# highfem/tqdne

Measured on AMD Instinct MI355X. Metric: waveforms/sec (train step + 18-step EDM sample), 3ch x 4096, higher is better.
Workload: dtype f32 (contractions on MFMA with fp32 accumulate: bf16x3, and fp16 + block-scaled-fp6 corrections on the 128/256-channel forward convs; sampler state f64)

## Files before the change

### include/tqdne_hip.h

```cpp
#ifndef TQDNE_HIP_H
#define TQDNE_HIP_H

#include <stddef.h>
#include <stdint.h>

#ifdef __cplusplus
extern "C" {
#endif

#ifndef __HIP__
typedef struct ihipStream_t* hipStream_t;
#endif

#define TQ_ABI_VERSION 8

#define TQ_ERR_ARG (-1)
#define TQ_ERR_SHAPE (-2)

#define TQ_CONV_GN 1
#define TQ_CONV_SILU 2
#define TQ_CONV_EMB 4
#define TQ_CONV_RES 8
#define TQ_CONV_STATS 16
#define TQ_CONV_DROPOUT 32
#define TQ_CONV_POLY2 64
#define TQ_CONV_CH_TILES 128
#define TQ_CONV_WIDE_TABLE 256

#define TQ_WFMT_BF16X3 0
#define TQ_WFMT_F16_MX8 1
#define TQ_WFMT_F16_MX6 2

typedef struct TqGnFold {
    const float* stats0;
    const float* stats1;
    int32_t slot0, slot1;
    const float* gamma;
    const float* beta;
    float* mean_rstd;
} TqGnFold;

typedef struct TqConvDesc {
    int32_t B, T_in, T_out;
    int32_t C_in0, C_in1;
    int32_t C_out;
    int32_t ktaps, stride, pad;
    int32_t upsample;
    int32_t flags;
    int32_t emb_stride;
    uint32_t dropout_site;
    float dropout_p;
    uint64_t dropout_seed;
    int32_t C_skip0, C_skip1;
    int32_t wfmt;
    int32_t* range_flag;
    const void* reserved1;
    int32_t t_tile;
    int32_t reserved2;
    const TqGnFold* gn_fold;
} TqConvDesc;

#define TQ_BWD_GN 1
#define TQ_BWD_SILU 2
#define TQ_BWD_DROPOUT 4
#define TQ_BWD_ACCUM 8
#define TQ_BWD_STATS 16

typedef struct TqConvBwdDesc {
    int32_t B, T;
    int32_t C_dy;
    int32_t C_dx0, C_dx1;
    int32_t ktaps;
    int32_t flags;
    uint32_t dropout_site;
    float dropout_p;
    uint64_t dropout_seed;
    int32_t wfmt;
    int32_t reserved;
    const uint32_t* dy_amax;
} TqConvBwdDesc;

int tq_abi_version(void);
int tq_build_flags(void);

size_t tq_conv_weight_pack_bytes(int C_out, int C_in, int K, int mode);
int tq_pack_conv_weight(const float* w, int C_out, int C_in, int K, int mode, void* packed, hipStream_t stream);
int tq_conv_tile_co(int C_out);
int tq_conv1d_max_cin(int wfmt, int C_out);
int tq_conv1d_max_cout(void);
size_t tq_conv1d_wide_lds_bytes(int ktaps, int t_tile, int C_out);
int tq_conv1d_gn_table_entries(int wide);
int tq_conv1d_gn_fold_max_cin(int wfmt, int t_tile, int C_out);
int tq_colsum_max_channels(void);
typedef struct TqPackJob {
    const void* src;
    void* dst;
    int32_t C_out, C_in, K, mode;
    int32_t block_begin;
    int32_t reserved;
} TqPackJob;
int tq_pack_job_blocks(int C_out, int C_in, int K, int mode);
int tq_pack_jobs(const TqPackJob* jobs_device, int njobs, int total_blocks, hipStream_t stream);

int tq_conv1d_fwd(const TqConvDesc* desc, const float* x0, const float* x1, const float* gscale, const float* gshift,
                  const void* packed_w, const float* bias, const float* emb, const float* residual, float* y,
                  float* stats_partial, hipStream_t stream);

int tq_conv1d_fwd_skip(const TqConvDesc* desc, const float* x0, const float* x1, const float* gscale, const float* gshift,
                       const void* packed_w_main_then_skip, const float* bias, const float* emb, const float* skip_x0,
                       const float* skip_x1, const float* skip_bias, float* y, float* stats_partial, hipStream_t stream);

#define TQ_KV_V_BF16 0
#define TQ_KV_V_F16 1
int tq_conv1d_fwd_qkv(const TqConvDesc* desc, const float* x, const float* gscale, const float* gshift, const void* packed_w,
                      const float* bias, float* qkv, void* kv_planes, int H, int D, int v_format, hipStream_t stream);

int tq_conv1d_bwd_data(const TqConvBwdDesc* desc, const float* dy, const void* packed_w_t, const float* x0, const float* x1,
                       const float* gscale, const float* gshift, float* dx0, float* dx1, float* gstats_partial,
                       hipStream_t stream);

size_t tq_conv1d_bwd_weight_workspace(const TqConvDesc* desc);
int tq_conv1d_bwd_weight(const TqConvDesc* desc, const float* dy, const float* x0, const float* x1, const float* gscale,
                         const float* gshift, float* dw, void* workspace, size_t ws_bytes, hipStream_t stream);
int tq_conv1d_bwd_weight_colsum(const TqConvDesc* desc, const float* dy, const float* x0, const float* x1, const float* gscale,
                                const float* gshift, float* dw, void* workspace, size_t ws_bytes, float* colsum_bc, int bc_stride,
                                float* colsum_c, float* colsum_c2, hipStream_t stream);

size_t tq_stem_conv_lds_bytes(int C_in, int C_out, int ktaps);
int tq_stem_conv_fwd(const float* x_nct, const float* in_scale, const float* w, const float* bias, float* y,
                     float* stats_partial, int B, int C_in, int T, int C_out, int ktaps, hipStream_t stream);

size_t tq_head_conv_lds_bytes(int C_in, int C_out, int ktaps);
int tq_head_conv_fwd(const float* x, const float* gscale, const float* gshift, const float* w, const float* bias,
                     const float* c_out, const float* c_skip, const float* skip_src, float* y_nct, int B, int T, int C_in,
                     int C_out, int ktaps, hipStream_t stream);

int tq_gn_finalize(const float* stats0, int C0, const float* stats1, int C1, int B, int T, const float* gamma,
                   const float* beta, float* gscale, float* gshift, float* mean_rstd, int slot0, int slot1, hipStream_t stream);

int tq_gn_bwd_finalize(const float* gstats_partial, const float* mean_rstd, const float* gamma, int B, int C, int T,
                       float* coef_a, float* coef_b, float* coef_c, float* dgamma, float* dbeta, hipStream_t stream);
int tq_gn_bwd_apply(const float* g, const float* x, const float* r, const float* coef_a, const float* coef_b,
                    const float* coef_c, float* dx, int B, int T, int C_src, int C_total, int c_offset, int accumulate,
                    hipStream_t stream);
int tq_gn_bwd_apply_colsum(const float* g, const float* x, const float* r, const float* coef_a, const float* coef_b,
                           const float* coef_c, float* dx, int B, int T, int C_src, int C_total, int c_offset, int accumulate,
                           float* colsum_bc, int bc_stride, float* colsum_c, float* colsum_c2, uint32_t* amax_out,
                           hipStream_t stream);
typedef struct TqGemmJob {
    const float* A;
    const float* B;
    float* C;
    const float* U;
    int32_t M, N, K;
    int32_t sam, sak, sbk, sbn, ldc, ldu;
    int32_t pre_b;
    int32_t tile_begin;
} TqGemmJob;
int tq_gemm_tiles(int M, int N);
int tq_gemm_f32_jobs(const TqGemmJob* jobs_device, int njobs, int total_tiles, hipStream_t stream);
int tq_fourier_features(const float* t, const float* W, float* out, int B, int half, hipStream_t stream);

#define TQ_AMAX_WAYS 16
#define TQ_AMAX_STRIDE 32
#define TQ_AMAX_WORDS (TQ_AMAX_WAYS * TQ_AMAX_STRIDE)
int tq_colsum(const float* dy, int B, int T, int C, float* out_bc, int bc_stride, float* out_c, float* out_c2,
              const float* bscale, uint32_t* amax_out, hipStream_t stream);
int tq_zero_stuff(const float* dy, float* out, int B, int T_out, int T_in, int C, hipStream_t stream);
int tq_pair_sum(const float* d_up, float* dx, int B, int T, int C, int accumulate, hipStream_t stream);
int tq_upsample_poly_wgrad_fold(const float* dw2, float* dw, int C_out, int C_in, hipStream_t stream);
int tq_stem_conv_bwd_weight(const float* dy, const float* x_nct, const float* in_scale, float* dw, int B, int C_in, int T,
                            int C_out, int ktaps, hipStream_t stream);
size_t tq_stem_head_bwd_workspace(void);
int tq_stem_conv_bwd_weight_ws(const float* dy, const float* x_nct, const float* in_scale, float* dw, int B, int C_in, int T,
                               int C_out, int ktaps, void* workspace, size_t ws_bytes, hipStream_t stream);
int tq_head_conv_bwd_ws(const float* dpred_nct, const float* c_out, const float* x, const float* gscale, const float* gshift,
                        const float* w, float* g_out, float* gstats_partial, float* dw, float* db, int B, int T, int C_in,
                        int C_out, int ktaps, void* workspace, size_t ws_bytes, hipStream_t stream);
size_t tq_head_conv_bwd_lds_bytes(int C_in, int C_out, int ktaps);
int tq_head_conv_bwd(const float* dpred_nct, const float* c_out, const float* x, const float* gscale, const float* gshift,
                     const float* w, float* g_out, float* gstats_partial, float* dw, float* db, int B, int T, int C_in,
                     int C_out, int ktaps, hipStream_t stream);

int tq_embed_fwd(const float* t, const float* cond, const float* fourier_w, const float* w0, const float* b0,
                 const float* w2, const float* b2, const float* cw0, const float* cb0, const float* cw2, const float* cb2,
                 float* emb, float* silu_emb, float* hidden ,
                 int B, int mc, int ncond, hipStream_t stream);

int tq_linear_fwd(const float* x, const float* w, const float* bias, float* out, int B, int E, int N, hipStream_t stream);

size_t tq_attention_workspace_bytes(int B, int T, int H, int D);
int tq_attention_fwd(const float* qkv, float* out, float* lse ,
                     void* workspace , int B, int T,
                     int H, int D, hipStream_t stream);
int tq_attention_fwd_presplit(const float* qkv, const void* kv_planes, float* out, int B, int T, int H, int D, int v_format,
                              hipStream_t stream);
int tq_attention_bwd(const float* qkv, const float* out, const float* dout, const float* lse, float* delta, float* dqkv, int B,
                     int T, int H, int D, hipStream_t stream);
int tq_attention_bwd_ws(const float* qkv, const float* out, const float* dout, const float* lse, float* delta, float* dqkv,
                        void* workspace, int B, int T, int H, int D, hipStream_t stream);
int tq_attention_bwd_ws_kv(const float* qkv, const float* out, const float* dout, const float* lse, float* delta, float* dqkv,
                           void* workspace, const void* kv_planes, int B, int T, int H, int D, hipStream_t stream);

int tq_attention_head_tile(int D);
size_t tq_attention_hd_lds_bytes(int D, int pass);
size_t tq_attention_hd_workspace_bytes(int B, int T, int H, int D);
int tq_attention_fwd_hd(const float* qkv, float* out, float* lse, void* workspace, int B, int T, int H, int D, hipStream_t stream);
int tq_attention_bwd_hd(const float* qkv, const float* out, const float* dout, const float* lse, float* delta, float* dqkv,
                        void* workspace, int B, int T, int H, int D, hipStream_t stream);

int tq_edm_scalars(const float* sigma, int sigma_stride, float sigma_data, float* c_in, float* c_out, float* c_skip,
                   float* c_noise, float* lweight, int B, hipStream_t stream);
int tq_cm_scalars(const float* sigma, int sigma_stride, float sigma_data, float sigma_min, float* c_out, float* c_skip,
                  int B, hipStream_t stream);
int tq_edm_noise_inject(const float* y, const float* unit_noise, const float* eps, float P_mean, float P_std,
                        float* sigma, float* x_noisy, int B, int n_per_sample, hipStream_t stream);
int tq_edm_loss(const float* pred, const float* y, const float* lweight, float* loss_out, float* dpred, int B,
                int n_per_sample, hipStream_t stream);
int tq_heun_euler(const double* x, const float* denoised, const float* sigma, const float* sigma_next, double* d_cur,
                  double* x_next, float* x32, size_t n, hipStream_t stream);
int tq_heun_correct(const double* x, const double* x_next, const float* denoised_next, const double* d_cur,
                    const float* sigma, const float* sigma_next, double* x_out, float* x32, size_t n, hipStream_t stream);
int tq_sampler_init(const double* unit_noise, const float* sigma0, double* x, float* x32, size_t n, hipStream_t stream);

int tq_heun_churn(const double* x, const double* unit_noise, const float* coef, double s_noise, double* x_hat, float* x32,
                  size_t n, hipStream_t stream);

int tq_axpy_sigma(const float* x, const float* noise, const float* sigma, float* out, int B, int n_per_sample,
                  hipStream_t stream);

int tq_scale_add2(const float* x, const float* y, const float* a, const float* c, float* out, int B, int n_per_sample,
                  hipStream_t stream);
int tq_ddpm_step(const float* x, const float* model_out, const float* noise, float* out, size_t n, int epsilon_prediction,
                 double sqrt_one_minus_abar, double inv_sqrt_abar, double clip, double coef_x0, double coef_xt, double sigma,
                 hipStream_t stream);

int tq_pseudo_huber_loss(const float* pred, const float* target, const float* weight, float c, float* loss_out, float* dpred,
                         int B, int n_per_sample, hipStream_t stream);

int tq_mse_loss(const float* a, const float* b, float* loss_out, float* d, size_t n, hipStream_t stream);

int tq_vae_reparam_fwd(const float* enc, const float* eps, float* z, float* kl_out, int B, int L, int T, hipStream_t stream);
int tq_vae_reparam_bwd(const float* enc, const float* eps, const float* dz, float* denc, float kl_weight, int B, int L, int T,
                       hipStream_t stream);

int tq_concat_scale(const float* x, const float* scale, const float* cond_signal, float* out, int B, int C0, int C1, int T,
                    hipStream_t stream);

int tq_boundary_max_channels(void);
int tq_nct_to_btc(const float* x_nct, const float* scale, const float* cond_nct, float* out_btc, int B, int C0, int C1, int T, int Cp,
                  hipStream_t stream);
int tq_btc_to_nct(const float* v_btc, const float* a, const float* s, const float* skip_src, float* y_nct, int B, int T, int Cp,
                  int c_off, int C, hipStream_t stream);

int tq_avg_pool2_fwd(const float* x, float* y, float* stats, int B, int T_in, int C, hipStream_t stream);
int tq_nearest_up2_fwd(const float* x, float* y, float* stats, int B, int T_in, int C, hipStream_t stream);
int tq_avg_pool2_bwd(const float* dy, float* dx, int B, int T_in, int C, int accumulate, hipStream_t stream);

#define TQ_ADAM_CHUNK 4096
typedef struct TqAdamChunk {
    float* p;
    const float* g;
    float* m;
    float* v;
    float* ema;
    int32_t n;
    int32_t reserved;
} TqAdamChunk;
int tq_adam_ema_step(const TqAdamChunk* chunks, int n_chunks, double step_size, double beta1, double beta2, double eps,
                     double inv_bias2_sqrt, double ema_weight, double grad_scale, double decay_factor, hipStream_t stream);
int tq_adam_ema_step_guarded(const TqAdamChunk* chunks, int n_chunks, double step_size, double beta1, double beta2, double eps,
                             double inv_bias2_sqrt, double ema_weight, double grad_scale, double decay_factor,
// ... 36 lines not shown
```

### tqdne_amd/_build.py

```python

from __future__ import annotations

import os
import subprocess
import sys

HERE = os.path.dirname(os.path.abspath(__file__))
CSRC = os.path.join(HERE, "csrc")
LIBDIR = os.path.join(HERE, "lib")
LIBPATH = os.path.join(LIBDIR, "libtqdne_hip.so")
SOURCES = ["conv1d_fwd_k5a.hip", "conv1d_fwd_k5b.hip", "conv1d_fwd_k13.hip", "conv1d_resample.hip", "conv1d_dgrad.hip", "conv1d_mfma.hip",
           "conv1d_fwd_wide.hip", "conv1d_fwd_wide_k13.hip", "small_ops.hip", "attention.hip", "attention_hd.hip", "backward.hip", "ends_wide.hip", "boundary.hip",
           "resample_plain.hip", "classifier.hip"]
ARCH = "gfx950"


def _hipcc() -> str:
    for c in (os.environ.get("HIPCC"), "/opt/rocm/bin/hipcc", "hipcc"):
        if c and (os.path.isabs(c) and os.path.exists(c) or not os.path.isabs(c)):
            return c
    raise RuntimeError("hipcc not found")


def _deps():
    return [os.path.join(CSRC, f) for f in os.listdir(CSRC)] + [os.path.join(HERE, "..", "include", "tqdne_hip.h")]


def needs_build(path: str = None) -> bool:
    path = path or LIBPATH
    if not os.path.exists(path):
        return True
    t = os.path.getmtime(path)
    return any(os.path.getmtime(d) > t for d in _deps() if os.path.exists(d))


def build(force: bool = False, verbose: bool = True, extra_flags=(), out_name=None) -> str:
    global_out = LIBPATH if out_name is None else os.path.join(LIBDIR, out_name)
    if out_name is None and not force and not needs_build(global_out):
        return global_out
    os.makedirs(LIBDIR, exist_ok=True)
    tag = "" if out_name is None else "." + out_name.replace(".so", "")
    objs = []
    procs = []
    for src in SOURCES:
        path = os.path.join(CSRC, src)
        if not os.path.exists(path):
            continue
        obj = os.path.join(LIBDIR, src.replace(".hip", tag + ".o"))
        cmd = [_hipcc(), f"--offload-arch={ARCH}", "-O3", "-fPIC", "-std=c++17", "-Wno-unused-value", "-Wno-ignored-attributes", "-Wno-cuda-compat", *extra_flags,
               "-c", path, "-o", obj]
        if verbose:
            print("[tqdne_amd build]", " ".join(cmd), flush=True)
        procs.append((cmd, subprocess.Popen(cmd, stdout=subprocess.PIPE, stderr=subprocess.STDOUT, text=True)))
        objs.append(obj)
    for cmd, p in procs:
        out, _ = p.communicate()
        if p.returncode != 0:
            raise RuntimeError("hipcc failed: %s\n%s" % (" ".join(cmd), out))
        if verbose and out.strip():
            print(out)
    cmd = [_hipcc(), f"--offload-arch={ARCH}", "-shared", "-fPIC", "-o", global_out] + objs
    if verbose:
        print("[tqdne_amd build]", " ".join(cmd), flush=True)
    r = subprocess.run(cmd, stdout=subprocess.PIPE, stderr=subprocess.STDOUT, text=True)
    if r.returncode != 0:
        raise RuntimeError("link failed:\n" + r.stdout)
    return global_out


if __name__ == "__main__":
    print(build(force="--force" in sys.argv))
```

### tqdne_amd/_lib.py

```python

from __future__ import annotations

import ctypes as C
import os
from typing import Optional

from . import _build

_LIB = None

c_f32p = C.c_void_p
VP = C.c_void_p
I = C.c_int
F = C.c_float
SZ = C.c_size_t

TQ_CONV_GN, TQ_CONV_SILU, TQ_CONV_EMB, TQ_CONV_RES, TQ_CONV_STATS, TQ_CONV_DROPOUT = 1, 2, 4, 8, 16, 32
TQ_CONV_POLY2 = 64
TQ_CONV_CH_TILES = 128
TQ_CONV_WIDE_TABLE = 256
TQ_WFMT_BF16X3, TQ_WFMT_F16_MX8, TQ_WFMT_F16_MX6 = 0, 1, 2
TQ_KV_V_BF16, TQ_KV_V_F16 = 0, 1
PACK_MODE = {TQ_WFMT_BF16X3: 0, TQ_WFMT_F16_MX8: 2, TQ_WFMT_F16_MX6: 3}
PACK_MODE_T = {TQ_WFMT_BF16X3: 1, TQ_WFMT_F16_MX6: 5}


DEFAULT_SCHEME = "f16mx6"
ABI_VERSION = 8


def requested_scheme() -> str:
    v = os.environ.get("TQDNE_CONV_SCHEME", DEFAULT_SCHEME).lower()
    if v not in ("bf16x3", "f16mx8", "f16mx6"):
        raise ValueError(f"TQDNE_CONV_SCHEME={v!r}: expected bf16x3, f16mx8 or f16mx6")
    return v


def attn_v_format() -> int:
    if os.environ.get("TQDNE_ATTN_VF16", "1") == "0" or requested_scheme() == "bf16x3":
        return TQ_KV_V_BF16
    return TQ_KV_V_F16


MX6_C64 = os.environ.get("TQDNE_CONV_MX6_C64", "0") == "1"


WIDE_MX6 = os.environ.get("TQDNE_WIDE_MX6", "1") != "0"


def conv_max_cin(wfmt: int, C_out: int = 0) -> int:
    return load().tq_conv1d_max_cin(wfmt, C_out)


def forward_wfmt(C_out: int, sources, stride: int = 1, upsample: bool = False, k5_act: bool = False,
                 gn: Optional[bool] = None) -> int:
    v = requested_scheme()
    co_ok = C_out % 128 == 0 or (C_out % 64 == 0 and k5_act and not upsample and v == "f16mx6" and MX6_C64)
    ok = stride == 1 and co_ok and all(c % 64 == 0 for c in sources if c)
    if not ok or v == "bf16x3":
        return TQ_WFMT_BF16X3
    fmt = TQ_WFMT_F16_MX6 if v == "f16mx6" else TQ_WFMT_F16_MX8
    cin = sum(c for c in list(sources)[:2] if c)
    if gn is None or gn:
        if cin > conv_max_cin(fmt, C_out) or (cin > load().tq_conv1d_gn_table_entries(0) and not WIDE_MX6):
            return TQ_WFMT_BF16X3
    return fmt
TQ_BWD_GN, TQ_BWD_SILU, TQ_BWD_DROPOUT, TQ_BWD_ACCUM, TQ_BWD_STATS = 1, 2, 4, 8, 16
STAT_SLOT = 128
TQ_AMAX_WAYS, TQ_AMAX_STRIDE = 16, 32
TQ_AMAX_WORDS = TQ_AMAX_WAYS * TQ_AMAX_STRIDE


class TqGnFold(C.Structure):
    _fields_ = [("stats0", C.c_void_p), ("stats1", C.c_void_p), ("slot0", C.c_int32), ("slot1", C.c_int32),
                ("gamma", C.c_void_p), ("beta", C.c_void_p), ("mean_rstd", C.c_void_p)]


class TqConvDesc(C.Structure):
    _fields_ = [
        ("B", C.c_int32), ("T_in", C.c_int32), ("T_out", C.c_int32),
        ("C_in0", C.c_int32), ("C_in1", C.c_int32), ("C_out", C.c_int32),
        ("ktaps", C.c_int32), ("stride", C.c_int32), ("pad", C.c_int32),
        ("upsample", C.c_int32), ("flags", C.c_int32), ("emb_stride", C.c_int32),
        ("dropout_site", C.c_uint32), ("dropout_p", C.c_float), ("dropout_seed", C.c_uint64),
        ("C_skip0", C.c_int32), ("C_skip1", C.c_int32), ("wfmt", C.c_int32),
        ("range_flag", C.c_void_p), ("reserved1", C.c_void_p), ("t_tile", C.c_int32), ("reserved2", C.c_int32),
        ("gn_fold", C.POINTER(TqGnFold)),
    ]


class TqAdamChunk(C.Structure):
    _fields_ = [("p", C.c_void_p), ("g", C.c_void_p), ("m", C.c_void_p), ("v", C.c_void_p), ("ema", C.c_void_p),
                ("n", C.c_int32), ("reserved", C.c_int32)]


TQ_ADAM_CHUNK = 4096


class TqGemmJob(C.Structure):
    _fields_ = [("A", C.c_void_p), ("B", C.c_void_p), ("C", C.c_void_p), ("U", C.c_void_p),
                ("M", C.c_int32), ("N", C.c_int32), ("K", C.c_int32),
                ("sam", C.c_int32), ("sak", C.c_int32), ("sbk", C.c_int32), ("sbn", C.c_int32), ("ldc", C.c_int32), ("ldu", C.c_int32),
                ("pre_b", C.c_int32), ("tile_begin", C.c_int32)]


class TqPackJob(C.Structure):
    _fields_ = [("src", C.c_void_p), ("dst", C.c_void_p), ("C_out", C.c_int32), ("C_in", C.c_int32), ("K", C.c_int32),
                ("mode", C.c_int32), ("block_begin", C.c_int32), ("reserved", C.c_int32)]


class TqConvBwdDesc(C.Structure):
    _fields_ = [
        ("B", C.c_int32), ("T", C.c_int32), ("C_dy", C.c_int32), ("C_dx0", C.c_int32), ("C_dx1", C.c_int32),
        ("ktaps", C.c_int32), ("flags", C.c_int32), ("dropout_site", C.c_uint32), ("dropout_p", C.c_float),
        ("dropout_seed", C.c_uint64), ("wfmt", C.c_int32), ("reserved", C.c_int32), ("dy_amax", C.c_void_p),
    ]


_PROTOS = {
    "tq_abi_version": (I, []),
    "tq_build_flags": (I, []),
    "tq_conv_weight_pack_bytes": (SZ, [I, I, I, I]),
    "tq_pack_conv_weight": (I, [VP, I, I, I, I, VP, VP]),
    "tq_conv_tile_co": (I, [I]),
    "tq_conv1d_max_cin": (I, [I, I]),
    "tq_conv1d_max_cout": (I, []),
    "tq_conv1d_gn_table_entries": (I, [I]),
    "tq_conv1d_wide_lds_bytes": (SZ, [I, I, I]),
    "tq_conv1d_gn_fold_max_cin": (I, [I, I, I]),
    "tq_colsum_max_channels": (I, []),
    "tq_conv1d_fwd": (I, [C.POINTER(TqConvDesc)] + [VP] * 11),
    "tq_conv1d_fwd_skip": (I, [C.POINTER(TqConvDesc)] + [VP] * 13),
    "tq_stem_conv_fwd": (I, [VP] * 6 + [I] * 5 + [VP]),
    "tq_head_conv_fwd": (I, [VP] * 9 + [I] * 5 + [VP]),
    "tq_head_conv_lds_bytes": (SZ, [I, I, I]),
    "tq_stem_conv_lds_bytes": (SZ, [I, I, I]),
    "tq_head_conv_bwd_lds_bytes": (SZ, [I, I, I]),
    "tq_gn_finalize": (I, [VP, I, VP, I, I, I, VP, VP, VP, VP, VP, I, I, VP]),
    "tq_embed_fwd": (I, [VP] * 14 + [I, I, I, VP]),
    "tq_linear_fwd": (I, [VP] * 4 + [I, I, I, VP]),
    "tq_attention_fwd": (I, [VP, VP, VP, VP, I, I, I, I, VP]),
    "tq_attention_fwd_presplit": (I, [VP, VP, VP, I, I, I, I, I, VP]),
    "tq_conv1d_fwd_qkv": (I, [C.POINTER(TqConvDesc)] + [VP] * 7 + [I, I, I, VP]),
    "tq_attention_workspace_bytes": (SZ, [I, I, I, I]),
    "tq_attention_bwd": (I, [VP] * 6 + [I, I, I, I, VP]),
    "tq_attention_bwd_ws": (I, [VP] * 7 + [I, I, I, I, VP]),
    "tq_attention_bwd_ws_kv": (I, [VP] * 8 + [I, I, I, I, VP]),
    "tq_attention_head_tile": (I, [I]),
    "tq_attention_hd_lds_bytes": (SZ, [I, I]),
    "tq_attention_hd_workspace_bytes": (SZ, [I, I, I, I]),
    "tq_attention_fwd_hd": (I, [VP, VP, VP, VP, I, I, I, I, VP]),
    "tq_attention_bwd_hd": (I, [VP] * 7 + [I, I, I, I, VP]),
    "tq_edm_scalars": (I, [VP, I, F, VP, VP, VP, VP, VP, I, VP]),
    "tq_cm_scalars": (I, [VP, I, F, F, VP, VP, I, VP]),
    "tq_edm_noise_inject": (I, [VP, VP, VP, F, F, VP, VP, I, I, VP]),
    "tq_edm_loss": (I, [VP, VP, VP, VP, VP, I, I, VP]),
    "tq_heun_euler": (I, [VP] * 7 + [SZ, VP]),
    "tq_heun_correct": (I, [VP] * 8 + [SZ, VP]),
    "tq_sampler_init": (I, [VP] * 4 + [SZ, VP]),
    "tq_heun_churn": (I, [VP, VP, VP, C.c_double, VP, VP, SZ, VP]),
    "tq_axpy_sigma": (I, [VP, VP, VP, VP, I, I, VP]),
    "tq_pseudo_huber_loss": (I, [VP, VP, VP, F, VP, VP, I, I, VP]),
    "tq_mse_loss": (I, [VP, VP, VP, VP, SZ, VP]),
    "tq_scale_add2": (I, [VP, VP, VP, VP, VP, I, I, VP]),
    "tq_ddpm_step": (I, [VP, VP, VP, VP, SZ, I] + [C.c_double] * 6 + [VP]),
    "tq_vae_reparam_fwd": (I, [VP, VP, VP, VP, I, I, I, VP]),
    "tq_vae_reparam_bwd": (I, [VP, VP, VP, VP, F, I, I, I, VP]),
    "tq_concat_scale": (I, [VP, VP, VP, VP, I, I, I, I, VP]),
    "tq_envelope_fwd": (I, [VP, VP, I, I, I, I, C.c_double, C.c_double, VP]),
    "tq_envelope_inv": (I, [VP, VP, I, I, I, C.c_double, C.c_double, VP]),
    "tq_adam_ema_step": (I, [VP, I] + [C.c_double] * 8 + [VP]),
    "tq_adam_ema_step_guarded": (I, [VP, I] + [C.c_double] * 8 + [VP, VP]),
    "tq_radam_ema_step_guarded": (I, [VP, I] + [C.c_double] * 7 + [VP, VP]),
    "tq_adam_ema_step_clipped": (I, [VP, I] + [C.c_double] * 8 + [VP, VP, C.c_double, VP]),
    "tq_radam_ema_step_clipped": (I, [VP, I] + [C.c_double] * 7 + [VP, VP, C.c_double, VP]),
    "tq_grad_sumsq": (I, [VP, I, VP, VP]),
    "tq_grad_clip_coef": (I, [VP, I, C.c_double, C.c_double, VP, VP]),
    "tq_ema_swap": (I, [VP, I, VP]),
    "tq_conv1d_bwd_data": (I, [VP] * 11),
    "tq_conv1d_bwd_weight_workspace": (SZ, [VP]),
    "tq_conv1d_bwd_weight": (I, [VP] * 8 + [SZ, VP]),
    "tq_conv1d_bwd_weight_colsum": (I, [VP] * 8 + [SZ, VP, I, VP, VP, VP]),
    "tq_gn_bwd_finalize": (I, [VP, VP, VP, I, I, I, VP, VP, VP, VP, VP, VP]),
    "tq_gn_bwd_apply": (I, [VP] * 7 + [I] * 6 + [VP]),
    "tq_gn_bwd_apply_colsum": (I, [VP] * 7 + [I] * 6 + [VP, I, VP, VP, VP, VP]),
    "tq_pack_job_blocks": (I, [I, I, I, I]),
    "tq_pack_jobs": (I, [VP, I, I, VP]),
    "tq_gemm_tiles": (I, [I, I]),
    "tq_gemm_f32_jobs": (I, [VP, I, I, VP]),
    "tq_fourier_features": (I, [VP, VP, VP, I, I, VP]),
    "tq_colsum": (I, [VP, I, I, I, VP, I, VP, VP, VP, VP, VP]),
    "tq_zero_stuff": (I, [VP, VP, I, I, I, I, VP]),
    "tq_pair_sum": (I, [VP, VP, I, I, I, I, VP]),
    "tq_upsample_poly_wgrad_fold": (I, [VP, VP, I, I, VP]),
    "tq_stem_conv_bwd_weight": (I, [VP] * 4 + [I] * 5 + [VP]),
    "tq_head_conv_bwd": (I, [VP] * 10 + [I] * 5 + [VP]),
    "tq_stem_head_bwd_workspace": (SZ, []),
    "tq_stem_conv_bwd_weight_ws": (I, [VP] * 4 + [I] * 5 + [VP, SZ, VP]),
    "tq_head_conv_bwd_ws": (I, [VP] * 10 + [I] * 5 + [VP, SZ, VP]),
    "tq_boundary_max_channels": (I, []),
    "tq_nct_to_btc": (I, [VP] * 4 + [I] * 5 + [VP]),
    "tq_btc_to_nct": (I, [VP] * 5 + [I] * 5 + [VP]),
    "tq_avg_pool2_fwd": (I, [VP, VP, VP, I, I, I, VP]),
    "tq_nearest_up2_fwd": (I, [VP, VP, VP, I, I, I, VP]),
    "tq_avg_pool2_bwd": (I, [VP, VP, I, I, I, I, VP]),
    "tq_classifier_head_max_channels": (I, []),
    "tq_classifier_head_max_classes": (I, []),
    "tq_classifier_head_bwd_workspace": (SZ, [I, I]),
    "tq_classifier_head_fwd": (I, [VP] * 11 + [I] * 4 + [VP]),
    "tq_cross_entropy": (I, [VP, VP, VP, C.c_int64, VP, VP, I, I, VP]),
    "tq_classifier_head_bwd": (I, [VP] * 15 + [SZ] + [I] * 4 + [VP]),
}

def lib_path() -> str:
    return os.environ.get("TQDNE_HIP_LIB", _build.LIBPATH)


def load():
    global _LIB
    if _LIB is not None:
        return _LIB
    path = lib_path()
    if not os.path.exists(path):
        raise RuntimeError(
            f"{path} is missing: the tqdne_amd hot path is HIP-only (no CPU / PyTorch fallback). "
            "Build it with `python -m tqdne_amd._build` (needs hipcc, cross-compiles gfx950 without a GPU)."
        )
    lib = C.CDLL(path)
    for name, (res, args) in _PROTOS.items():
        fn = getattr(lib, name)
        fn.restype = res
        fn.argtypes = args
    if lib.tq_abi_version() != ABI_VERSION:
        raise RuntimeError("libtqdne_hip.so ABI version mismatch")
    _LIB = lib
    return lib


def exported_symbols():
    return sorted(_PROTOS)


class TqError(RuntimeError):
    pass


def _p(t):
    return None if t is None else t.data_ptr()


def check(rc: int, what: str = ""):
    if rc != 0:
        kind = {-1: "TQ_ERR_ARG", -2: "TQ_ERR_SHAPE"}.get(rc, f"hipError_t {rc}")
        raise TqError(f"libtqdne_hip: {what} failed with {kind}")
```

### tqdne_amd/csrc/backward.hip

```cpp
#include <cstdlib>
#include "common.hpp"
#include "ends_wide.hpp"
#include "../../include/tqdne_hip.h"

using namespace tq;

namespace {

typedef short s16x4 __attribute__((ext_vector_type(4)));

__device__ __forceinline__ uint2 lds_tr_read(const unsigned char* p) {
    s16x4 v = __builtin_amdgcn_ds_read_tr16_b64_v4i16((__attribute__((address_space(3))) s16x4*)(p));
    union { s16x4 s; uint2 u; } c;
    c.s = v;
    return c.u;
}

struct WgArgs {
    const float* dy;
    const float* x0;
    const float* x1;
    const float* gscale;
    const float* gshift;
    float* slab;
// ... 500 lines not shown

extern "C" size_t tq_conv1d_bwd_weight_workspace(const TqConvDesc* d) {
    if (!d) return 0;
    int a, b, c, nsplit, nsplit4, ups;
    wgrad_plan(d, true, a, b, c, nsplit, ups);
    wgrad_plan(d, false, a, b, c, nsplit4, ups);
    return (size_t)(nsplit > nsplit4 ? nsplit : nsplit4) * d->ktaps * d->C_out * (d->C_in0 + d->C_in1) * sizeof(float);
}

extern "C" int tq_conv1d_bwd_weight(const TqConvDesc* d, const float* dy, const float* x0, const float* x1,
                                    const float* gscale, const float* gshift, float* dw, void* workspace, size_t ws_bytes,
                                    hipStream_t stream) {
    return tq_conv1d_bwd_weight_colsum(d, dy, x0, x1, gscale, gshift, dw, workspace, ws_bytes, nullptr, 0, nullptr, nullptr, stream);
}

extern "C" int tq_conv1d_bwd_weight_colsum(const TqConvDesc* d, const float* dy, const float* x0, const float* x1,
                                           const float* gscale, const float* gshift, float* dw, void* workspace, size_t ws_bytes,
                                           float* colsum_bc, int bc_stride, float* colsum_c, float* colsum_c2,
                                           hipStream_t stream) {
    if (!d || !dy || !x0 || !dw || !workspace) return TQ_ERR_ARG;
    if (colsum_c2 && !colsum_c) return TQ_ERR_ARG;
    if (d->C_in0 <= 0 || d->C_in0 % 32 || d->C_in1 < 0 || d->C_in1 % 32 || d->C_out <= 0 || d->C_out % 32) return TQ_ERR_SHAPE;
    if (d->C_in1 > 0 && !x1) return TQ_ERR_ARG;
    if ((d->flags & TQ_CONV_GN) && (!gscale || !gshift)) return TQ_ERR_ARG;
    if (ws_bytes < tq_conv1d_bwd_weight_workspace(d)) return TQ_ERR_ARG;
    WgArgs a;
    a.dy = dy; a.x0 = x0; a.x1 = x1; a.gscale = gscale; a.gshift = gshift; a.slab = reinterpret_cast<float*>(workspace);
    a.B = d->B; a.T_in = d->T_in; a.T_out = d->T_out; a.C0 = d->C_in0; a.C1 = d->C_in1; a.C_out = d->C_out;
    a.flags = d->flags;
    a.cs_bc = colsum_bc; a.cs_stride = bc_stride; a.cs_c = colsum_c; a.cs_c2 = colsum_c2;
    const bool wide = !(colsum_bc || colsum_c);
    wgrad_plan(d, wide, a.n_cotiles, a.n_cichunks, a.n_ttiles, a.nsplit, a.units_per_split);
    static const bool plain_order = [] { const char* e = getenv("TQDNE_WGRAD_XCD"); return e && atoi(e) == 0; }();
    if (plain_order) a.flags |= TQ_WGRAD_PLAIN_ORDER;
    a.drop_site = d->dropout_site; a.drop_seed = d->dropout_seed;
    float pdrop = d->dropout_p;
    if (!(d->flags & TQ_CONV_DROPOUT) || pdrop <= 0.f) { a.flags &= ~TQ_CONV_DROPOUT; pdrop = 0.f; }
    a.drop_thresh = (uint32_t)((double)pdrop * 4294967296.0);
    a.drop_scale = 1.0f / (1.0f - pdrop);
    int rc;
    const int nci = wgrad_nci(d);
    const bool h64 = wide && wgrad_h64(d);
    const bool w8 = wide && !h64 && wgrad_w8(d);
    if (d->stride == 2) {
        if (d->ktaps != 3) return TQ_ERR_SHAPE;
        rc = launch_wgrad<3, 2, 0>(a, nci, w8, false, stream);
    } else if (d->upsample) {
        if (d->ktaps == 5) rc = launch_wgrad<5, 1, 1>(a, nci, w8, false, stream);
        else if (d->ktaps == 3) rc = launch_wgrad<3, 1, 1>(a, nci, w8, false, stream);
        else return TQ_ERR_SHAPE;
    } else {
        if (d->ktaps == 5) rc = launch_wgrad<5, 1, 0>(a, nci, w8, h64, stream);
        else if (d->ktaps == 3) rc = launch_wgrad<3, 1, 0>(a, nci, w8, h64, stream);
        else if (d->ktaps == 1) rc = launch_wgrad<1, 1, 0>(a, nci, false, false, stream);
        else return TQ_ERR_SHAPE;
    }
    if (rc) return rc;
    const size_t n = (size_t)d->C_out * (d->C_in0 + d->C_in1);
    const dim3 rgrid((unsigned)((n + 63) / 64)), rblock(16, 16);
    if (d->ktaps == 5) hipLaunchKernelGGL(wgrad_reduce_kernel<5>, rgrid, rblock, 0, stream, a.slab, dw, a.nsplit, n);
    else if (d->ktaps == 3) hipLaunchKernelGGL(wgrad_reduce_kernel<3>, rgrid, rblock, 0, stream, a.slab, dw, a.nsplit, n);
    else hipLaunchKernelGGL(wgrad_reduce_kernel<1>, rgrid, rblock, 0, stream, a.slab, dw, a.nsplit, n);
    TQ_CHECK_LAUNCH();
    return 0;
}

namespace {
__global__ __launch_bounds__(256) void gn_bwd_finalize_kernel(const float* __restrict__ gst, const float* __restrict__ mr,
                                                              const float* __restrict__ gamma, int C, int T, int nslots,
                                                              float* __restrict__ cA, float* __restrict__ cB,
                                                              float* __restrict__ cC, float* __restrict__ dgamma,
                                                              float* __restrict__ dbeta) {
    extern __shared__ double sh[];
    const int b = blockIdx.x;
    const int Cb = C / (int)gridDim.y;
    const int c0 = (int)blockIdx.y * Cb;
    int nsub = Cb <= 128 ? (int)blockDim.x / Cb : 1;
    if (nsub > nslots) nsub = nslots;
    double* cs = sh;
    double* gp = sh + 2 * Cb * nsub;
    for (int idx = threadIdx.x; idx < Cb * nsub; idx += blockDim.x) {
        const int c = idx % Cb, sub = idx / Cb;
        const float* pp = gst + ((size_t)b * nslots * C + c0 + c) * 2;
        double s1 = 0.0, s2 = 0.0;
        int s = sub;
        for (; s + 3 * nsub < nslots; s += 4 * nsub) {
            const float2 v0 = *reinterpret_cast<const float2*>(pp + (size_t)s * C * 2);
            const float2 v1 = *reinterpret_cast<const float2*>(pp + (size_t)(s + nsub) * C * 2);
            const float2 v2 = *reinterpret_cast<const float2*>(pp + (size_t)(s + 2 * nsub) * C * 2);
            const float2 v3 = *reinterpret_cast<const float2*>(pp + (size_t)(s + 3 * nsub) * C * 2);
            s1 += ((double)v0.x + (double)v1.x) + ((double)v2.x + (double)v3.x);
            s2 += ((double)v0.y + (double)v1.y) + ((double)v2.y + (double)v3.y);
        }
        for (; s < nslots; s += nsub) {
            const float2 v = *reinterpret_cast<const float2*>(pp + (size_t)s * C * 2);
            s1 += (double)v.x; s2 += (double)v.y;
        }
        cs[2 * idx] = s1; cs[2 * idx + 1] = s2;
    }
    __syncthreads();
    if (nsub > 1) {
        double t1 = 0.0, t2 = 0.0;
        const int c = threadIdx.x;
        if (c < Cb)
            for (int sub = 0; sub < nsub; ++sub) { t1 += cs[2 * (sub * Cb + c)]; t2 += cs[2 * (sub * Cb + c) + 1]; }
        __syncthreads();
        if (c < Cb) { cs[2 * c] = t1; cs[2 * c + 1] = t2; }
        __syncthreads();
    }
    const int G = C / GN_GROUPS;
    const int ngrp = Cb / G, g0 = c0 / G;
    if ((int)threadIdx.x < ngrp) {
        const int gl = threadIdx.x, g = g0 + gl;
        const double mean = (double)mr[((size_t)b * GN_GROUPS + g) * 2], rstd = (double)mr[((size_t)b * GN_GROUPS + g) * 2 + 1];
        double p1 = 0.0, p2 = 0.0;
        for (int j = 0; j < G; ++j) {
            const int cl = gl * G + j;
            const double gm = (double)gamma[c0 + cl];
            p1 += gm * cs[2 * cl];
            p2 += gm * (cs[2 * cl + 1] - mean * cs[2 * cl]);
        }
        p2 *= rstd;
        const double n = (double)G * (double)T;
        gp[2 * gl] = -rstd * rstd * p2 / n;
        gp[2 * gl + 1] = rstd * rstd * p2 * mean / n - rstd * p1 / n;
    }
    __syncthreads();
    for (int cl = threadIdx.x; cl < Cb; cl += blockDim.x) {
        const int c = c0 + cl;
        const int g = c / G, gl = g - g0;
        const float mean = mr[((size_t)b * GN_GROUPS + g) * 2], rstd = mr[((size_t)b * GN_GROUPS + g) * 2 + 1];
        cA[(size_t)b * C + c] = rstd * gamma[c];
        cB[(size_t)b * C + c] = (float)gp[2 * gl];
        cC[(size_t)b * C + c] = (float)gp[2 * gl + 1];
        atomicAdd(dgamma + c, (float)((double)rstd * (cs[2 * cl + 1] - (double)mean * cs[2 * cl])));
        atomicAdd(dbeta + c, (float)cs[2 * cl]);
    }
}

__global__ void gn_bwd_apply_kernel(const float* __restrict__ g, const float* __restrict__ x, const float* __restrict__ r,
                                    const float* __restrict__ cA, const float* __restrict__ cB, const float* __restrict__ cC,
                                    float* __restrict__ dx, int T, int Cs, int Ctot, int coff, int accum, size_t n4) {
    const int c4n = Cs >> 2;
    for (size_t i = (size_t)blockIdx.x * blockDim.x + threadIdx.x; i < n4; i += (size_t)gridDim.x * blockDim.x) {
        const int c4 = (int)(i % c4n);
        const size_t bt = i / c4n;
        const int b = (int)(bt / T);
        const size_t ko = (size_t)b * Ctot + coff + 4 * c4;
        const float4 a = *reinterpret_cast<const float4*>(cA + ko);
        const float4 bb = *reinterpret_cast<const float4*>(cB + ko);
        const float4 cc = *reinterpret_cast<const float4*>(cC + ko);
        const float4 gv = reinterpret_cast<const float4*>(g)[i];
        const float4 xv = reinterpret_cast<const float4*>(x)[i];
        float4 o = make_float4(a.x * gv.x + bb.x * xv.x + cc.x, a.y * gv.y + bb.y * xv.y + cc.y,
                               a.z * gv.z + bb.z * xv.z + cc.z, a.w * gv.w + bb.w * xv.w + cc.w);
        if (r) { const float4 rv = reinterpret_cast<const float4*>(r)[i]; o.x += rv.x; o.y += rv.y; o.z += rv.z; o.w += rv.w; }
        if (accum) { const float4 ov = reinterpret_cast<const float4*>(dx)[i]; o.x += ov.x; o.y += ov.y; o.z += ov.z; o.w += ov.w; }
        reinterpret_cast<float4*>(dx)[i] = o;
    }
}

constexpr int AMAX_WAYS = TQ_AMAX_WAYS;
constexpr int AMAX_STRIDE = TQ_AMAX_STRIDE;

template <int NT>
__device__ __forceinline__ void colsum_finish(float* red, const float4& a, float mx, bool active, int c4n, int nrow, int c4, int tr, int C,
                                              int b, float sc, float* __restrict__ out_bc, int bc_stride, float* __restrict__ out_c,
                                              float* __restrict__ out_c2, unsigned* __restrict__ amax_out) {
    if (active) *reinterpret_cast<float4*>(red + (tr * c4n + c4) * 4) = a;
    unsigned* wmax = reinterpret_cast<unsigned*>(red + (size_t)nrow * c4n * 4);
    if (amax_out) {
        unsigned m = __float_as_uint(mx);
#pragma unroll
        for (int o = 32; o > 0; o >>= 1) m = max(m, (unsigned)__shfl_xor((int)m, o));
        if ((threadIdx.x & 63) == 0) wmax[threadIdx.x >> 6] = m;
    }
    __syncthreads();
    if (amax_out && threadIdx.x == 0) {
        unsigned m = wmax[0];
#pragma unroll
        for (int w = 1; w < NT / 64; ++w) m = max(m, wmax[w]);
        if (m != 0u) atomicMax(amax_out + (blockIdx.x % AMAX_WAYS) * AMAX_STRIDE, m);
    }
    for (int c = threadIdx.x; c < C; c += NT) {
        float s = 0.f;
        for (int r2 = 0; r2 < nrow; ++r2) s += red[(r2 * c4n + (c >> 2)) * 4 + (c & 3)];
        s *= sc;
        if (out_bc) atomicAdd(out_bc + (size_t)b * bc_stride + c, s);
        if (out_c) atomicAdd(out_c + c, s);
        if (out_c2) atomicAdd(out_c2 + c, s);
    }
}
__device__ __forceinline__ float amax4(float m, const float4& v) {
    const float t = fmaxf(fmaxf(fabsf(v.x), fabsf(v.y)), fmaxf(fabsf(v.z), fabsf(v.w)));
    const bool bad = (v.x != v.x) | (v.y != v.y) | (v.z != v.z) | (v.w != v.w);
    return bad ? __builtin_inff() : fmaxf(m, t);
}

template <int NT>
__global__ __launch_bounds__(NT) void colsum_kernel(const float* __restrict__ dy, int T, int C, float* __restrict__ out_bc,
                                                     int bc_stride, float* __restrict__ out_c, float* __restrict__ out_c2,
                                                     const float* __restrict__ bscale, unsigned* __restrict__ amax_out, int rpw) {
    extern __shared__ float red[];
    const int nsl = (T + rpw - 1) / rpw;
    const int slot = blockIdx.x % nsl, b = blockIdx.x / nsl;
    const int c4n = C >> 2;
    const int nrow = NT / c4n > 0 ? NT / c4n : 1;
    const int c4 = threadIdx.x % c4n, tr = threadIdx.x / c4n;
    float4 a = make_float4(0.f, 0.f, 0.f, 0.f);
    float mx = 0.f;
    const bool active = tr < nrow && threadIdx.x < nrow * c4n;
    if (active) {
        const int nvalid = min(rpw, T - slot * rpw);
        const float* src = dy + ((size_t)b * T + (size_t)slot * rpw) * C + 4 * c4;
        int tl = tr;
        for (; tl + 7 * nrow < nvalid; tl += 8 * nrow) {
            float4 v[8];
#pragma unroll
            for (int q = 0; q < 8; ++q) v[q] = *reinterpret_cast<const float4*>(src + (size_t)(tl + q * nrow) * C);
#pragma unroll
            for (int q = 0; q < 8; ++q) { a.x += v[q].x; a.y += v[q].y; a.z += v[q].z; a.w += v[q].w; }
            if (amax_out) {
#pragma unroll
                for (int q = 0; q < 8; ++q) mx = amax4(mx, v[q]);
            }
        }
        for (; tl < nvalid; tl += nrow) {
            const float4 v = *reinterpret_cast<const float4*>(src + (size_t)tl * C);
            a.x += v.x; a.y += v.y; a.z += v.z; a.w += v.w;
            if (amax_out) mx = amax4(mx, v);
        }
    }
    colsum_finish<NT>(red, a, mx, active, c4n, nrow, c4, tr, C, b, bscale ? bscale[b] : 1.0f, out_bc, bc_stride, out_c, out_c2, amax_out);
}

template <int NT>
__global__ __launch_bounds__(NT) void gn_bwd_apply_cs_kernel(const float* __restrict__ g, const float* __restrict__ x,
                                                              const float* __restrict__ r, const float* __restrict__ cA,
                                                              const float* __restrict__ cB, const float* __restrict__ cC,
                                                              float* __restrict__ dx, int T, int Cs, int Ctot, int coff, int accum,
                                                              float* __restrict__ out_bc, int bc_stride, float* __restrict__ out_c,
                                                              float* __restrict__ out_c2, unsigned* __restrict__ amax_out, int rpw) {
    extern __shared__ float red[];
    const int nsl = (T + rpw - 1) / rpw;
    const int slot = blockIdx.x % nsl, b = blockIdx.x / nsl;
    const int c4n = Cs >> 2;
    const int nrow = NT / c4n > 0 ? NT / c4n : 1;
    const int c4 = threadIdx.x % c4n, tr = threadIdx.x / c4n;
    float4 a = make_float4(0.f, 0.f, 0.f, 0.f);
    float mx = 0.f;
    const bool active = tr < nrow && threadIdx.x < nrow * c4n;
    if (active) {
        const int nvalid = min(rpw, T - slot * rpw);
        const size_t ko = (size_t)b * Ctot + coff + 4 * c4;
        const float4 ka = *reinterpret_cast<const float4*>(cA + ko);
        const float4 kb = *reinterpret_cast<const float4*>(cB + ko);
        const float4 kc = *reinterpret_cast<const float4*>(cC + ko);
        const size_t base = ((size_t)b * T + (size_t)slot * rpw) * Cs + 4 * c4;
        auto one = [&](const float4& gv, const float4& xv, const float4& rv, const float4& ov) -> float4 __attribute__((always_inline)) {
            float4 o = make_float4(ka.x * gv.x + kb.x * xv.x + kc.x, ka.y * gv.y + kb.y * xv.y + kc.y,
                                   ka.z * gv.z + kb.z * xv.z + kc.z, ka.w * gv.w + kb.w * xv.w + kc.w);
            o.x += rv.x; o.y += rv.y; o.z += rv.z; o.w += rv.w;
            o.x += ov.x; o.y += ov.y; o.z += ov.z; o.w += ov.w;
            return o;
        };
        const float4 z4 = make_float4(0.f, 0.f, 0.f, 0.f);
        int tl = tr;
        for (; tl + 3 * nrow < nvalid; tl += 4 * nrow) {
            float4 gv[4], xv[4], rv[4], ov[4];
#pragma unroll
            for (int q = 0; q < 4; ++q) {
                const size_t o = base + (size_t)(tl + q * nrow) * Cs;
                gv[q] = *reinterpret_cast<const float4*>(g + o);
                xv[q] = *reinterpret_cast<const float4*>(x + o);
                rv[q] = r ? *reinterpret_cast<const float4*>(r + o) : z4;
                ov[q] = accum ? *reinterpret_cast<const float4*>(dx + o) : z4;
            }
#pragma unroll
            for (int q = 0; q < 4; ++q) {
                const float4 o4 = one(gv[q], xv[q], rv[q], ov[q]);
                *reinterpret_cast<float4*>(dx + base + (size_t)(tl + q * nrow) * Cs) = o4;
                a.x += o4.x; a.y += o4.y; a.z += o4.z; a.w += o4.w;
                mx = amax4(mx, o4);
            }
        }
        for (; tl < nvalid; tl += nrow) {
            const size_t o = base + (size_t)tl * Cs;
            const float4 o4 = one(*reinterpret_cast<const float4*>(g + o), *reinterpret_cast<const float4*>(x + o),
                                  r ? *reinterpret_cast<const float4*>(r + o) : z4, accum ? *reinterpret_cast<const float4*>(dx + o) : z4);
            *reinterpret_cast<float4*>(dx + o) = o4;
            a.x += o4.x; a.y += o4.y; a.z += o4.z; a.w += o4.w;
            mx = amax4(mx, o4);
        }
    }
    colsum_finish<NT>(red, a, mx, active, c4n, nrow, c4, tr, Cs, b, 1.0f, out_bc, bc_stride, out_c, out_c2, amax_out);
}

struct CsChunk { int c0, cw; };
__device__ __forceinline__ CsChunk cs_chunk(int C, int cw) {
    const int c0 = (int)blockIdx.y * cw;
    return CsChunk{c0, min(cw, C - c0)};
}

template <int NT>
__global__ __launch_bounds__(NT) void colsum_chunk_kernel(const float* __restrict__ dy, int T, int C, int cw, float* __restrict__ out_bc,
                                                           int bc_stride, float* __restrict__ out_c, float* __restrict__ out_c2,
                                                           const float* __restrict__ bscale, unsigned* __restrict__ amax_out, int rpw) {
    extern __shared__ float red[];
    const CsChunk ck = cs_chunk(C, cw);
    const int nsl = (T + rpw - 1) / rpw;
    const int slot = blockIdx.x % nsl, b = blockIdx.x / nsl;
    const int c4n = ck.cw >> 2;
    const int nrow = NT / c4n > 0 ? NT / c4n : 1;
    const int c4 = threadIdx.x % c4n, tr = threadIdx.x / c4n;
    float4 a = make_float4(0.f, 0.f, 0.f, 0.f);
    float mx = 0.f;
    const bool active = tr < nrow && threadIdx.x < nrow * c4n;
    if (active) {
        const int nvalid = min(rpw, T - slot * rpw);
        const float* src = dy + ((size_t)b * T + (size_t)slot * rpw) * C + ck.c0 + 4 * c4;
        int tl = tr;
        for (; tl + 7 * nrow < nvalid; tl += 8 * nrow) {
            float4 v[8];
#pragma unroll
            for (int q = 0; q < 8; ++q) v[q] = *reinterpret_cast<const float4*>(src + (size_t)(tl + q * nrow) * C);
#pragma unroll
            for (int q = 0; q < 8; ++q) { a.x += v[q].x; a.y += v[q].y; a.z += v[q].z; a.w += v[q].w; }
            if (amax_out) {
#pragma unroll
                for (int q = 0; q < 8; ++q) mx = amax4(mx, v[q]);
            }
        }
        for (; tl < nvalid; tl += nrow) {
            const float4 v = *reinterpret_cast<const float4*>(src + (size_t)tl * C);
            a.x += v.x; a.y += v.y; a.z += v.z; a.w += v.w;
            if (amax_out) mx = amax4(mx, v);
        }
    }
    colsum_finish<NT>(red, a, mx, active, c4n, nrow, c4, tr, ck.cw, b, bscale ? bscale[b] : 1.0f, out_bc ? out_bc + ck.c0 : nullptr, bc_stride,
                      out_c ? out_c + ck.c0 : nullptr, out_c2 ? out_c2 + ck.c0 : nullptr, amax_out);
}

template <int NT>
__global__ __launch_bounds__(NT) void gn_bwd_apply_cs_chunk_kernel(const float* __restrict__ g, const float* __restrict__ x,
                                                                    const float* __restrict__ r, const float* __restrict__ cA,
                                                                    const float* __restrict__ cB, const float* __restrict__ cC,
                                                                    float* __restrict__ dx, int T, int Cs, int cw, int Ctot, int coff, int accum,
                                                                    float* __restrict__ out_bc, int bc_stride, float* __restrict__ out_c,
                                                                    float* __restrict__ out_c2, unsigned* __restrict__ amax_out, int rpw) {
    extern __shared__ float red[];
    const CsChunk ck = cs_chunk(Cs, cw);
    const int nsl = (T + rpw - 1) / rpw;
    const int slot = blockIdx.x % nsl, b = blockIdx.x / nsl;
    const int c4n = ck.cw >> 2;
    const int nrow = NT / c4n > 0 ? NT / c4n : 1;
    const int c4 = threadIdx.x % c4n, tr = threadIdx.x / c4n;
    float4 a = make_float4(0.f, 0.f, 0.f, 0.f);
    float mx = 0.f;
    const bool active = tr < nrow && threadIdx.x < nrow * c4n;
    if (active) {
        const int nvalid = min(rpw, T - slot * rpw);
        const size_t ko = (size_t)b * Ctot + coff + ck.c0 + 4 * c4;
        const float4 ka = *reinterpret_cast<const float4*>(cA + ko);
        const float4 kb = *reinterpret_cast<const float4*>(cB + ko);
        const float4 kc = *reinterpret_cast<const float4*>(cC + ko);
        const size_t base = ((size_t)b * T + (size_t)slot * rpw) * Cs + ck.c0 + 4 * c4;
        const float4 z4 = make_float4(0.f, 0.f, 0.f, 0.f);
        for (int tl = tr; tl < nvalid; tl += nrow) {
            const size_t o = base + (size_t)tl * Cs;
            const float4 gv = *reinterpret_cast<const float4*>(g + o), xv = *reinterpret_cast<const float4*>(x + o);
            const float4 rv = r ? *reinterpret_cast<const float4*>(r + o) : z4, ov = accum ? *reinterpret_cast<const float4*>(dx + o) : z4;
            float4 o4 = make_float4(ka.x * gv.x + kb.x * xv.x + kc.x, ka.y * gv.y + kb.y * xv.y + kc.y,
                                    ka.z * gv.z + kb.z * xv.z + kc.z, ka.w * gv.w + kb.w * xv.w + kc.w);
            o4.x += rv.x; o4.y += rv.y; o4.z += rv.z; o4.w += rv.w;
            o4.x += ov.x; o4.y += ov.y; o4.z += ov.z; o4.w += ov.w;
            *reinterpret_cast<float4*>(dx + o) = o4;
            a.x += o4.x; a.y += o4.y; a.z += o4.z; a.w += o4.w;
            mx = amax4(mx, o4);
        }
    }
    colsum_finish<NT>(red, a, mx, active, c4n, nrow, c4, tr, ck.cw, b, 1.0f, out_bc ? out_bc + ck.c0 : nullptr, bc_stride,
                      out_c ? out_c + ck.c0 : nullptr, out_c2 ? out_c2 + ck.c0 : nullptr, amax_out);
}


__global__ void zero_stuff_kernel(const float* __restrict__ dy, float* __restrict__ out, int T_out, int T_in, int C, size_t n4) {
    const int c4n = C >> 2;
    for (size_t i = (size_t)blockIdx.x * blockDim.x + threadIdx.x; i < n4; i += (size_t)gridDim.x * blockDim.x) {
        const int c4 = (int)(i % c4n);
        const size_t bu = i / c4n;
        const int u = (int)(bu % T_in);
        const size_t b = bu / T_in;
        float4 v = make_float4(0.f, 0.f, 0.f, 0.f);
        if (!(u & 1) && (u >> 1) < T_out) v = reinterpret_cast<const float4*>(dy)[(b * T_out + (u >> 1)) * c4n + c4];
        reinterpret_cast<float4*>(out)[i] = v;
    }
}

__global__ void pair_sum_kernel(const float* __restrict__ dup, float* __restrict__ dx, int T, int C, int accum, size_t n4) {
    const int c4n = C >> 2;
    for (size_t i = (size_t)blockIdx.x * blockDim.x + threadIdx.x; i < n4; i += (size_t)gridDim.x * blockDim.x) {
        const int c4 = (int)(i % c4n);
        const size_t bt = i / c4n;
        const int t = (int)(bt % T);
        const size_t b = bt / T;
        const float4 a = reinterpret_cast<const float4*>(dup)[(b * 2 * T + 2 * t) * c4n + c4];
        const float4 c = reinterpret_cast<const float4*>(dup)[(b * 2 * T + 2 * t + 1) * c4n + c4];
        float4 o = make_float4(a.x + c.x, a.y + c.y, a.z + c.z, a.w + c.w);
        if (accum) { const float4 ov = reinterpret_cast<const float4*>(dx)[i]; o.x += ov.x; o.y += ov.y; o.z += ov.z; o.w += ov.w; }
        reinterpret_cast<float4*>(dx)[i] = o;
    }
}

inline unsigned ew_grid4(size_t n4) {
    size_t g = (n4 + 255) / 256;
    return (unsigned)(g > 4096 ? 4096 : (g ? g : 1));
}
}

extern "C" int tq_gn_bwd_finalize(const float* gstats, const float* mean_rstd, const float* gamma, int B, int C, int T,
                                  float* coef_a, float* coef_b, float* coef_c, float* dgamma, float* dbeta,
                                  hipStream_t stream) {
    if (!gstats || !mean_rstd || !gamma || !coef_a || !coef_b || !coef_c || !dgamma || !dbeta) return TQ_ERR_ARG;
    if (B <= 0 || T <= 0 || C <= 0 || C % GN_GROUPS) return TQ_ERR_SHAPE;
    const int nslots = (T + STAT_SLOT - 1) / STAT_SLOT;
    const int NP = 4;
    const int Cb = C / NP;
    int nsub = Cb <= 128 ? 256 / Cb : 1;
    if (nsub > nslots) nsub = nslots;
    const size_t sh = (size_t)(2 * Cb * nsub + 2 * GN_GROUPS) * sizeof(double);
    hipLaunchKernelGGL(gn_bwd_finalize_kernel, dim3(B, NP), dim3(256), sh, stream, gstats, mean_rstd, gamma, C, T, nslots, coef_a,
                       coef_b, coef_c, dgamma, dbeta);
    TQ_CHECK_LAUNCH();
    return 0;
}

extern "C" int tq_gn_bwd_apply(const float* g, const float* x, const float* r, const float* coef_a, const float* coef_b,
                               const float* coef_c, float* dx, int B, int T, int C_src, int C_total, int c_offset, int accumulate,
                               hipStream_t stream) {
    if (!g || !x || !coef_a || !coef_b || !coef_c || !dx) return TQ_ERR_ARG;
    if (B <= 0 || T <= 0 || C_src <= 0 || C_src % 4 || c_offset % 4 || c_offset + C_src > C_total) return TQ_ERR_SHAPE;
    const size_t n4 = (size_t)B * T * (C_src / 4);
    hipLaunchKernelGGL(gn_bwd_apply_kernel, dim3(ew_grid4(n4)), dim3(256), 0, stream, g, x, r, coef_a, coef_b, coef_c, dx, T,
                       C_src, C_total, c_offset, accumulate, n4);
    TQ_CHECK_LAUNCH();
    return 0;
}

constexpr int CS_NT = 256;
struct CsTiling { int rows; };
static CsTiling colsum_tiling(int B, int T) {
    CsTiling t;
    const size_t min_wgs = 256;
    int rpw = STAT_SLOT;
    while (rpw < 4096 && (size_t)B * ((T + 2 * rpw - 1) / (2 * rpw)) >= min_wgs) rpw <<= 1;
    t.rows = rpw;
    return t;
}

constexpr int CS_CHUNK = 1024;
constexpr int CS_MAX_C = CS_CHUNK * 64;
static int colsum_chunk_width(int C, int& nchunks) {
    const int c4 = C / 4;
    nchunks = (c4 + CS_CHUNK / 4 - 1) / (CS_CHUNK / 4);
    return ((c4 + nchunks - 1) / nchunks) * 4;
}
extern "C" int tq_colsum_max_channels(void) { return CS_MAX_C; }

extern "C" int tq_colsum(const float* dy, int B, int T, int C, float* out_bc, int bc_stride, float* out_c, float* out_c2,
                         const float* bscale, uint32_t* amax_out, hipStream_t stream) {
    if (!dy || (!out_bc && !out_c && !out_c2 && !amax_out)) return TQ_ERR_ARG;
    if (B <= 0 || T <= 0 || C < 4 || C % 4 || C > CS_MAX_C) return TQ_ERR_SHAPE;
    const CsTiling tl = colsum_tiling(B, T);
    const int nsl = (T + tl.rows - 1) / tl.rows;
    if (C > CS_CHUNK) {
        int nch;
        const int cw = colsum_chunk_width(C, nch);
        const size_t shw = (size_t)(CS_NT > cw / 4 ? CS_NT : cw / 4) * 4 * sizeof(float) + (CS_NT / 64) * sizeof(unsigned);
        hipLaunchKernelGGL(colsum_chunk_kernel<CS_NT>, dim3(B * nsl, nch), dim3(CS_NT), shw, stream, dy, T, C, cw, out_bc, bc_stride, out_c, out_c2, bscale, amax_out, tl.rows);
        TQ_CHECK_LAUNCH();
        return 0;
    }
    const int c4n = C / 4;
    const int nrow = CS_NT / c4n > 0 ? CS_NT / c4n : 1;
    const size_t sh = (size_t)nrow * c4n * 4 * sizeof(float) + (CS_NT / 64) * sizeof(unsigned);
    hipLaunchKernelGGL(colsum_kernel<CS_NT>, dim3(B * nsl), dim3(CS_NT), sh, stream, dy, T, C, out_bc, bc_stride, out_c, out_c2, bscale, amax_out, tl.rows);
    TQ_CHECK_LAUNCH();
    return 0;
}

extern "C" int tq_gn_bwd_apply_colsum(const float* g, const float* x, const float* r, const float* coef_a, const float* coef_b,
                                      const float* coef_c, float* dx, int B, int T, int C_src, int C_total, int c_offset, int accumulate,
                                      float* colsum_bc, int bc_stride, float* colsum_c, float* colsum_c2, uint32_t* amax_out,
                                      hipStream_t stream) {
    if (!g || !x || !coef_a || !coef_b || !coef_c || !dx) return TQ_ERR_ARG;
    if (colsum_c2 && !colsum_c) return TQ_ERR_ARG;
    if (B <= 0 || T <= 0 || C_src <= 0 || C_src % 4 || C_src > CS_MAX_C || c_offset % 4 || c_offset + C_src > C_total) return TQ_ERR_SHAPE;
    if (!colsum_bc && !colsum_c && !amax_out)
        return tq_gn_bwd_apply(g, x, r, coef_a, coef_b, coef_c, dx, B, T, C_src, C_total, c_offset, accumulate, stream);
    const CsTiling tl = colsum_tiling(B, T);
    const int nsl = (T + tl.rows - 1) / tl.rows;
    if (C_src > CS_CHUNK) {
        int nch;
        const int cw = colsum_chunk_width(C_src, nch);
        const size_t shw = (size_t)(CS_NT > cw / 4 ? CS_NT : cw / 4) * 4 * sizeof(float) + (CS_NT / 64) * sizeof(unsigned);
        hipLaunchKernelGGL(gn_bwd_apply_cs_chunk_kernel<CS_NT>, dim3(B * nsl, nch), dim3(CS_NT), shw, stream, g, x, r, coef_a, coef_b, coef_c, dx, T,
                           C_src, cw, C_total, c_offset, accumulate, colsum_bc, bc_stride, colsum_c, colsum_c2, amax_out, tl.rows);
        TQ_CHECK_LAUNCH();
        return 0;
    }
    const int c4n = C_src / 4;
    const int nrow = CS_NT / c4n > 0 ? CS_NT / c4n : 1;
    const size_t sh = (size_t)nrow * c4n * 4 * sizeof(float) + (CS_NT / 64) * sizeof(unsigned);
    hipLaunchKernelGGL(gn_bwd_apply_cs_kernel<CS_NT>, dim3(B * nsl), dim3(CS_NT), sh, stream, g, x, r, coef_a, coef_b, coef_c, dx, T, C_src,
                       C_total, c_offset, accumulate, colsum_bc, bc_stride, colsum_c, colsum_c2, amax_out, tl.rows);
    TQ_CHECK_LAUNCH();
    return 0;
}

extern "C" int tq_zero_stuff(const float* dy, float* out, int B, int T_out, int T_in, int C, hipStream_t stream) {
    if (!dy || !out || B <= 0 || T_out <= 0 || T_in <= 0 || C <= 0 || C % 4) return TQ_ERR_ARG;
    const size_t n4 = (size_t)B * T_in * (C / 4);
    hipLaunchKernelGGL(zero_stuff_kernel, dim3(ew_grid4(n4)), dim3(256), 0, stream, dy, out, T_out, T_in, C, n4);
    TQ_CHECK_LAUNCH();
    return 0;
}
// ... 593 lines not shown
```

### tqdne_amd/csrc/common.hpp

```cpp
#pragma once
#include <hip/hip_runtime.h>
#include <stdint.h>

#include <cstdlib>

namespace tq {

typedef __bf16 bf16x8 __attribute__((ext_vector_type(8)));
typedef __bf16 bf16x4 __attribute__((ext_vector_type(4)));
typedef float f32x4 __attribute__((ext_vector_type(4)));
typedef _Float16 f16x8 __attribute__((ext_vector_type(8)));
typedef _Float16 f16x4 __attribute__((ext_vector_type(4)));
typedef short i16x2 __attribute__((ext_vector_type(2)));
typedef int i32x8 __attribute__((ext_vector_type(8)));

constexpr int WAVE = 64;

constexpr int GN_GROUPS = 32;
constexpr float GN_EPS = 1e-5f;
constexpr int STAT_SLOT = 128;

__device__ __forceinline__ float silu_f(float u) {
    return u * __builtin_amdgcn_rcpf(1.0f + __expf(-u));
}
__device__ __forceinline__ float dsilu_f(float u) {
    float s = __builtin_amdgcn_rcpf(1.0f + __expf(-u));
    return s * (1.0f + u * (1.0f - s));
}

__device__ __forceinline__ void split_bf16(float x, __bf16& hi, __bf16& lo) {
    hi = (__bf16)x;
    lo = (__bf16)(x - (float)hi);
}

union Frag {
    bf16x8 v;
    uint4 u;
    uint2 h[2];
};

__device__ __forceinline__ f32x4 mfma_bf16(const bf16x8& a, const bf16x8& b, f32x4 c) {
    return __builtin_amdgcn_mfma_f32_16x16x32_bf16(a, b, c, 0, 0, 0);
}

__device__ __forceinline__ f32x4 mfma_x3(const bf16x8& ah, const bf16x8& al, const bf16x8& bh, const bf16x8& bl, f32x4 c) {
    c = mfma_bf16(al, bh, c);
    c = mfma_bf16(ah, bl, c);
    c = mfma_bf16(ah, bh, c);
    return c;
}

__device__ __forceinline__ int xcd_group_id(int bid, int inner, int n_outer) {
    if (n_outer & 7) return bid;
    const int x = bid & 7, s = bid >> 3;
    return (x + 8 * (s / inner)) * inner + (s % inner);
}

__device__ __forceinline__ float wave_sum(float v) {
#pragma unroll
    for (int o = 32; o > 0; o >>= 1) v += __shfl_xor(v, o);
    return v;
}
__device__ __forceinline__ double wave_sum_d(double v) {
#pragma unroll
    for (int o = 32; o > 0; o >>= 1) v += __shfl_xor(v, o);
    return v;
}

__device__ __forceinline__ uint32_t mix32(uint32_t x) {
    x ^= x >> 16; x *= 0x7FEB352Du;
    x ^= x >> 15; x *= 0x846CA68Bu;
    x ^= x >> 16;
    return x;
}
struct DropKey { uint32_t a, b; };
__device__ __forceinline__ DropKey drop_key(uint64_t seed, uint32_t site, uint32_t b) {
    uint32_t k = mix32((uint32_t)seed ^ 0x9E3779B9u);
    k = mix32(k ^ (uint32_t)(seed >> 32));
    k = mix32(k + 0x85EBCA6Bu * (site + 1u));
    DropKey r;
    r.a = mix32(k + 0xC2B2AE35u * (b + 1u));
    r.b = mix32((k ^ 0x27D4EB2Fu) + 0x165667B1u * (b + 1u));
    return r;
}
__device__ __forceinline__ uint32_t drop_hash(DropKey key, uint32_t e) {
    uint32_t x = e ^ key.a;
    x ^= x >> 16; x *= 0x7FEB352Du;
    x += key.b;
    x ^= x >> 15; x *= 0x846CA68Bu;
    x ^= x >> 16;
    return x;
}

}

#define TQ_CHECK_LAUNCH()                                   \
    do {                                                    \
        hipError_t e__ = hipGetLastError();                 \
        if (e__ != hipSuccess) return (int)e__;             \
    } while (0)
```

### tqdne_amd/csrc/conv1d_kernel.hpp

```cpp
#pragma once
#include <cmath>
#include <cstdlib>
#include <type_traits>

#include "common.hpp"
#include "conv_args.hpp"
#include "gn_fold.hpp"
#include <atomic>
#include "../../include/tqdne_hip.h"

using namespace tq;

#ifdef TQ_STAMP
static __device__ unsigned long long tq_stamps[12];
#ifdef TQ_STAMP_OWNER
extern "C" int tq_debug_read_stamps(unsigned long long* out, int reset) {
    hipError_t e = hipMemcpyFromSymbol(out, HIP_SYMBOL(tq_stamps), sizeof(unsigned long long) * 12);
    if (e != hipSuccess) return (int)e;
    if (reset) {
        unsigned long long z[12] = {0, 0, 0, 0, 0, 0, 0, 0, 0, 0, 0, 0};
        e = hipMemcpyToSymbol(HIP_SYMBOL(tq_stamps), z, sizeof(z));
    }
    return (int)e;
}
#endif
static __device__ unsigned long long tq_timeline[4096 * 8];
#ifdef TQ_STAMP_OWNER
extern "C" int tq_debug_read_timeline(unsigned long long* out, int n) {
    return (int)hipMemcpyFromSymbol(out, HIP_SYMBOL(tq_timeline), sizeof(unsigned long long) * 8 * n);
}
#endif
#define TQ_T(x) const unsigned long long x = __builtin_amdgcn_s_memtime(); __builtin_amdgcn_sched_barrier(0);
#else
#define TQ_T(x)
#endif

namespace {

#ifndef TQ_STAGE_PRE
#define TQ_STAGE_PRE 5
#endif

template <int KT, int STRIDE, int UPS, int WM, int WN, int SCH = 0, int TBW = 8, int NCB = 2>
struct Cfg {
    static constexpr int CH = SCH ? 64 : 32;
    static constexpr int ROWB = 2 * CH;
    static constexpr int TPR = (SCH == 2) ? 4 : CH / 4;
    static constexpr int NWB = SCH ? 4 : 2;
    static constexpr int NW = NWB * NCB;
    static constexpr int NBF = SCH ? 4 : 2;
    static constexpr int NTHR = 64 * WM * WN;
    static constexpr int WT = 16 * TBW;
    static constexpr int NT = WT * WN;
    static constexpr int MT = 16 * NCB * WM;
    static constexpr int ROWS = (STRIDE == 1) ? (NT + KT - 1) : (2 * NT + 1);
    static constexpr int NIT = (ROWS * TPR + NTHR - 1) / NTHR;
    static constexpr int PRE_MAX = (SCH == 1 && WM == 4) ? 1 : TQ_STAGE_PRE;
    static constexpr int PRE = NIT < PRE_MAX ? NIT : PRE_MAX;
    static constexpr int SYNC_BATCH = 4;
    static constexpr int ITERS = (NIT <= PRE) ? NIT : PRE + ((NIT - PRE + SYNC_BATCH - 1) / SYNC_BATCH) * SYNC_BATCH;
    static constexpr int NFULL = (SCH == 2) ? (NT * 4) / NTHR : 0;
    static constexpr int HALO_TASKS = (SCH == 2) ? (ROWS - NT) * 4 : 0;
    static constexpr int ROWS_PAD = (SCH == 2) ? ROWS : (ITERS * NTHR + TPR - 1) / TPR;
    static constexpr int PLANE = (ROWS_PAD > ROWS ? ROWS_PAD : ROWS) * ROWB;
    static constexpr int BUF = 2 * PLANE;
    static constexpr int LDS_BYTES = 2 * BUF;
    static constexpr int PAD = (STRIDE == 1) ? (KT / 2) : 1;
};

template <int KT, int STRIDE, int UPS, int WM, int WN, int EPI, int ACT, bool FUSE, int SCH, bool PW = false, int TBW = 8, int NCB = 2, int GTW = 1024>
__global__ __launch_bounds__(64 * WM * WN, 2) void conv1d_mfma_kernel(const ConvArgs p) {
    static_assert(GTW == 1024 || (GTW == 2048 && SCH == 2 && ACT >= 1 && EPI == 0 && !PW && STRIDE == 1 && UPS == 0 && WN == 1 && NCB == 2 && (TBW == 8 || TBW == 2)),
                  "wide coefficient table: the fp16 + MX-fp6 forward tiles of 128 and 32 positions");
    static_assert(SCH == 0 || STRIDE == 1, "the fp16-range schemes serve stride-1 launches");
    static_assert(EPI != 1 || SCH == 0 || (SCH == 2 && ACT == 0 && !FUSE && !PW), "data gradients: bf16x3, or fp16 + MX-fp6 on a dy scaled into the fp16 range");
    static_assert(NCB == 2, "waves are 32 channels wide");
    constexpr bool C64 = TBW == 4 && NCB == 2 && SCH == 2 && WM == 2 && WN == 2;
    static_assert(!C64 || (STRIDE == 1 && UPS == 0 && !PW && EPI != 2), "64-channel fp16 + MX-fp6 tile: stride-1 forward and data-gradient launches");
    static_assert(TBW == 8 || C64 || (TBW == 2 && (SCH == 0 || (SCH == 2 && WM == 4)) && STRIDE == 1 && UPS == 0 && EPI == 0 && WN == 1 && !PW),
                  "small tile (32 positions per workgroup): stride-1 forward, one wave column");
    static_assert(!PW || (KT == 1 && STRIDE == 1 && UPS == 0 && SCH >= 1 && !FUSE && WN == 1 && EPI != 1), "PW: 1x1, fp16-range schemes");
    static_assert(SCH != 2 || WN == 1 || C64, "scheme 2 tiles are 128 positions wide");
    using C = Cfg<KT, STRIDE, UPS, WM, WN, SCH, TBW, NCB>;
    extern __shared__ __attribute__((aligned(16))) unsigned char lds[];
#ifdef TQ_STAMP
    const unsigned long long t_entry = __builtin_amdgcn_s_memtime();
    const unsigned long long r_entry = __builtin_amdgcn_s_memrealtime();
#endif

    const int tid = threadIdx.x;
    const int lane = tid & 63;
    const int wave = __builtin_amdgcn_readfirstlane(tid >> 6);
    const int wm = wave % WM;
    const int wn = wave / WM;

    const int n_ttiles = (p.T_out + C::NT - 1) / C::NT;
    const int n_ctiles = (p.C_out + C::MT - 1) / C::MT;
    int bid = blockIdx.x;
    int ct, tile;
    const int ntile = p.B * n_ttiles;
    if constexpr (PW) {
        ct = 0;
        tile = bid;
    } else if (n_ctiles > 1 && (ntile & 7) == 0) {
        const int grp = bid / (8 * n_ctiles), within = bid % (8 * n_ctiles);
        ct = within >> 3;
        tile = grp * 8 + (within & 7);
    } else {
        ct = bid % n_ctiles;
        tile = bid / n_ctiles;
    }
    const int tt = tile % n_ttiles;
    const int b = tile / n_ttiles;
    const int t0 = tt * C::NT;
    float dy_scale = 1.f, dy_unscale = 1.f;
    if constexpr (EPI == 1 && SCH == 2) {
        if (p.in_amax) {
            uint32_t amx = 0u;
#pragma unroll
            for (int w = 0; w < TQ_AMAX_WAYS; ++w) amx = max(amx, p.in_amax[w * TQ_AMAX_STRIDE]);
            const int e = (int)((amx >> 23) & 0xFFu);
            int k = 140 - e;
            k = k > 126 ? 126 : (k < -126 ? -126 : k);
            dy_scale = __uint_as_float((unsigned)(127 + k) << 23);
            dy_unscale = __uint_as_float((unsigned)(127 - k) << 23);
        }
    }
    const DropKey dkey = (ACT == 3 || EPI == 1) ? drop_key(p.drop_seed, p.drop_site, (uint32_t)b) : DropKey{0u, 0u};
    int co_wave = ct * C::MT + wm * (16 * NCB);
    const bool wave_active = co_wave < p.C_out;

    const int Cin = p.C0 + p.C1;
    const int nchunks = Cin / C::CH;
    const int nskip = FUSE ? ((p.sC0 + p.sC1) / C::CH) : 0;
    const int nstages = nchunks + nskip;
    const int T_src = UPS ? 2 * p.T_in : p.T_in;

    const int m = tid % C::TPR;
    const int wslot = m >> 1, whalf = m & 1;
    constexpr bool TIGHT = SCH == 1 && WM == 8 && C::PRE == 5 && C::NIT == 5;
    constexpr int PRE = (TIGHT && ACT == 3) ? 1 : (TIGHT && FUSE) ? 4 : C::PRE;
    constexpr int SYNC_BATCH = (TIGHT && ACT == 3) ? 4 : (TIGHT && FUSE) ? 1 : C::SYNC_BATCH;
    float4 raw[PRE];
    float4 g_a, g_s;

    auto src_pos = [&](int i) -> int __attribute__((always_inline)) {
        if (STRIDE == 1) return t0 - C::PAD + i;
        const int par = (i > C::NT) ? 1 : 0;
        const int idx = i - par * (C::NT + 1);
        return 2 * t0 - C::PAD + 2 * idx + par;
    };

    auto chunk_base = [&](int stage, int& cs) -> const float* __attribute__((always_inline)) {
        const bool sk = FUSE && stage >= nchunks;
        const int cb = (sk ? stage - nchunks : stage) * C::CH;
        const float* a0 = sk ? p.sx0 : p.x0;
        const float* a1 = sk ? p.sx1 : p.x1;
        const int c0 = sk ? p.sC0 : p.C0, c1 = sk ? p.sC1 : p.C1;
        const bool first = cb < c0;
        const float* src = first ? a0 : a1;
        cs = first ? c0 : c1;
        const int coff = first ? cb : cb - c0;
        return src + (size_t)b * p.T_in * cs + coff + 4 * m;
    };

    auto load_one = [&](const float* base, int cs, int it) -> float4 __attribute__((always_inline)) {
        const int i = (tid + it * C::NTHR) / C::TPR;
        int pos = src_pos(i);
        pos = pos < 0 ? 0 : (pos >= T_src ? T_src - 1 : pos);
        const int srow = UPS ? (pos >> 1) : pos;
        return *reinterpret_cast<const float4*>(base + (size_t)srow * cs);
    };

    auto write_one = [&](int chunk, int buf, int it, const float4& rv) __attribute__((always_inline)) {
        unsigned char* hi_plane = lds + buf * C::BUF;
        unsigned char* lo_plane = hi_plane + C::PLANE;
        const int i = (tid + it * C::NTHR) / C::TPR;
        const int pos = src_pos(i);
        const float msk = (pos >= 0 && pos < T_src) ? 1.f : 0.f;
        float u[4] = {rv.x, rv.y, rv.z, rv.w};
        const bool act = !(FUSE && chunk >= nchunks);
        if (ACT >= 1 && act) {
            u[0] = fmaf(g_a.x, u[0], g_s.x); u[1] = fmaf(g_a.y, u[1], g_s.y);
            u[2] = fmaf(g_a.z, u[2], g_s.z); u[3] = fmaf(g_a.w, u[3], g_s.w);
        }
        if (ACT >= 2 && act) {
#pragma unroll
            for (int j = 0; j < 4; ++j)
                u[j] = u[j] * __builtin_amdgcn_rcpf(1.0f + __builtin_amdgcn_exp2f(u[j] * -1.4426950408889634f));
        }
        if (ACT == 3 && act) {
            const int cb = chunk * C::CH;
            const int pc = pos < 0 ? 0 : pos;
            const uint32_t e0 = (uint32_t)pc * (uint32_t)Cin + (uint32_t)(cb + 4 * m);
#pragma unroll
            for (int j = 0; j < 4; ++j)
                u[j] = (drop_hash(dkey, e0 + j) >= p.drop_thresh) ? u[j] * p.drop_scale : 0.f;
        }
        if constexpr (SCH == 0) {
            uint32_t hb[4];
            float lo[4];
#pragma unroll
            for (int j = 0; j < 4; ++j) {
                u[j] *= msk;
                hb[j] = __float_as_uint(u[j]) & 0xFFFF0000u;
                lo[j] = u[j] - __uint_as_float(hb[j]);
            }
            uint2 hv;
            hv.x = (hb[0] >> 16) | hb[1];
            hv.y = (hb[2] >> 16) | hb[3];
            bf16x4 l;
            l[0] = (__bf16)lo[0]; l[1] = (__bf16)lo[1]; l[2] = (__bf16)lo[2]; l[3] = (__bf16)lo[3];
            const int off = i * 64 + ((wslot ^ (((i >> 2) & 1) << 1)) << 4) + (whalf << 3);
            *reinterpret_cast<uint2*>(hi_plane + off) = hv;
            *reinterpret_cast<bf16x4*>(lo_plane + off) = l;
        } else {
            f16x4 hv;
            float xl[4], xc[4];
#pragma unroll
            for (int j = 0; j < 4; ++j) {
                u[j] *= msk;
                hv[j] = (_Float16)u[j];
                xl[j] = __builtin_amdgcn_fmed3f(u[j] - (float)hv[j], -0.109375f, 0.109375f);
                xc[j] = __builtin_amdgcn_fmed3f(u[j], -448.f, 448.f);
// ... 583 lines not shown
            const float sc = sec == 1 ? p.kvscale : 1.0f;
            const int dch = d0 + (odd ? 16 + 4 * (g - 1) : 4 * g);
            unsigned char* base0 = p.kv + (((size_t)b * p.kvH + h) * 4 + (sec == 1 ? 0 : 2)) * plane + (size_t)dch * 2;
            float vmax = 0.f;
#pragma unroll
            for (int tb = 0; tb < TBW; ++tb) {
                const int t = t0 + wn * C::WT + tb * 16 + (lane & 15);
                uint2 hi[2], lo[2];
#pragma unroll
                for (int cbk = 0; cbk < 2; ++cbk) {
                    const float v[4] = {acc[cbk][tb][0] + add[cbk].x, acc[cbk][tb][1] + add[cbk].y,
                                        acc[cbk][tb][2] + add[cbk].z, acc[cbk][tb][3] + add[cbk].w};
                    if (sec == 2 && p.kv_vf16) {
                        f16x4 hh, ll;
#pragma unroll
                        for (int j = 0; j < 4; ++j) {
                            hh[j] = (_Float16)v[j];
                            ll[j] = (_Float16)(v[j] - (float)hh[j]);
                            vmax = fmaxf(vmax, fabsf(v[j]));
                        }
                        hi[cbk] = __builtin_bit_cast(uint2, hh);
                        lo[cbk] = __builtin_bit_cast(uint2, ll);
                    } else {
                        bf16x4 hh, ll;
#pragma unroll
                        for (int j = 0; j < 4; ++j) {
                            __bf16 a, c;
                            split_bf16(v[j] * sc, a, c);
                            hh[j] = a; ll[j] = c;
                        }
                        hi[cbk] = __builtin_bit_cast(uint2, hh);
                        lo[cbk] = __builtin_bit_cast(uint2, ll);
                    }
                }
                const uint2 sh = odd ? hi[0] : hi[1], sl = odd ? lo[0] : lo[1];
                uint2 rh, rl;
                rh.x = __shfl_xor((int)sh.x, 16); rh.y = __shfl_xor((int)sh.y, 16);
                rl.x = __shfl_xor((int)sl.x, 16); rl.y = __shfl_xor((int)sl.y, 16);
                const uint4 oh = odd ? make_uint4(rh.x, rh.y, hi[1].x, hi[1].y) : make_uint4(hi[0].x, hi[0].y, rh.x, rh.y);
                const uint4 ol = odd ? make_uint4(rl.x, rl.y, lo[1].x, lo[1].y) : make_uint4(lo[0].x, lo[0].y, rl.x, rl.y);
                if (t < p.T_out) {
                    unsigned char* dst = base0 + (size_t)t * p.kvD * 2;
                    *reinterpret_cast<uint4*>(dst) = oh;
                    *reinterpret_cast<uint4*>(dst + plane) = ol;
                }
            }
            if (p.range_flag && !(vmax < 32752.f)) *p.range_flag = 1;
        }
    } else if constexpr (EPI == 0) {
    const bool poly = p.flags & TQ_CONV_POLY2;
    const int Cr = poly ? (p.C_out >> 1) : p.C_out;
    const int ph = (poly && co_wave >= Cr) ? 1 : 0;
    const int co_real = co_wave - ph * Cr;
    const int slot = poly ? 2 * ((t0 >> 7) + wn) + ph : (TBW == 2 ? (t0 >> 5) : (t0 >> 7) + (TBW == 8 ? wn : 0));
    const float* emb_b = (p.flags & TQ_CONV_EMB) ? p.emb + (size_t)b * p.emb_stride : nullptr;
    float4 add[NCB];
    float s1[NCB][4], s2[NCB][4];
#pragma unroll
    for (int cbk = 0; cbk < NCB; ++cbk) {
        const int co = co_real + cbk * 16 + 4 * (lane >> 4);
        add[cbk] = make_float4(0.f, 0.f, 0.f, 0.f);
        if (p.bias) add[cbk] = *reinterpret_cast<const float4*>(p.bias + co);
        if (emb_b) {
            const float4 e = *reinterpret_cast<const float4*>(emb_b + co);
            add[cbk].x += e.x; add[cbk].y += e.y; add[cbk].z += e.z; add[cbk].w += e.w;
        }
        if (FUSE && p.sbias) {
            const float4 e = *reinterpret_cast<const float4*>(p.sbias + co);
            add[cbk].x += e.x; add[cbk].y += e.y; add[cbk].z += e.z; add[cbk].w += e.w;
        }
#pragma unroll
        for (int j = 0; j < 4; ++j) { s1[cbk][j] = 0.f; s2[cbk][j] = 0.f; }
    }
    const bool res_epi = (!RES_EARLY || poly) && (p.flags & TQ_CONV_RES);
    float4 rq[TBW][NCB];
    if (res_epi) {
#pragma unroll
        for (int tb = 0; tb < TBW; ++tb) {
            const int t = t0 + wn * C::WT + tb * 16 + (lane & 15);
            const int tc = t < p.T_out ? t : p.T_out - 1;
#pragma unroll
            for (int cbk = 0; cbk < NCB; ++cbk) {
                const int co = co_real + cbk * 16 + 4 * (lane >> 4);
                const size_t o = poly ? ((size_t)b * 2 * p.T_out + 2 * tc + ph) * Cr + co : ((size_t)b * p.T_out + tc) * p.C_out + co;
                rq[tb][cbk] = *reinterpret_cast<const float4*>(p.res + o);
            }
        }
    }
#pragma unroll
    for (int tb = 0; tb < TBW; ++tb) {
        int t = t0 + wn * C::WT + tb * 16 + (lane & 15);
        asm volatile("" : "+v"(t));
        if (t < p.T_out) {
#pragma unroll
            for (int cbk = 0; cbk < NCB; ++cbk) {
                const int co = co_real + cbk * 16 + 4 * (lane >> 4);
                const size_t o = poly ? ((size_t)b * 2 * p.T_out + 2 * t + ph) * Cr + co : ((size_t)b * p.T_out + t) * p.C_out + co;
                float4 v = make_float4(acc[cbk][tb][0] + add[cbk].x, acc[cbk][tb][1] + add[cbk].y,
                                       acc[cbk][tb][2] + add[cbk].z, acc[cbk][tb][3] + add[cbk].w);
                if (res_epi) {
                    const float4 r = rq[tb][cbk];
                    v.x += r.x; v.y += r.y; v.z += r.z; v.w += r.w;
                }
#ifdef TQ_ABL_NOEPI
                if (v.x == 1.2345e30f)
#endif
                *reinterpret_cast<float4*>(p.y + o) = v;
                s1[cbk][0] += v.x; s1[cbk][1] += v.y; s1[cbk][2] += v.z; s1[cbk][3] += v.w;
                s2[cbk][0] += v.x * v.x; s2[cbk][1] += v.y * v.y; s2[cbk][2] += v.z * v.z; s2[cbk][3] += v.w * v.w;
            }
        }
    }
    if (p.flags & TQ_CONV_STATS) {
#pragma unroll
        for (int cbk = 0; cbk < NCB; ++cbk) {
#pragma unroll
            for (int j = 0; j < 4; ++j) {
#pragma unroll
                for (int o = 1; o < 16; o <<= 1) {
                    s1[cbk][j] += __shfl_xor(s1[cbk][j], o);
                    s2[cbk][j] += __shfl_xor(s2[cbk][j], o);
                }
            }
        }
        if constexpr (TBW == 4) {
            __syncthreads();
            float* red = reinterpret_cast<float*>(lds) + (wm * 4 + (lane >> 4)) * (8 * NCB);
            if (wn == 1 && (lane & 15) == 0) {
#pragma unroll
                for (int cbk = 0; cbk < NCB; ++cbk)
#pragma unroll
                    for (int j = 0; j < 4; ++j) { red[(cbk * 4 + j) * 2] = s1[cbk][j]; red[(cbk * 4 + j) * 2 + 1] = s2[cbk][j]; }
            }
            __syncthreads();
            if (wn == 0 && (lane & 15) == 0) {
#pragma unroll
                for (int cbk = 0; cbk < NCB; ++cbk)
#pragma unroll
                    for (int j = 0; j < 4; ++j) { s1[cbk][j] += red[(cbk * 4 + j) * 2]; s2[cbk][j] += red[(cbk * 4 + j) * 2 + 1]; }
            }
        }
#pragma unroll
        for (int cbk = 0; cbk < NCB; ++cbk) {
            const int co = co_real + cbk * 16 + 4 * (lane >> 4);
            if ((lane & 15) == 0 && slot < p.nslots && (TBW == 8 || wn == 0)) {
                float* st = p.stats + (((size_t)b * p.nslots + slot) * Cr + co) * 2;
                *reinterpret_cast<float4*>(st) = make_float4(s1[cbk][0], s2[cbk][0], s1[cbk][1], s2[cbk][1]);
                *reinterpret_cast<float4*>(st + 4) = make_float4(s1[cbk][2], s2[cbk][2], s1[cbk][3], s2[cbk][3]);
                const float q = fmaxf(fmaxf(s2[cbk][0], s2[cbk][1]), fmaxf(s2[cbk][2], s2[cbk][3]));
                if (p.range_flag && !(q < 1.0727e9f)) *p.range_flag = 1;
            }
        }
    }
    } else {
        const int slot = (t0 >> 7) + (TBW == 8 ? wn : 0);
        const int Ctot = p.C_out;
        float* dst[2]; const float* fx[2]; int cs[2], cc[2];
        float4 ga[2], gs[2];
        float s1[2][4], s2[2][4];
#pragma unroll
        for (int cbk = 0; cbk < 2; ++cbk) {
            const int co = co_wave + cbk * 16 + 4 * (lane >> 4);
            if (co < p.OC0) { dst[cbk] = p.y; fx[cbk] = p.fx0; cs[cbk] = p.OC0; cc[cbk] = co; }
            else            { dst[cbk] = p.y1; fx[cbk] = p.fx1; cs[cbk] = Ctot - p.OC0; cc[cbk] = co - p.OC0; }
            ga[cbk] = make_float4(1.f, 1.f, 1.f, 1.f); gs[cbk] = make_float4(0.f, 0.f, 0.f, 0.f);
            if (p.bflags & TQ_BWD_GN) {
                ga[cbk] = *reinterpret_cast<const float4*>(p.fgs + (size_t)b * Ctot + co);
                gs[cbk] = *reinterpret_cast<const float4*>(p.fgh + (size_t)b * Ctot + co);
            }
#pragma unroll
            for (int j = 0; j < 4; ++j) { s1[cbk][j] = 0.f; s2[cbk][j] = 0.f; }
        }
        const bool need_x = p.bflags & (TQ_BWD_GN | TQ_BWD_SILU | TQ_BWD_STATS);
        const bool accum = p.bflags & TQ_BWD_ACCUM;
        f32x4 lq[TBW][2];
        if (need_x || accum) {
#pragma unroll
            for (int tb = 0; tb < TBW; ++tb) {
                const int t = t0 + wn * C::WT + tb * 16 + (lane & 15);
                const int tc = t < p.T_out ? t : p.T_out - 1;
#pragma unroll
                for (int cbk = 0; cbk < 2; ++cbk) {
                    const size_t o = ((size_t)b * p.T_out + tc) * cs[cbk] + cc[cbk];
                    lq[tb][cbk] = *reinterpret_cast<const f32x4*>((need_x ? fx[cbk] : dst[cbk]) + o);
                }
            }
        }
#pragma unroll
        for (int tb = 0; tb < TBW; ++tb) {
            int t = t0 + wn * C::WT + tb * 16 + (lane & 15);
            asm volatile("" : "+v"(t));
            if (t < p.T_out) {
#pragma unroll
                for (int cbk = 0; cbk < 2; ++cbk) {
                    const int co = co_wave + cbk * 16 + 4 * (lane >> 4);
                    const size_t o = ((size_t)b * p.T_out + t) * cs[cbk] + cc[cbk];
                    float v[4] = {acc[cbk][tb][0], acc[cbk][tb][1], acc[cbk][tb][2], acc[cbk][tb][3]};
                    if constexpr (SCH == 2) { v[0] *= dy_unscale; v[1] *= dy_unscale; v[2] *= dy_unscale; v[3] *= dy_unscale; }
                    float xv[4] = {0.f, 0.f, 0.f, 0.f};
                    if (need_x) {
                        const f32x4 x4 = lq[tb][cbk];
                        xv[0] = x4[0]; xv[1] = x4[1]; xv[2] = x4[2]; xv[3] = x4[3];
                    }
                    if (p.bflags & TQ_BWD_SILU) {
                        const float a4[4] = {ga[cbk].x, ga[cbk].y, ga[cbk].z, ga[cbk].w};
                        const float h4[4] = {gs[cbk].x, gs[cbk].y, gs[cbk].z, gs[cbk].w};
#pragma unroll
                        for (int j = 0; j < 4; ++j) v[j] *= dsilu_f(a4[j] * xv[j] + h4[j]);
                    }
                    if (p.bflags & TQ_BWD_DROPOUT) {
                        const uint32_t e0 = (uint32_t)t * (uint32_t)Ctot + (uint32_t)co;
#pragma unroll
                        for (int j = 0; j < 4; ++j)
                            v[j] = (drop_hash(dkey, e0 + j) >= p.drop_thresh) ? v[j] * p.drop_scale : 0.f;
                    }
                    if (accum) {
                        f32x4 r = lq[tb][cbk];
                        if (need_x) r = *reinterpret_cast<const f32x4*>(dst[cbk] + o);
                        v[0] += r[0]; v[1] += r[1]; v[2] += r[2]; v[3] += r[3];
                    }
                    *reinterpret_cast<float4*>(dst[cbk] + o) = make_float4(v[0], v[1], v[2], v[3]);
#pragma unroll
                    for (int j = 0; j < 4; ++j) { s1[cbk][j] += v[j]; s2[cbk][j] += v[j] * xv[j]; }
                }
            }
        }
        if (p.bflags & TQ_BWD_STATS) {
#pragma unroll
            for (int cbk = 0; cbk < 2; ++cbk) {
                const int co = co_wave + cbk * 16 + 4 * (lane >> 4);
#pragma unroll
                for (int j = 0; j < 4; ++j) {
#pragma unroll
                    for (int o = 1; o < 16; o <<= 1) {
                        s1[cbk][j] += __shfl_xor(s1[cbk][j], o);
                        s2[cbk][j] += __shfl_xor(s2[cbk][j], o);
                    }
                }
                if constexpr (TBW == 8) {
                    if ((lane & 15) == 0 && slot < p.nslots) {
                        float* st = p.stats + (((size_t)b * p.nslots + slot) * Ctot + co) * 2;
                        *reinterpret_cast<float4*>(st) = make_float4(s1[cbk][0], s2[cbk][0], s1[cbk][1], s2[cbk][1]);
                        *reinterpret_cast<float4*>(st + 4) = make_float4(s1[cbk][2], s2[cbk][2], s1[cbk][3], s2[cbk][3]);
                    }
                }
            }
            if constexpr (TBW == 4) {
                __syncthreads();
                float* red = reinterpret_cast<float*>(lds) + (wm * 4 + (lane >> 4)) * 16;
                if (wn == 1 && (lane & 15) == 0) {
#pragma unroll
                    for (int cbk = 0; cbk < 2; ++cbk)
#pragma unroll
                        for (int j = 0; j < 4; ++j) { red[(cbk * 4 + j) * 2] = s1[cbk][j]; red[(cbk * 4 + j) * 2 + 1] = s2[cbk][j]; }
                }
                __syncthreads();
                if (wn == 0 && (lane & 15) == 0 && slot < p.nslots) {
#pragma unroll
                    for (int cbk = 0; cbk < 2; ++cbk) {
                        const int co = co_wave + cbk * 16 + 4 * (lane >> 4);
                        float a1[4], a2[4];
#pragma unroll
                        for (int j = 0; j < 4; ++j) { a1[j] = s1[cbk][j] + red[(cbk * 4 + j) * 2]; a2[j] = s2[cbk][j] + red[(cbk * 4 + j) * 2 + 1]; }
                        float* st = p.stats + (((size_t)b * p.nslots + slot) * Ctot + co) * 2;
                        *reinterpret_cast<float4*>(st) = make_float4(a1[0], a2[0], a1[1], a2[1]);
                        *reinterpret_cast<float4*>(st + 4) = make_float4(a1[2], a2[2], a1[3], a2[3]);
                    }
                }
            }
        }
    }
    if constexpr (PW) {
        co_wave += C::MT;
        if (++pass < npass) goto next_pass;
    }
#ifdef TQ_STAMP
    if (tid == 0 && blockIdx.x < 4096) {
        unsigned long long* tl = tq_timeline + blockIdx.x * 8;
        tl[3] = __builtin_amdgcn_s_memrealtime(); tl[7] = __builtin_amdgcn_s_memtime();
    }
#endif
}

template <int KT, int STRIDE, int UPS, int WM, int WN, int EPI, int ACT, int SCH, bool PW, int TBW, int NCB, int GTW>
struct ConvLds {
    using C = Cfg<KT, STRIDE, UPS, WM, WN, SCH, TBW, NCB>;
    static constexpr int GTAB_MAX = ((SCH == 2 && ACT >= 1) || (SCH == 0 && TBW == 2 && ACT >= 1 && !PW && EPI == 0)) ? 2 * 4 * GTW : 0;
    static constexpr int STAGE = PW ? 4 * C::BUF : C::LDS_BYTES;
    static constexpr int BYTES = STAGE + GTAB_MAX;
    static constexpr int FOLD_MAX_CIN = GTW != 1024 ? 0 : ((STAGE / 8 - 64) / 2 < 1024 ? (STAGE / 8 - 64) / 2 : 1024);
};
constexpr int TQ_LDS_WORKGROUP_MAX = 163840;

template <int KT, int STRIDE, int UPS, int WM, int WN, int EPI, int ACT, bool FUSE, int SCH = 0, bool PW = false, int TBW = 8, int NCB = 2, int GTW = 1024>
int launch(const ConvArgs& a, hipStream_t stream) {
    using C = Cfg<KT, STRIDE, UPS, WM, WN, SCH, TBW, NCB>;
    using L = ConvLds<KT, STRIDE, UPS, WM, WN, EPI, ACT, SCH, PW, TBW, NCB, GTW>;
    auto kern = conv1d_mfma_kernel<KT, STRIDE, UPS, WM, WN, EPI, ACT, FUSE, SCH, PW, TBW, NCB, GTW>;
    constexpr int GTAB_MAX = L::GTAB_MAX;
    constexpr int LDS_BYTES = L::BYTES;
    static_assert(LDS_BYTES <= TQ_LDS_WORKGROUP_MAX, "tile + coefficient table exceed the LDS a workgroup may declare");
    if (a.cf_st0 && GTW != 1024) return TQ_ERR_SHAPE;
    if (GTAB_MAX && a.cf_st0 && a.C0 + a.C1 > 1024) return TQ_ERR_SHAPE;
    if (SCH == 2 && ACT >= 1 && a.C0 + a.C1 > GTW) return TQ_ERR_SHAPE;
    if (a.cf_st0) {
        constexpr bool built = (TBW == 2 && ACT >= 1 && !PW && EPI == 0) || (SCH == 2 && ACT >= 1 && !PW && EPI == 0 && TBW == 8);
        if (!built || (size_t)(2 * (a.C0 + a.C1) + 64) * sizeof(double) > (size_t)(LDS_BYTES - GTAB_MAX)) return TQ_ERR_SHAPE;
    }
    static std::atomic<uint64_t> attr_done{0};
    int dev_ord = 0;
    (void)hipGetDevice(&dev_ord);
    const uint64_t dev_bit = 1ull << (dev_ord & 63);
    if (!(attr_done.load(std::memory_order_acquire) & dev_bit)) {
        hipError_t e = hipFuncSetAttribute(reinterpret_cast<const void*>(kern),
                                           hipFuncAttributeMaxDynamicSharedMemorySize, LDS_BYTES);
        if (e != hipSuccess) return (int)e;
        attr_done.fetch_or(dev_bit, std::memory_order_release);
    }
    const int n_ttiles = (a.T_out + C::NT - 1) / C::NT;
    const int n_ctiles = (a.C_out + C::MT - 1) / C::MT;
    const unsigned grid = (unsigned)(a.B * n_ttiles * (PW ? 1 : n_ctiles));
    hipLaunchKernelGGL(kern, dim3(grid), dim3(C::NTHR), LDS_BYTES, stream, a);
    TQ_CHECK_LAUNCH();
    return 0;
}

template <int KT, int STRIDE, int UPS, int EPI, int ACT, bool FUSE = false>
int dispatch_tile(const ConvArgs& a, hipStream_t s) {
    if (a.t_tile == 32) {
        if constexpr (KT == 5 && STRIDE == 1 && UPS == 0 && EPI == 0 && ACT >= 2) {
            if (a.flags & TQ_CONV_POLY2) return TQ_ERR_SHAPE;
            if (a.wfmt == TQ_WFMT_F16_MX6) {
                if (a.C0 % 64 || a.C1 % 64 || a.sC0 % 64 || a.sC1 % 64 || a.C_out % 128) return TQ_ERR_SHAPE;
                if (conv_wide_table(a)) return conv_launch_fwd_wide(a, KT, ACT, FUSE, s);
                return launch<KT, STRIDE, UPS, 4, 1, EPI, ACT, FUSE, 2, false, 2>(a, s);
            }
            if (a.wfmt != TQ_WFMT_BF16X3) return TQ_ERR_SHAPE;
            if (a.C_out % 128 == 0) return launch<KT, STRIDE, UPS, 4, 1, EPI, ACT, FUSE, 0, false, 2>(a, s);
            if (a.C_out % 64 == 0) return launch<KT, STRIDE, UPS, 2, 1, EPI, ACT, FUSE, 0, false, 2>(a, s);
            return launch<KT, STRIDE, UPS, 1, 1, EPI, ACT, FUSE, 0, false, 2>(a, s);
        }
        return TQ_ERR_SHAPE;
    }
    if (a.wfmt == TQ_WFMT_F16_MX6) {
        if constexpr (STRIDE == 1 && UPS == 0 && EPI == 1 && ACT == 0 && !FUSE) {
            if (a.C0 % 64 || a.C1) return TQ_ERR_SHAPE;
            if (a.C_out % 256 == 0) return launch<KT, STRIDE, UPS, 8, 1, EPI, ACT, FUSE, 2>(a, s);
            if (a.C_out % 128 == 0) return launch<KT, STRIDE, UPS, 4, 1, EPI, ACT, FUSE, 2>(a, s);
            if (a.C_out % 64 == 0) return launch<KT, STRIDE, UPS, 2, 2, EPI, ACT, FUSE, 2, false, 4>(a, s);
            return TQ_ERR_SHAPE;
        }
        if constexpr (STRIDE == 1 && EPI != 1) {
            if (a.C0 % 64 || a.C1 % 64 || a.sC0 % 64 || a.sC1 % 64) return TQ_ERR_SHAPE;
            if constexpr (UPS == 0 && EPI == 0 && ACT >= 1) {
                if (conv_wide_table(a)) return conv_launch_fwd_wide(a, KT, ACT, FUSE, s);
            }
            if constexpr (KT == 1 && UPS == 0 && ACT <= 1) {
                const int cin = a.C0 + a.C1;
                const bool pw = !(a.flags & TQ_CONV_CH_TILES);
                if (pw && a.C_out % 256 == 0 && a.C_out >= 512 && (cin == 128 || cin == 256))
                    return launch<KT, STRIDE, UPS, 8, 1, EPI, ACT, FUSE, 2, true>(a, s);
            }
            if (a.C_out % 256 == 0) return launch<KT, STRIDE, UPS, 8, 1, EPI, ACT, FUSE, 2>(a, s);
            if (a.C_out % 128 == 0) return launch<KT, STRIDE, UPS, 4, 1, EPI, ACT, FUSE, 2>(a, s);
            if constexpr (KT == 5 && UPS == 0 && EPI == 0 && ACT >= 2) {
                if (a.C_out % 64 == 0 && !(a.flags & TQ_CONV_POLY2)) return launch<KT, STRIDE, UPS, 2, 2, EPI, ACT, FUSE, 2, false, 4>(a, s);
            }
        }
        return TQ_ERR_SHAPE;
    }
    if (a.wfmt == TQ_WFMT_F16_MX8) {
        if constexpr (STRIDE == 1 && EPI != 1) {

            if (a.C0 % 64 || a.C1 % 64 || a.sC0 % 64 || a.sC1 % 64) return TQ_ERR_SHAPE;
            if constexpr (KT == 1 && UPS == 0 && ACT <= 1) {
                const int cin = a.C0 + a.C1;
                if (a.C_out % 256 == 0 && a.C_out >= 512 && (cin == 128 || cin == 256))
                    return launch<KT, STRIDE, UPS, 8, 1, EPI, ACT, FUSE, 1, true>(a, s);
            }
            if (a.C_out % 256 == 0) return launch<KT, STRIDE, UPS, 8, 1, EPI, ACT, FUSE, 1>(a, s);
            if (a.C_out % 128 == 0) return launch<KT, STRIDE, UPS, 4, 1, EPI, ACT, FUSE, 1>(a, s);
        }
        return TQ_ERR_SHAPE;
    }
    if (a.wfmt != TQ_WFMT_BF16X3) return TQ_ERR_ARG;
    if constexpr (STRIDE == 1 && UPS == 0) {
        if (a.C_out % 256 == 0) return launch<KT, STRIDE, UPS, 8, 1, EPI, ACT, FUSE>(a, s);
    }
    if (a.C_out % 128 == 0) return launch<KT, STRIDE, UPS, 4, 1, EPI, ACT, FUSE>(a, s);
    if constexpr (STRIDE == 1) {
        if (a.C_out % 64 == 0) return launch<KT, STRIDE, UPS, 2, 2, EPI, ACT, FUSE>(a, s);
        return launch<KT, STRIDE, UPS, 1, 2, EPI, ACT, FUSE>(a, s);
    } else {
        if (a.C_out % 64 == 0) return launch<KT, STRIDE, UPS, 2, 1, EPI, ACT, FUSE>(a, s);
        return launch<KT, STRIDE, UPS, 1, 1, EPI, ACT, FUSE>(a, s);
    }
}

template <int KT>
int dispatch_act(const ConvArgs& a, hipStream_t s) {
    const bool gn = a.flags & TQ_CONV_GN, silu = a.flags & TQ_CONV_SILU, drop = a.flags & TQ_CONV_DROPOUT;
    if ((!gn && silu) || (drop && !silu)) return TQ_ERR_ARG;
    if (a.sx0) {
        if constexpr (KT == 5) {
            if (gn && silu && drop) return dispatch_tile<KT, 1, 0, 0, 3, true>(a, s);
            if (gn && silu) return dispatch_tile<KT, 1, 0, 0, 2, true>(a, s);
        }
        return TQ_ERR_SHAPE;
    }
    if (gn && silu && drop) return dispatch_tile<KT, 1, 0, 0, 3>(a, s);
    if (gn && silu) return dispatch_tile<KT, 1, 0, 0, 2>(a, s);
    if (gn) return dispatch_tile<KT, 1, 0, 0, 1>(a, s);
    return dispatch_tile<KT, 1, 0, 0, 0>(a, s);
}

}
```

### tqdne_amd/csrc/conv1d_mfma.hip

```cpp
#include <cmath>

#include "common.hpp"
#include "conv_args.hpp"
#include "../../include/tqdne_hip.h"

using namespace tq;

extern "C" int tq_conv_tile_co(int C_out) {
    if (C_out % 128 == 0) return 128;
    if (C_out % 64 == 0) return 64;
    return 32;
}

static int conv1d_fwd_impl(const TqConvDesc* d, const float* x0, const float* x1, const float* gscale, const float* gshift,
                           const void* wpk, const float* bias, const float* emb, const float* res, const float* skip_x0,
                           const float* skip_x1, const float* skip_bias, float* y, float* stats, hipStream_t stream,
                           unsigned char* kv_planes = nullptr, int kvH = 0, int kvD = 0, int kvTp = 0, float kvscale = 1.f, int kv_vf16 = 0);

extern "C" int tq_conv1d_fwd_qkv(const TqConvDesc* d, const float* x, const float* gscale, const float* gshift, const void* wpk,
                                 const float* bias, float* qkv, void* kv_planes, int H, int D, int v_format, hipStream_t stream) {
    if (!d || !kv_planes || H <= 0 || (D != 32 && D != 64)) return TQ_ERR_ARG;
    if (v_format != TQ_KV_V_BF16 && v_format != TQ_KV_V_F16) return TQ_ERR_ARG;
    if (d->ktaps != 1 || d->stride != 1 || d->upsample || d->C_in1 || d->C_out != 3 * H * D || (d->C_skip0 | d->C_skip1)) return TQ_ERR_SHAPE;
    if (d->flags & (TQ_CONV_EMB | TQ_CONV_RES | TQ_CONV_STATS | TQ_CONV_DROPOUT | TQ_CONV_SILU)) return TQ_ERR_ARG;
    const int Tp = (d->T_out + 63) / 64 * 64;
    const float scale = (float)(1.0 / sqrt(sqrt((double)D)));
    return conv1d_fwd_impl(d, x, nullptr, gscale, gshift, wpk, bias, nullptr, nullptr, nullptr, nullptr, nullptr, qkv, nullptr, stream,
                           reinterpret_cast<unsigned char*>(kv_planes), H, D, Tp, scale, v_format == TQ_KV_V_F16 ? 1 : 0);
}

extern "C" int tq_conv1d_fwd(const TqConvDesc* d, const float* x0, const float* x1, const float* gscale,
                             const float* gshift, const void* wpk, const float* bias, const float* emb,
                             const float* res, float* y, float* stats, hipStream_t stream) {
    if (d && (d->C_skip0 || d->C_skip1)) return TQ_ERR_ARG;
    return conv1d_fwd_impl(d, x0, x1, gscale, gshift, wpk, bias, emb, res, nullptr, nullptr, nullptr, y, stats, stream);
}

extern "C" int tq_conv1d_fwd_skip(const TqConvDesc* d, const float* x0, const float* x1, const float* gscale,
                                  const float* gshift, const void* wpk_main_then_skip, const float* bias, const float* emb,
                                  const float* skip_x0, const float* skip_x1, const float* skip_bias, float* y, float* stats,
                                  hipStream_t stream) {
    if (!d || !skip_x0 || d->C_skip0 <= 0 || d->C_skip0 % 32 || d->C_skip1 < 0 || d->C_skip1 % 32) return TQ_ERR_ARG;
    if (d->C_skip1 > 0 && !skip_x1) return TQ_ERR_ARG;
    if (d->stride != 1 || d->upsample || (d->flags & TQ_CONV_RES)) return TQ_ERR_SHAPE;
    return conv1d_fwd_impl(d, x0, x1, gscale, gshift, wpk_main_then_skip, bias, emb, nullptr, skip_x0, skip_x1, skip_bias, y,
                           stats, stream);
}

static int conv1d_fwd_impl(const TqConvDesc* d, const float* x0, const float* x1, const float* gscale, const float* gshift,
                           const void* wpk, const float* bias, const float* emb, const float* res, const float* skip_x0,
                           const float* skip_x1, const float* skip_bias, float* y, float* stats, hipStream_t stream,
                           unsigned char* kv_planes, int kvH, int kvD, int kvTp, float kvscale, int kv_vf16) {
    if (!d || !x0 || !wpk || !y) return TQ_ERR_ARG;
    if (d->C_in0 <= 0 || d->C_in0 % 32 || d->C_in1 < 0 || d->C_in1 % 32 || d->C_out <= 0 || d->C_out % 32) return TQ_ERR_SHAPE;
    if (d->C_in1 > 0 && !x1) return TQ_ERR_ARG;
    if ((d->flags & TQ_CONV_GN) && (!gscale || !gshift)) return TQ_ERR_ARG;
    if ((d->flags & TQ_CONV_EMB) && !emb) return TQ_ERR_ARG;
    if ((d->flags & TQ_CONV_RES) && !res) return TQ_ERR_ARG;
    if ((d->flags & TQ_CONV_STATS) && !stats) return TQ_ERR_ARG;
    if (d->B <= 0 || d->T_in <= 0 || d->T_out <= 0) return TQ_ERR_SHAPE;
    if (d->stride == 1) {
        const int Tsrc = d->upsample ? 2 * d->T_in : d->T_in;
        if (d->T_out != Tsrc || d->pad != d->ktaps / 2) return TQ_ERR_SHAPE;
    } else if (d->stride == 2) {
        if (d->ktaps != 3 || d->pad != 1 || d->upsample || d->T_out != (d->T_in + 2 - 3) / 2 + 1) return TQ_ERR_SHAPE;
    } else {
        return TQ_ERR_SHAPE;
    }
    ConvArgs a;
    a.x0 = x0; a.x1 = x1; a.gscale = gscale; a.gshift = gshift;
    a.wpk = reinterpret_cast<const uint4*>(wpk);
    a.bias = bias; a.emb = emb; a.res = res; a.y = y; a.stats = stats;
    a.B = d->B; a.T_in = d->T_in; a.T_out = d->T_out; a.C0 = d->C_in0; a.C1 = d->C_in1; a.C_out = d->C_out;
    a.emb_stride = d->emb_stride; a.flags = d->flags;
    const int tile = tq_conv_tile_co(d->C_out);
    a.ncob_pad = ((d->C_out + tile - 1) / tile) * tile / 16;
    a.nslots = (d->T_out + STAT_SLOT - 1) / STAT_SLOT;
    a.t_tile = 0;
    if (d->t_tile) {
        const int need = TQ_CONV_GN | TQ_CONV_SILU;
        if (d->t_tile != 32) return TQ_ERR_ARG;
        if (d->ktaps != 5 || d->stride != 1 || d->upsample || kv_planes || (d->flags & need) != need || (d->flags & TQ_CONV_POLY2))
            return TQ_ERR_SHAPE;
        a.t_tile = 32;
        a.nslots = (d->T_out + 31) / 32;
    }
    if (d->flags & TQ_CONV_POLY2) {
        if (d->ktaps != 3 || d->stride != 1 || d->upsample || (d->C_out & 63) || kv_planes || d->C_skip0 || d->C_skip1) return TQ_ERR_SHAPE;
        if ((d->flags & TQ_CONV_STATS) && d->T_out % STAT_SLOT && d->T_out % STAT_SLOT <= STAT_SLOT / 2) return TQ_ERR_SHAPE;
        a.nslots *= 2;
    }
    a.drop_site = d->dropout_site;
    a.drop_seed = d->dropout_seed;
    float pdrop = d->dropout_p;
    if (!(d->flags & TQ_CONV_DROPOUT) || pdrop <= 0.f) { a.flags &= ~TQ_CONV_DROPOUT; pdrop = 0.f; }
    if (pdrop >= 1.f) return TQ_ERR_ARG;
    a.drop_thresh = (uint32_t)((double)pdrop * 4294967296.0);
    a.drop_scale = 1.0f / (1.0f - pdrop);
    a.fx0 = a.fx1 = a.fgs = a.fgh = nullptr; a.y1 = nullptr; a.OC0 = d->C_out; a.bflags = 0;
    a.sx0 = skip_x0; a.sx1 = skip_x1; a.sbias = skip_bias; a.sC0 = d->C_skip0; a.sC1 = d->C_skip1;
    a.wfmt = d->wfmt;
    a.kv = kv_planes; a.kvH = kvH; a.kvD = kvD; a.kvTp = kvTp; a.kvscale = kvscale; a.kv_vf16 = (kv_planes && kv_vf16) ? 1 : 0;
    a.range_flag = d->range_flag;
    a.in_amax = nullptr;
    a.cf_st0 = a.cf_st1 = a.cf_gamma = a.cf_beta = nullptr; a.cf_mean_rstd = nullptr; a.cf_ns0 = a.cf_ns1 = 0;
    if (d->gn_fold) {
        const TqGnFold* f = d->gn_fold;
        if (!(d->flags & TQ_CONV_GN) || kv_planes || (a.t_tile != 32 && d->wfmt != TQ_WFMT_F16_MX6)) return TQ_ERR_SHAPE;
        if (!f->stats0 || !f->gamma || !f->beta || (d->C_in1 > 0 && !f->stats1)) return TQ_ERR_ARG;
        const int s0 = f->slot0 ? f->slot0 : STAT_SLOT, s1 = f->slot1 ? f->slot1 : STAT_SLOT;
        if ((s0 != STAT_SLOT && s0 != 32) || (s1 != STAT_SLOT && s1 != 32)) return TQ_ERR_ARG;
        if ((d->C_in0 + d->C_in1) % GN_GROUPS) return TQ_ERR_SHAPE;
        a.cf_st0 = f->stats0; a.cf_st1 = d->C_in1 > 0 ? f->stats1 : nullptr;
        a.cf_ns0 = (d->T_in + s0 - 1) / s0; a.cf_ns1 = (d->T_in + s1 - 1) / s1;
        a.cf_gamma = f->gamma; a.cf_beta = f->beta; a.cf_mean_rstd = f->mean_rstd;
    }
    if (d->reserved1) return TQ_ERR_ARG;

    if (d->stride == 2 || d->upsample) {
        if (a.flags & (TQ_CONV_GN | TQ_CONV_SILU | TQ_CONV_DROPOUT)) return TQ_ERR_SHAPE;
        return conv_launch_resample(a, d->ktaps, d->stride, stream);
    }
    if (a.kv) {
        return conv_launch_qkv(a, stream);
    }
    switch (d->ktaps) {
        case 1: return conv_launch_fwd_k1(a, stream);
        case 3: return conv_launch_fwd_k3(a, stream);
        case 5: return conv_launch_fwd_k5(a, stream);
        default: return TQ_ERR_SHAPE;
    }
}

extern "C" int tq_conv1d_bwd_data(const TqConvBwdDesc* d, const float* dy, const void* wpk_t, const float* x0,
                                  const float* x1, const float* gscale, const float* gshift, float* dx0, float* dx1,
                                  float* gstats, hipStream_t stream) {
    if (!d || !dy || !wpk_t || !dx0) return TQ_ERR_ARG;
    if (d->C_dy <= 0 || d->C_dy % 32 || d->C_dx0 <= 0 || d->C_dx0 % 32 || d->C_dx1 < 0 || d->C_dx1 % 32) return TQ_ERR_SHAPE;
    if (d->C_dx1 > 0 && !dx1) return TQ_ERR_ARG;
    const int need_x = d->flags & (TQ_BWD_GN | TQ_BWD_SILU | TQ_BWD_STATS);
    if (need_x && (!x0 || (d->C_dx1 > 0 && !x1))) return TQ_ERR_ARG;
    if ((d->flags & TQ_BWD_GN) && (!gscale || !gshift)) return TQ_ERR_ARG;
    if ((d->flags & TQ_BWD_STATS) && !gstats) return TQ_ERR_ARG;
    if (d->B <= 0 || d->T <= 0 || (d->ktaps != 1 && d->ktaps != 3 && d->ktaps != 5)) return TQ_ERR_SHAPE;
    ConvArgs a;
    a.x0 = dy; a.x1 = nullptr; a.gscale = nullptr; a.gshift = nullptr;
    a.wpk = reinterpret_cast<const uint4*>(wpk_t);
    a.bias = nullptr; a.emb = nullptr; a.res = nullptr; a.y = dx0; a.stats = gstats;
    a.B = d->B; a.T_in = d->T; a.T_out = d->T; a.C0 = d->C_dy; a.C1 = 0; a.C_out = d->C_dx0 + d->C_dx1;
    a.emb_stride = 0; a.flags = 0;
    const int tile = tq_conv_tile_co(a.C_out);
    a.ncob_pad = ((a.C_out + tile - 1) / tile) * tile / 16;
    a.nslots = (d->T + STAT_SLOT - 1) / STAT_SLOT;
    a.drop_site = d->dropout_site; a.drop_seed = d->dropout_seed;
    float pdrop = d->dropout_p;
    a.bflags = d->flags;
    if (!(d->flags & TQ_BWD_DROPOUT) || pdrop <= 0.f) { a.bflags &= ~TQ_BWD_DROPOUT; pdrop = 0.f; }
    if (pdrop >= 1.f) return TQ_ERR_ARG;
    a.drop_thresh = (uint32_t)((double)pdrop * 4294967296.0);
    a.drop_scale = 1.0f / (1.0f - pdrop);
    a.fx0 = x0; a.fx1 = x1; a.fgs = gscale; a.fgh = gshift; a.y1 = dx1; a.OC0 = d->C_dx0;
    a.sx0 = a.sx1 = a.sbias = nullptr; a.sC0 = a.sC1 = 0;
    a.wfmt = TQ_WFMT_BF16X3;
    a.in_amax = nullptr;
    a.t_tile = 0;
    if (d->wfmt == TQ_WFMT_F16_MX6) {
        if (!d->dy_amax) return TQ_ERR_ARG;
        if (d->C_dy % 64 || a.C_out % 64) return TQ_ERR_SHAPE;
        a.wfmt = TQ_WFMT_F16_MX6;
        a.in_amax = d->dy_amax;
    } else if (d->wfmt != TQ_WFMT_BF16X3) {
        return TQ_ERR_ARG;
    }
    a.kv = nullptr; a.kvH = a.kvD = a.kvTp = 0; a.kvscale = 1.f; a.kv_vf16 = 0;
    a.range_flag = nullptr;
    a.cf_st0 = a.cf_st1 = a.cf_gamma = a.cf_beta = nullptr; a.cf_mean_rstd = nullptr; a.cf_ns0 = a.cf_ns1 = 0;
    return conv_launch_dgrad(a, d->ktaps, stream);
}

namespace {
__device__ __forceinline__ void pack_mx_body(const float* __restrict__ w, int C_out, int C_in, int K, int ncob_pad,
                                             uint4* __restrict__ out, size_t gid) {
    const int nchunks = (C_in + 63) / 64;
    const size_t total = (size_t)nchunks * K * ncob_pad * 64;
    if (gid >= total) return;
    const int lane = gid & 63;
    size_t r = gid >> 6;
    const int cob = r % ncob_pad; r /= ncob_pad;
    const int tap = r % K;
    const int chunk = r / K;
    const int row = cob * 16 + (lane & 15), kq = lane >> 4;
    auto wv = [&](int ch) -> float {
        return (row < C_out && ch < C_in) ? w[((size_t)row * C_in + ch) * K + tap] : 0.f;
    };
    f16x8 m0, m1;
#pragma unroll
    for (int j = 0; j < 8; ++j) {
        m0[j] = (_Float16)wv(chunk * 64 + 8 * kq + j);
        m1[j] = (_Float16)wv(chunk * 64 + 32 + 8 * kq + j);
    }
    int c0[4], c1[4];
#pragma unroll
    for (int q = 0; q < 4; ++q) {
        float a[4], l[4];
#pragma unroll
        for (int j = 0; j < 4; ++j) {
            const float v = wv(chunk * 64 + 16 * kq + 4 * q + j);
            a[j] = __builtin_amdgcn_fmed3f(v, -448.f, 448.f);
            l[j] = __builtin_amdgcn_fmed3f((v - (float)(_Float16)v) * 4096.f, -448.f, 448.f);
        }
        c0[q] = __builtin_amdgcn_cvt_pk_fp8_f32(a[0], a[1], 0, false);
        c0[q] = __builtin_amdgcn_cvt_pk_fp8_f32(a[2], a[3], c0[q], true);
        c1[q] = __builtin_amdgcn_cvt_pk_fp8_f32(l[0], l[1], 0, false);
        c1[q] = __builtin_amdgcn_cvt_pk_fp8_f32(l[2], l[3], c1[q], true);
    }
    const size_t o = ((((size_t)chunk * K + tap) * ncob_pad + cob) * 4) * 64 + lane;
    out[o] = __builtin_bit_cast(uint4, m0);
    out[o + 64] = __builtin_bit_cast(uint4, m1);
    out[o + 128] = make_uint4((unsigned)c0[0], (unsigned)c0[1], (unsigned)c0[2], (unsigned)c0[3]);
    out[o + 192] = make_uint4((unsigned)c1[0], (unsigned)c1[1], (unsigned)c1[2], (unsigned)c1[3]);
}

__global__ void pack_conv_weight_mx_kernel(const float* __restrict__ w, int C_out, int C_in, int K, int ncob_pad,
                                           uint4* __restrict__ out) {
    pack_mx_body(w, C_out, C_in, K, ncob_pad, out, (size_t)blockIdx.x * blockDim.x + threadIdx.x);
}

template <bool TRANSPOSED = false>
__device__ __forceinline__ void pack_mx6_body(const float* __restrict__ w, int C_out, int C_in, int K, int ncob_pad,
                                              uint4* __restrict__ out, size_t gid) {
    const int rows = TRANSPOSED ? C_in : C_out, kdim = TRANSPOSED ? C_out : C_in;
    const int nchunks = (kdim + 63) / 64;
    const size_t total = (size_t)nchunks * K * ncob_pad * 64;
    if (gid >= total) return;
    const int lane = gid & 63;
    size_t r = gid >> 6;
    const int cob = r % ncob_pad; r /= ncob_pad;
    const int tap = r % K;
    const int chunk = r / K;
    const int row = cob * 16 + (lane & 15), kq = lane >> 4;
    auto wv = [&](int ch) -> float {
        if (!(row < rows && ch < kdim)) return 0.f;
        return TRANSPOSED ? w[((size_t)ch * C_in + row) * K + (K - 1 - tap)] : w[((size_t)row * C_in + ch) * K + tap];
    };
    f16x8 m0, m1;
#pragma unroll
    for (int j = 0; j < 8; ++j) {
        m0[j] = (_Float16)wv(chunk * 64 + 8 * kq + j);
        m1[j] = (_Float16)wv(chunk * 64 + 32 + 8 * kq + j);
    }
    f32x16 wa, wl;
    float mx = 0.f;
#pragma unroll
    for (int i = 0; i < 16; ++i) {
        const float v = wv(chunk * 64 + 16 * kq + i);
        const float l = (v - (float)(_Float16)v) * 4096.f;
        wa[i] = v; wl[i] = l;
        mx = fmaxf(mx, fmaxf(fabsf(v), fabsf(l)));
    }
    const unsigned ba = e8m0_block_scale(mx);
    const u32x6 pk = cvt_2xpk16_fp6(wa, wl, __uint_as_float(ba << 23));
    const size_t o = ((((size_t)chunk * K + tap) * ncob_pad + cob) * 4) * 64 + lane;
    out[o] = __builtin_bit_cast(uint4, m0);
    out[o + 64] = __builtin_bit_cast(uint4, m1);
    out[o + 128] = make_uint4(pk[0], pk[1], pk[2], pk[3]);
    out[o + 192] = make_uint4(pk[4], pk[5], ba, 0u);
}

__global__ void pack_conv_weight_mx6_kernel(const float* __restrict__ w, int C_out, int C_in, int K, int ncob_pad,
                                            uint4* __restrict__ out, int transposed) {
    if (transposed) pack_mx6_body<true>(w, C_out, C_in, K, ncob_pad, out, (size_t)blockIdx.x * blockDim.x + threadIdx.x);
    else pack_mx6_body<false>(w, C_out, C_in, K, ncob_pad, out, (size_t)blockIdx.x * blockDim.x + threadIdx.x);
}

__device__ __forceinline__ void pack_bf16_body(const float* __restrict__ w, int C_out, int C_in, int K, int mode, int rows, int kdim,
                                               int ncob_pad, uint4* __restrict__ out, size_t gid) {
    const int nchunks = (kdim + 31) / 32;
    const size_t total = (size_t)nchunks * K * ncob_pad * 64;
    if (gid >= total) return;
    const int lane = gid & 63;
    size_t r = gid >> 6;
    const int cob = r % ncob_pad; r /= ncob_pad;
    const int tap = r % K;
    const int chunk = r / K;
    const int row = cob * 16 + (lane & 15);
    Frag hi, lo;
#pragma unroll
    for (int j = 0; j < 8; ++j) {
        const int kk = chunk * 32 + 8 * (lane >> 4) + j;
        float v = 0.f;
        if (row < rows && kk < kdim) {
            if (mode == 0) v = w[((size_t)row * C_in + kk) * K + tap];
            else           v = w[((size_t)kk * C_in + row) * K + (K - 1 - tap)];
        }
        __bf16 h, l;
        split_bf16(v, h, l);
        hi.v[j] = h; lo.v[j] = l;
    }
    const size_t o = ((((size_t)chunk * K + tap) * ncob_pad + cob) * 2) * 64 + lane;
    out[o] = hi.u;
    out[o + 64] = lo.u;
}

__global__ void pack_conv_weight_kernel(const float* __restrict__ w, int C_out, int C_in, int K, int mode,
                                        int rows, int kdim, int ncob_pad, uint4* __restrict__ out) {
    pack_bf16_body(w, C_out, C_in, K, mode, rows, kdim, ncob_pad, out, (size_t)blockIdx.x * blockDim.x + threadIdx.x);
}

__global__ __launch_bounds__(256) void pack_jobs_kernel(const TqPackJob* __restrict__ jobs, int njobs) {
    int lo = 0, hi = njobs - 1;
    while (lo < hi) {
        const int mid = (lo + hi + 1) >> 1;
        if (jobs[mid].block_begin <= (int)blockIdx.x) lo = mid; else hi = mid - 1;
    }
    const TqPackJob jb = jobs[lo];
    const size_t gid = (size_t)(blockIdx.x - jb.block_begin) * 256 + threadIdx.x;
    const float* w = reinterpret_cast<const float*>(jb.src);
    if (jb.mode == 4) {
        if (gid < (size_t)jb.C_out) reinterpret_cast<float*>(jb.dst)[gid] = w[gid];
        return;
    }
    const bool tr = jb.mode == 1 || jb.mode == 5;
    const int rows = tr ? jb.C_in : jb.C_out;
    const int kdim = tr ? jb.C_out : jb.C_in;
    const int tile = (rows % 128 == 0) ? 128 : ((rows % 64 == 0) ? 64 : 32);
    const int ncob_pad = ((rows + tile - 1) / tile) * tile / 16;
    uint4* out = reinterpret_cast<uint4*>(jb.dst);
    if (jb.mode == 2) pack_mx_body(w, jb.C_out, jb.C_in, jb.K, ncob_pad, out, gid);
    else if (jb.mode == 3) pack_mx6_body<false>(w, jb.C_out, jb.C_in, jb.K, ncob_pad, out, gid);
    else if (jb.mode == 5) pack_mx6_body<true>(w, jb.C_out, jb.C_in, jb.K, ncob_pad, out, gid);
// ... 63 lines not shown
```

### tqdne_amd/csrc/conv_args.hpp

```cpp
#pragma once
#include "common.hpp"
#include "../../include/tqdne_hip.h"

namespace tq {

struct ConvArgs {
    const float* x0;
    const float* x1;
    const float* gscale;
    const float* gshift;
    const uint4* wpk;
    const float* bias;
    const float* emb;
    const float* res;
    float* y;
    float* stats;
    int B, T_in, T_out, C0, C1, C_out;
    int emb_stride, flags, ncob_pad, nslots;
    uint32_t drop_site;
    uint32_t drop_thresh;
    float drop_scale;
    uint64_t drop_seed;
    const float* fx0;
    const float* fx1;
    const float* fgs;
    const float* fgh;
    float* y1;
    int OC0;
    int bflags;
    const float* sx0;
    const float* sx1;
    const float* sbias;
    int sC0, sC1;
    int wfmt;
    unsigned char* kv;
    int kvH, kvD, kvTp;
    float kvscale;
    int kv_vf16;
    int* range_flag;
    int t_tile;
    const uint32_t* in_amax;
    const float* cf_st0;
    const float* cf_st1;
    int cf_ns0, cf_ns1;
    const float* cf_gamma;
    const float* cf_beta;
    float* cf_mean_rstd;
};


typedef float f32x16 __attribute__((ext_vector_type(16)));
typedef float f32x2 __attribute__((ext_vector_type(2)));
typedef unsigned u32x6 __attribute__((ext_vector_type(6)));

__device__ __forceinline__ u32x6 cvt_2xpk16_fp6(const f32x16& a, const f32x16& b, float scale) {
    u32x6 out;
    asm volatile("v_cvt_scalef32_2xpk16_fp6_f32 %0, %1, %2, %3" : "=&v"(out) : "v"(a), "v"(b), "v"(scale));
    return out;
}
__device__ __forceinline__ unsigned e8m0_block_scale(float mx) {
    const unsigned b = (__float_as_uint(mx * (1.0f / 7.5f)) + 0x7FFFFFu) >> 23;
    return b < 13u ? 13u : (b > 254u ? 254u : b);
}


int conv_launch_fwd_k1(const ConvArgs& a, hipStream_t stream);
int conv_launch_fwd_k3(const ConvArgs& a, hipStream_t stream);
int conv_launch_fwd_k5(const ConvArgs& a, hipStream_t stream);
int conv_launch_fwd_k5b(const ConvArgs& a, hipStream_t stream);
int conv_launch_qkv(const ConvArgs& a, hipStream_t stream);
int conv_launch_resample(const ConvArgs& a, int ktaps, int stride, hipStream_t stream);
int conv_launch_dgrad(const ConvArgs& a, int ktaps, hipStream_t stream);
constexpr int CONV_GTAB_NARROW = 1024, CONV_GTAB_WIDE = 2048;
inline bool conv_wide_table(const ConvArgs& a) { return a.C0 + a.C1 > CONV_GTAB_NARROW || (a.flags & TQ_CONV_WIDE_TABLE); }
int conv_launch_fwd_wide(const ConvArgs& a, int ktaps, int act, bool fuse, hipStream_t stream);
int conv_launch_fwd_wide_k5(const ConvArgs& a, int act, bool fuse, hipStream_t stream);
int conv_launch_fwd_wide_k13(const ConvArgs& a, int ktaps, int act, hipStream_t stream);

}
```

### tqdne_amd/engine_bwd.py

```python

from __future__ import annotations

import ctypes as C
import math
from typing import Dict, List

import torch

from . import _lib
from ._lib import (PACK_MODE_T, TQ_AMAX_WORDS, TQ_BWD_ACCUM, TQ_BWD_DROPOUT, TQ_BWD_GN, TQ_BWD_SILU, TQ_BWD_STATS, TQ_WFMT_BF16X3, TQ_WFMT_F16_MX6, STAT_SLOT,
                   TqConvBwdDesc, TqConvDesc, _p, check)


TAIL_WORDS = 2


BWD_STREAMS = int(__import__("os").environ.get("TQDNE_BWD_STREAMS", "2"))

DGRAD_MX6_C64 = __import__("os").environ.get("TQDNE_DGRAD_MX6_C64", "0") == "1"
N_AMAX = 160


def _copy_floats(dst, src, n, stream):
    from .engine import _lib_copy_floats
    _lib_copy_floats(dst, src, n, stream)
    return 0


def _nslots(T):
    return (T + STAT_SLOT - 1) // STAT_SLOT


class BackwardPlan:
    def __init__(self, eng):
        self.e = eng
        self.lib = eng.lib
        self.B, self.dev = eng.B, eng.dev
        self.m = eng.m
        self._keep = []
        self.ops: List = []
        self.bwd_dropout_descs: List[TqConvBwdDesc] = []
        self._scratch: Dict = {}
        self.op_flops: Dict[int, int] = {}
        self._trace = None
        self._wgrad_ops = []
        self.ws_bytes = 0
        self._grad_writer = {}
        self.head_op = self.stem_op = None
        self.dx_op = None
        self.last_dx = None
        self.wide_head = eng.wide_head
        self.wide_stem = eng.wide_stem
        self.stem_cp = eng.x_btc.C if eng.wide_stem else 32
        self.stem_generic = False
        self.stem_x_btc = self.dw_stem32 = None
        self._side_evs = {}
        self._fire_cache = None
        self._gemm_levels = None
        self._layout_gradients()
        for a in eng.acts:
            a.gw = False
        self._build()
        self._finish_workspace()
        eng.enable_block_kv()

    def _finish_workspace(self):
        self.ws = torch.empty(max(self.ws_bytes, 16), dtype=torch.uint8, device=self.dev)
        for i in self._wgrad_ops:
            self.ops[i][1][7] = self.ws.data_ptr()
            self.ops[i][1][8] = self.ws.numel()

    def _empty(self, *shape):
        t = torch.empty(*shape, dtype=torch.float32, device=self.dev)
        self._keep.append(t)
        return t

    def scratch(self, tag, *shape):
        key = (tag,) + tuple(shape)
        t = self._scratch.get(key)
        if t is None:
            t = self._empty(self.B, *shape)
            self._scratch[key] = t
        return t

    def grad(self, act):
        if act.grad is None:
            act.grad = self._empty(self.B, act.T, act.C)
        return act.grad

    def _readiness_keys(self):
        e, m = self.e, self.m
        n = len(e.tape)
        key = {}

        def mark(ps, k):
            for p in ps:
                if p is not None:
                    key.setdefault(id(p), k)

        head = [m.out] if hasattr(m, "out") else [m.output_layer]
        for mod in head:
            mark(mod.parameters(), 0)
        for k, (kind, t) in enumerate(e.tape):
            pos = n - k
            if kind == "res":
                mark([p for name, p in t["rb"].named_parameters() if not name.startswith("emb_layers")], pos)
            elif kind == "attn":
                mark(t["ab"].parameters(), pos)
            elif kind in ("down_plain", "up_plain"):
                pass
            else:
                mark([t["rec"].site.weight, t["rec"].site.bias], pos)
        stem = m.input_blocks[0][0] if hasattr(m, "input_blocks") else m.input_layer
        mark(stem.parameters(), n + 1)
        return key, n + 2

    def _layout_gradients(self):
        e, m = self.e, self.m
        named = list(m.named_parameters())
        self.param_order = [p for _, p in named]
        emb_w, emb_b = [], []
        for rb in e.res_blocks:
            if hasattr(rb, "emb_layers"):
                emb_w.append(rb.emb_layers[1].weight)
                emb_b.append(rb.emb_layers[1].bias)
        emb_ids = {id(p) for p in emb_w + emb_b}
        key, last = self._readiness_keys()
        rest = [p for _, p in named if id(p) not in emb_ids]
        order = sorted(range(len(rest)), key=lambda i: (key.get(id(rest[i]), last), i))
        swept = [rest[i] for i in order if key.get(id(rest[i]), last) < last]
        tail = [rest[i] for i in order if key.get(id(rest[i]), last) >= last]
        total, offs = 0, {}
        for p in swept:
            total = (total + 63) // 64 * 64
            offs[id(p)] = total
            total += p.numel()
        total = (total + 63) // 64 * 64
        self.off_emb = total
        for p in emb_w + emb_b:
            offs[id(p)] = total
            total += p.numel()
        for p in tail:
            total = (total + 63) // 64 * 64
            offs[id(p)] = total
            total += p.numel()
        self.n_grad = total
        total += TAIL_WORDS
        total = (total + 63) // 64 * 64
        self.off_demb = total
        total += self.B * e.emb_total
        total = (total + 63) // 64 * 64
        off_amax = total
        total += N_AMAX * TQ_AMAX_WORDS
        self.flat = torch.zeros(total, dtype=torch.float32, device=self.dev)
        self.amax = self.flat[off_amax:off_amax + N_AMAX * TQ_AMAX_WORDS].view(torch.int32)
        self._amax_slot = {}
        self.dgrad_descs = []
        self._mx6_dgrads = []
        self.gview = {id(p): self.flat[offs[id(p)]:offs[id(p)] + p.numel()].view_as(p) for p in swept + emb_w + emb_b + tail}
        self.demb_all = self.flat[self.off_demb:self.off_demb + self.B * e.emb_total].view(self.B, e.emb_total)
        o = self.off_emb
        self.g_emb_w = self.flat[o:o + e.emb_total * e.E].view(e.emb_total, e.E)
        self.g_emb_b = self.flat[o + e.emb_total * e.E:o + e.emb_total * e.E + e.emb_total]
        self.offs = offs
        self._ready = {}
        self._swept_ids = {id(p) for p in swept}

    END = 1 << 30

    def plan_buckets(self, bucket_elems: int):
        spans = []
        for p in self.param_order:
            o = self.offs[id(p)]
            r = self._ready.get(id(p), self.END) if id(p) in self._swept_ids else self.END
            if r >= len(self.ops):
                r = self.END
            if not p.requires_grad:
                r = -1
            spans.append((o, o + p.numel(), r))
        spans.sort()
        buckets, lo, ready = [], 0, -1
        for o, hi, r in spans:
            ready = max(ready, r)
            if hi - lo >= bucket_elems:
                hi_al = min((hi + 63) // 64 * 64, self.n_grad)
                buckets.append((lo, hi_al, ready))
                lo = hi_al
        if lo < self.n_grad:
            buckets.append((lo, self.n_grad, max(ready, spans[-1][2]) if buckets else ready))
        out, run_max = [], -1
        for lo_, hi_, r in buckets:
            run_max = max(run_max, r)
            out.append((lo_, hi_, run_max))
        return out

    def amax_ptr(self, dy_ptr: int, create: bool = True):
        i = self._amax_slot.get(dy_ptr)
        if i is None:
            if not create or len(self._amax_slot) >= N_AMAX:
                return None
            i = self._amax_slot[dy_ptr] = len(self._amax_slot)
        return self.amax.data_ptr() + 4 * TQ_AMAX_WORDS * i

    def g(self, param):
        self._ready[id(param)] = len(self.ops)
        return self.gview[id(param)]

    def gv(self, param):
        return self.gview[id(param)]

    def _wgrad(self, rec, dy, bias_colsum=True, colsum=None, dw=None):
        lib, site = self.lib, rec.site
        need = lib.tq_conv1d_bwd_weight_workspace(C.byref(rec.desc))
        self.ws_bytes = max(self.ws_bytes, need)
        self._wgrad_ops.append(len(self.ops))
        s0 = rec.srcs[0]
        s1 = rec.srcs[1] if len(rec.srcs) > 1 else None
        if colsum is None and bias_colsum and site.bias is not None:
            colsum = (None, 0, site.bias, None)
        if colsum is not None:
            self._colsum_pass(dy, rec.out.T if rec.out is not None else rec.desc.T_out, site.C_out, *colsum, site.name)
            self._wgrad_ops[-1] = len(self.ops)
        self.op_flops[len(self.ops)] = 2 * site.C_in * site.C_out * site.K * rec.desc.T_out * self.B
        self.ops.append([lib.tq_conv1d_bwd_weight_colsum, [C.byref(rec.desc), _p(dy), _p(s0.buf), _p(s1.buf) if s1 else None,
                                                           _p(rec.gn[0]) if rec.gn else None, _p(rec.gn[1]) if rec.gn else None,
                                                           _p(dw) if dw is not None else _p(self.g(site.weight)), None, 0, None, 0, None,
                                                           None], "wgrad:" + site.name])

    def _colsum_pass(self, dy, T_dy, C_dy, bc, stride, c1, c2, name):
        lib = self.lib
        amax = self.amax_ptr(dy.data_ptr())
        wr = self._grad_writer.get(dy.data_ptr())
        if wr is not None and wr[0][0] is lib.tq_gn_bwd_apply:
            op = wr[0]
            op[0] = lib.tq_gn_bwd_apply_colsum
            op[1] = op[1] + [bc, stride, _p(self.g(c1)) if c1 is not None else None, _p(self.g(c2)) if c2 is not None else None, amax]
            op[2] = "gn_bwd_apply+colsum:" + name
        else:
            self.ops.append([lib.tq_colsum, [_p(dy), self.B, T_dy, C_dy, bc, stride,
                                             _p(self.g(c1)) if c1 is not None else None, _p(self.g(c2)) if c2 is not None else None, None, amax],
                             "colsum:" + name])

    def _dgrad(self, rec, dy, T, dsts, accumulate, chain=True, stats=True, amax_of=None):
        lib, site = self.lib, rec.site
        amax = self.amax_ptr((amax_of if amax_of is not None else dy).data_ptr(), create=False)
        cin_ok = site.C_in % 128 == 0 or (site.C_in % 64 == 0 and DGRAD_MX6_C64)
        mx6 = (_lib.requested_scheme() == "f16mx6"
               and amax is not None and site.C_out % 64 == 0 and cin_ok
               and self.e.scheme == "auto" and getattr(self.m, "_conv_scheme", "auto") == "auto")
        want = 5 if mx6 else 1
        if site.packed_t is None:
            nb = max(lib.tq_conv_weight_pack_bytes(site.C_out, site.C_in, site.K, 1),
                     lib.tq_conv_weight_pack_bytes(site.C_out, site.C_in, site.K, 5) if site.C_out % 64 == 0 else 0)
            site.packed_t = torch.empty(nb, dtype=torch.uint8, device=self.dev)
            site.pack_mode_t = want
            self.e.dgrad_sites.append(site)
        elif site.pack_mode_t != want:
            raise RuntimeError(f"{site.name}: data gradient planned twice with different weight formats")
        d = TqConvBwdDesc()
        d.wfmt = TQ_WFMT_F16_MX6 if mx6 else TQ_WFMT_BF16X3
        d.dy_amax = amax if mx6 else None
        self.dgrad_descs.append(d)
        if mx6:
            self._mx6_dgrads.append((d, site))
        d.B, d.T, d.C_dy = self.B, T, site.C_out
        d.C_dx0 = dsts[0].shape[2]
        d.C_dx1 = dsts[1].shape[2] if len(dsts) > 1 else 0
        assert d.C_dx0 + d.C_dx1 == site.C_in
        d.ktaps = site.K
        f = TQ_BWD_ACCUM if accumulate else 0
        gst = None
        s0 = rec.srcs[0]
        s1 = rec.srcs[1] if len(rec.srcs) > 1 else None
        if chain:
            if rec.gn is not None:
                f |= TQ_BWD_GN
                if stats:
                    f |= TQ_BWD_STATS
                    gst = self._empty(self.B, _nslots(T), site.C_in, 2)
            if rec.silu:
                f |= TQ_BWD_SILU
            if rec.dropout:
                self.bwd_dropout_descs.append(d)
        d.flags = f
        d.dropout_site = rec.desc.dropout_site
        self._keep.append(d)
        self.op_flops[len(self.ops)] = 2 * site.C_in * site.C_out * site.K * (rec.desc.T_out if rec.stride == 2 else T) * self.B
        self.ops.append([lib.tq_conv1d_bwd_data, [C.byref(d), _p(dy), _p(site.packed_t), _p(s0.buf) if chain else None,
                                                  _p(s1.buf) if (chain and s1) else None,
                                                  _p(rec.gn[0]) if (chain and rec.gn) else None,
                                                  _p(rec.gn[1]) if (chain and rec.gn) else None, _p(dsts[0]),
                                                  _p(dsts[1]) if len(dsts) > 1 else None, _p(gst)], "dgrad:" + site.name])
        for t_ in dsts:
            self._wrote(t_)
        return gst

    def _gn_bwd(self, gst, gn, norm, T, Ctot):
        ca, cb, cc = self._empty(self.B, Ctot), self._empty(self.B, Ctot), self._empty(self.B, Ctot)
        self.ops.append([self.lib.tq_gn_bwd_finalize, [_p(gst), _p(gn[2]), _p(norm.weight), self.B, Ctot, T, _p(ca), _p(cb), _p(cc),
                                                       _p(self.g(norm.weight)), _p(self.g(norm.bias))], "gn_bwd_finalize"])
        return ca, cb, cc

    def _gn_apply(self, G, act, coef, Ctot, coff, r=None):
        dx = self.grad(act)
        self.ops.append([self.lib.tq_gn_bwd_apply, [_p(G), _p(act.buf), _p(r), _p(coef[0]), _p(coef[1]), _p(coef[2]), _p(dx), self.B,
                                                    act.T, act.C, Ctot, coff, int(act.gw)], "gn_bwd_apply"])
        self._wrote(dx)
        act.gw = True

    def _wrote(self, grad_tensor):
        self._grad_writer[grad_tensor.data_ptr()] = (self.ops[-1],)

    def _build(self):
        e, m, lib, B = self.e, self.m, self.lib, self.B
        final = e.final
        head = m.out[2]
        from .engine import _check_head_bwd_limits
        if not self.wide_head:
            _check_head_bwd_limits(final.C, m.out_channels, head.kernel_size[0])
        Gh = self.scratch("G", final.T, final.C)
        nws = lib.tq_stem_head_bwd_workspace()
        self._ws_head = torch.empty(nws, dtype=torch.uint8, device=self.dev)
        self._ws_stem = torch.empty(nws, dtype=torch.uint8, device=self.dev)
        if self.wide_head:
            gst = self._wide_head_bwd(e.head_rec, head, final, Gh, m.out_channels)
        else:
            gst = self._empty(B, _nslots(final.T), final.C, 2)
            self.head_op = [lib.tq_head_conv_bwd_ws, [None, None, _p(final.buf), _p(e.head_gn[0]), _p(e.head_gn[1]), _p(head.weight), _p(Gh),
                                                      _p(gst), _p(self.g(head.weight)), _p(self.g(head.bias)), B, final.T, final.C,
                                                      m.out_channels, head.kernel_size[0], _p(self._ws_head), nws], "head bwd"]
        coef = self._gn_bwd(gst, e.head_gn, m.out[0], final.T, final.C)
        self._gn_apply(Gh, final, coef, final.C, 0)
        for kind, t in reversed(e.tape):
            getattr(self, "_bwd_" + kind)(t)
        stem = m.input_blocks[0][0]
        so = e.stem_out
        self.stem_op = [lib.tq_stem_conv_bwd_weight_ws, [_p(so.grad), None, None, _p(self.g(stem.weight)), B, m.in_channels, so.T,
                                                         stem.out_channels, stem.kernel_size[0], _p(self._ws_stem), nws], "stem wgrad"]
        self._ready[id(stem.weight)] = self.END
        self._stem_gradients(stem, self.wide_stem or stem.out_channels * m.in_channels * stem.kernel_size[0] > 2048, "wgrad:stem (generic)")

    def _stem_gradients(self, stem, generic: bool, what: str):
        e, lib, B, so = self.e, self.lib, self.B, self.e.stem_out
        assert so.gw
        self.stem_generic = generic
        if generic:
            K, Cp = stem.kernel_size[0], self.stem_cp
            if self.wide_stem:
                self.stem_x_btc = e.x_btc.buf
            else:
                self.stem_x_btc = self._empty(B, so.T, Cp)
                self.stem_x_btc.zero_()
            d = TqConvDesc()
            d.B, d.T_in, d.T_out, d.C_in0, d.C_in1, d.C_out = B, so.T, so.T, Cp, 0, stem.out_channels
            d.ktaps, d.stride, d.pad, d.upsample, d.flags = K, 1, K // 2, 0, 0
            self._keep.append(d)
            self.dw_stem32 = self._empty(stem.out_channels, Cp, K)
            self.ws_bytes = max(self.ws_bytes, lib.tq_conv1d_bwd_weight_workspace(C.byref(d)))
            self._wgrad_ops.append(len(self.ops))
            self.ops.append([lib.tq_conv1d_bwd_weight, [C.byref(d), _p(so.grad), _p(self.stem_x_btc), None, None, None,
                                                        _p(self.dw_stem32), None, 0], what])
        self.ops.append([lib.tq_colsum, [_p(so.grad), B, so.T, so.C, None, 0, _p(self.g(stem.bias)), None, None, None], "colsum:stem"])

    def _wide_head_bwd(self, rec, head, final, Gh, co):
        site, Cp = rec.site, rec.site.C_out
        self.dF = self._empty(self.B, final.T, Cp)
        self.head_op = [self.lib.tq_nct_to_btc, [None, None, None, _p(self.dF), self.B, co, 0, final.T, Cp], "head dF (nct_to_btc)"]
        if self.offs[id(head.bias)] % 64 or Cp > 64 or id(head.bias) not in self._swept_ids:
            raise RuntimeError(f"{site.name}: the padded bias gradient ({Cp} column sums) needs the 64-float alignment gap behind the bias "
                               "gradient in the flat buffer (_layout_gradients)")
        self._colsum_pass(self.dF, final.T, Cp, None, 0, head.bias, None, site.name)
        self.dw_head_pad = self._empty(Cp, site.C_in, site.K)
        self._wgrad(rec, self.dF, bias_colsum=False, dw=self.dw_head_pad)
        self.ops.append([_copy_floats, [_p(self.g(head.weight)), _p(self.dw_head_pad), head.weight.numel()], "wgrad:rows:" + site.name])
        return self._dgrad(rec, self.dF, final.T, [Gh], accumulate=False)

    def _recompute(self, t):
        for i in t.get("recompute") or ():
            fn, args, what, _fl = self.e.ops[i]
            self.ops.append([fn, list(args), "recompute:" + what])

    def _bwd_res(self, t):
        self._recompute(t)
        rb, srcs, h1, out = t["rb"], t["srcs"], t["h1"], t["out"]
        rec1, rec2, rec_sk = t["rec1"], t["rec2"], t["rec_sk"]
        B, T, Co = self.B, out.T, out.C
        assert out.gw, "gradient of a block output must be complete before its backward"
        dout = out.grad
        self._wgrad(rec2, dout, colsum=(None, 0, rec2.site.bias, rec_sk.site.bias if rec_sk is not None else None))
        G2 = self.scratch("G", T, Co)
        gst2 = self._dgrad(rec2, dout, T, [G2], accumulate=False)
        coef2 = self._gn_bwd(gst2, t["g2"], rb.out_layers[0], T, Co)
        h1.gw = False
        self._gn_apply(G2, h1, coef2, Co, 0)
        dh1 = h1.grad
        emb_dst = None
        if hasattr(rb, "emb_layers"):
            emb_dst = self.demb_all.data_ptr() + 4 * self.e.emb_offsets[id(rb)]
        self._wgrad(rec1, dh1, colsum=(emb_dst, self.e.emb_total, rec1.site.bias, None))
        Ctot = sum(s.C for s in srcs)
        G1 = [self.scratch("G1_%d" % i, T, s.C) for i, s in enumerate(srcs)]
        gst1 = self._dgrad(rec1, dh1, T, G1, accumulate=False)
        coef1 = self._gn_bwd(gst1, t["g1"], rb.in_layers[0], T, Ctot)
        if rec_sk is None:
            self._gn_apply(G1[0], srcs[0], coef1, Ctot, 0, r=dout)
        else:
            self._wgrad(rec_sk, dout, bias_colsum=False)
            acc = srcs[0].gw
            assert all(s.gw == acc for s in srcs)
            self._dgrad(rec_sk, dout, T, [self.grad(s) for s in srcs], accumulate=acc, chain=False)
            for s in srcs:
                s.gw = True
            coff = 0
            for Gs, s in zip(G1, srcs):
                self._gn_apply(Gs, s, coef1, Ctot, coff)
                coff += s.C

    def _bwd_attn(self, t):
        self._recompute(t)
        ab, x, qkv, att, out = t["ab"], t["x"], t["qkv"], t["att"], t["out"]
        B, T, Cc = self.B, x.T, x.C
        assert out.gw
        dout = out.grad
        self._wgrad(t["rec_proj"], dout)
        datt = self.grad(att)
        self._dgrad(t["rec_proj"], dout, T, [datt], accumulate=False, chain=False)
        dqkv = self.grad(qkv)
        delta = self._empty(B, ab.num_heads, T)
        self.op_flops[len(self.ops)] = 2 * 4 * ab.channels * T * T * B
        Tp = (T + 63) // 64 * 64
        ws = self.scratch("attn_bwd_ws", 4 * ab.num_heads * Tp * t["D"]) if t["D"] in (32, 64) else None
        if ws is not None:
            e, lib = self.e, self.lib

            def attn_bwd(qkv_p, att_p, datt_p, lse_p, delta_p, dqkv_p, ws_p, B_, T_, H_, D_, stream, _t=t):
                kv = _t.get("kv_ws") if (e._last.get("block_kv") or _t.get("kv_always")) else None
                if kv is not None:
                    return lib.tq_attention_bwd_ws_kv(qkv_p, att_p, datt_p, lse_p, delta_p, dqkv_p, ws_p, kv.data_ptr(), B_, T_, H_, D_, stream)
                return lib.tq_attention_bwd_ws(qkv_p, att_p, datt_p, lse_p, delta_p, dqkv_p, ws_p, B_, T_, H_, D_, stream)
            fn = attn_bwd
        else:
            fn = self.lib.tq_attention_bwd_ws if t["D"] in (32, 64, 128) else self.lib.tq_attention_bwd_hd
        self.ops.append([fn, [_p(qkv.buf), _p(att.buf), _p(datt), _p(t["lse"]), _p(delta), _p(dqkv), _p(ws),
                              B, T, ab.num_heads, t["D"]], "attention bwd"])
        self._wrote(dqkv)
        self._wgrad(t["rec_qkv"], dqkv)
        G = self.scratch("G", T, Cc)
        gst = self._dgrad(t["rec_qkv"], dqkv, T, [G], accumulate=False)
        coef = self._gn_bwd(gst, t["g"], ab.norm, T, Cc)
        self._gn_apply(G, x, coef, Cc, 0, r=dout)

    def _bwd_down(self, t):
        x, out, rec = t["x"], t["out"], t["rec"]
        assert out.gw
        dout = out.grad
        self._wgrad(rec, dout)
        dyz = self.scratch("dyz", x.T, out.C)
        self.ops.append([self.lib.tq_zero_stuff, [_p(dout), _p(dyz), self.B, out.T, x.T, out.C], "zero_stuff"])
        self._dgrad(rec, dyz, x.T, [self.grad(x)], accumulate=x.gw, chain=False, amax_of=dout)
        x.gw = True

    def _bwd_up_poly(self, t):
        from .engine import ConvRec
        lib = self.lib
        x, out, rec = t["x"], t["out"], t["rec"]
        ps, d2 = rec.poly
        site = rec.site
        assert out.gw and len(rec.srcs) == 1
        dout = out.grad
        self._colsum_pass(dout, out.T, site.C_out, None, 0, site.bias, None, site.name)
        dw = TqConvDesc()
        dw.B, dw.T_in, dw.T_out, dw.C_in0, dw.C_in1, dw.C_out = self.B, x.T, x.T, x.C, 0, 2 * site.C_out
        dw.ktaps, dw.stride, dw.pad, dw.upsample, dw.flags = 3, 1, 1, 0, 0
        self._keep.append(dw)
        dW2 = self._empty(2 * site.C_out, site.C_in, 3)
        self.ws_bytes = max(self.ws_bytes, lib.tq_conv1d_bwd_weight_workspace(C.byref(dw)))
        self._wgrad_ops.append(len(self.ops))
        self.op_flops[len(self.ops)] = 2 * site.C_in * 2 * site.C_out * 3 * x.T * self.B
        self.ops.append([lib.tq_conv1d_bwd_weight_colsum, [C.byref(dw), _p(dout), _p(x.buf), None, None, None, _p(dW2), None, 0,
                                                           None, 0, None, None], "wgrad:" + site.name + "+polyphase"])
        self.ops.append([lib.tq_upsample_poly_wgrad_fold, [_p(dW2), _p(self.g(site.weight)), site.C_out, site.C_in],
                         "wgrad:fold:" + site.name])
        rec2 = ConvRec(ps, d2, rec.srcs, None, None, 1, False, False, False)
        self._dgrad(rec2, dout, x.T, [self.grad(x)], accumulate=x.gw, chain=False)
        x.gw = True

    def _bwd_up(self, t):
        if t["rec"].poly is not None:
            return self._bwd_up_poly(t)
        x, out, rec = t["x"], t["out"], t["rec"]
        assert out.gw
        dout = out.grad
        self._wgrad(rec, dout)
        dup = self.scratch("dup", out.T, x.C)
        self._dgrad(rec, dout, out.T, [dup], accumulate=False, chain=False)
        self.ops.append([self.lib.tq_pair_sum, [_p(dup), _p(self.grad(x)), self.B, x.T, x.C, int(x.gw)], "pair_sum"])
        self._wrote(x.grad)
        x.gw = True

    def _bwd_down_plain(self, t):
        x, out = t["x"], t["out"]
        assert out.gw
        self.ops.append([self.lib.tq_avg_pool2_bwd, [_p(out.grad), _p(self.grad(x)), self.B, x.T, x.C, int(x.gw)], "avg_pool2_bwd"])
        self._wrote(x.grad)
        x.gw = True

    def _bwd_up_plain(self, t):
        x, out = t["x"], t["out"]
        assert out.gw
        self.ops.append([self.lib.tq_pair_sum, [_p(out.grad), _p(self.grad(x)), self.B, x.T, x.C, int(x.gw)], "pair_sum"])
        self._wrote(x.grad)
        x.gw = True

    def _input_gradient(self, stem, stream, what: str, in_scale=None, c0=None):
        lib, so = self.lib, self.e.stem_out
        cin, K = stem.in_channels, stem.kernel_size[0]
        Cp = self.stem_cp
        if cin > Cp:
            raise NotImplementedError(f"input gradient for more than {Cp} input channels")
        if self.dx_op is None:
            self.dx_btc = self._empty(self.B, so.T, Cp)
            self.stem_packed_t = torch.empty(lib.tq_conv_weight_pack_bytes(stem.out_channels, cin, K, 1), dtype=torch.uint8, device=self.dev)
            bd = TqConvBwdDesc()
            bd.B, bd.T, bd.C_dy, bd.C_dx0, bd.C_dx1, bd.ktaps, bd.flags = self.B, so.T, stem.out_channels, Cp, 0, K, 0
            self._keep.append(bd)
            self.dx_op = [lib.tq_conv1d_bwd_data, [C.byref(bd), _p(so.grad), _p(self.stem_packed_t), None, None, None, None,
                                                   _p(self.dx_btc), None, None], "dgrad:" + what]
        check(lib.tq_pack_conv_weight(stem.weight.data_ptr(), stem.out_channels, cin, K, 1, self.stem_packed_t.data_ptr(), stream),
              "pack^T " + what)
        fn, args, name = self.dx_op
        check(fn(*args, stream), name)
        if self.wide_stem:
            c0 = cin if c0 is None else c0
            dx = torch.empty(self.B, c0, so.T, dtype=torch.float32, device=self.dev)
            check(lib.tq_btc_to_nct(_p(self.dx_btc), _p(in_scale), None, None, _p(dx), self.B, so.T, Cp, 0, c0, stream),
                  "input gradient (btc_to_nct)")
            return dx
        dx = self.dx_btc[:, :, :cin].permute(0, 2, 1).contiguous()
        if in_scale is not None:
            dx.mul_(in_scale[:, None, None])
        return dx

    def _begin_run(self, stream):
        last = self.e._last
        self._follow_scheme()
        self.e.repack_transposed(stream)
        self.flat.zero_()
        self.e._arm_dropout(float(last["dropout_p"]), int(last["dropout_seed"]), self.bwd_dropout_descs, TQ_BWD_DROPOUT)
        return last

    def _sweep(self, stream, side=None, fire=None, on_bucket=None, trace=None):
        if side is None and not fire and trace is None:
            for fn, args, what in self.ops:
                rc = fn(*args, stream)
                if rc:
                    check(rc, what)
            return
        from .engine import _recorded_event
        main_t = torch.cuda.current_stream(self.dev)
        fire = fire or {}
        for i, (fn, args, what) in enumerate(self.ops):
            on = stream
            if side is not None:
                if what.startswith("recompute:"):
                    main_t.wait_stream(side)
                elif what.startswith("wgrad:"):
                    ev = self._side_evs.get(i)
                    if ev is None:
                        ev = self._side_evs[i] = torch.cuda.Event()
# ... 209 lines not shown
```

### tqdne_amd/ops.py

```python

from __future__ import annotations

import ctypes as C
from typing import Optional, Tuple

import torch

from . import _lib
from ._lib import (TQ_CONV_DROPOUT, TQ_CONV_EMB, TQ_CONV_GN, TQ_CONV_RES, TQ_CONV_SILU, TQ_CONV_STATS, STAT_SLOT,
                   TqConvDesc, _p, check)


def _stream(dev):
    return torch.cuda.current_stream(dev).cuda_stream


def nslots(T):
    return (T + STAT_SLOT - 1) // STAT_SLOT


def pack_conv_weight(w: torch.Tensor, mode: int = 0, geometry=None) -> torch.Tensor:
    lib = _lib.load()
    co, ci, k = w.shape
    gco, gci = geometry or (co, ci)
# ... 63 lines not shown
        check(lib.tq_conv1d_fwd_skip(C.byref(d), _p(x0), _p(x1), _p(gscale), _p(gshift), _p(wp), _p(bias), _p(emb), _p(sx0),
                                     _p(sx1), _p(bsk), _p(y), _p(st), _stream(x0.device)), "conv1d_skip")
        return y, st
    check(lib.tq_conv1d_fwd(C.byref(d), _p(x0), _p(x1), _p(gscale), _p(gshift), _p(wp), _p(bias), _p(emb), _p(residual),
                            _p(y), _p(st), _stream(x0.device)), "conv1d")
    return y, st


def gn_finalize(stats0, C0, T, gamma, beta, stats1=None, C1=0, slot0=0, slot1=0):
    lib = _lib.load()
    B = stats0.shape[0]
    Cn = C0 + C1
    gs, gh = torch.empty(B, Cn, device=gamma.device), torch.empty(B, Cn, device=gamma.device)
    mr = torch.empty(B, 32, 2, device=gamma.device)
    check(lib.tq_gn_finalize(_p(stats0), C0, _p(stats1), C1, B, T, _p(gamma), _p(beta), _p(gs), _p(gh), _p(mr), slot0, slot1,
                             _stream(gamma.device)), "gn_finalize")
    return gs, gh, mr


def stem_conv(x_nct, weight, bias, in_scale=None, stats=True, out=None):
    lib = _lib.load()
    B, Cin, T = x_nct.shape
    Cout, _, K = weight.shape
    if out is not None:
        y, st = out
    else:
        y = torch.empty(B, T, Cout, device=x_nct.device)
        st = torch.empty(B, nslots(T), Cout, 2, device=x_nct.device) if stats else None
    check(lib.tq_stem_conv_fwd(_p(x_nct.contiguous()), _p(in_scale), _p(weight.contiguous()), _p(bias), _p(y), _p(st), B, Cin,
                               T, Cout, K, _stream(x_nct.device)), "stem")
    return y, st


def head_conv(x, weight, bias, gscale=None, gshift=None, c_out=None, c_skip=None, skip_src=None, out=None):
    lib = _lib.load()
    B, T, Cin = x.shape
    Cout, _, K = weight.shape
    y = torch.empty(B, Cout, T, device=x.device) if out is None else out
    check(lib.tq_head_conv_fwd(_p(x), _p(gscale), _p(gshift), _p(weight.contiguous()), _p(bias), _p(c_out), _p(c_skip),
                               _p(skip_src), _p(y), B, T, Cin, Cout, K, _stream(x.device)), "head")
    return y


def nct_to_btc(x_nct, scale=None, cond_nct=None, Cp=None, out=None):
    lib = _lib.load()
    B, C0, T = x_nct.shape
    C1 = 0 if cond_nct is None else cond_nct.shape[1]
    if Cp is None:
        Cp = (C0 + C1 + 31) // 32 * 32 if out is None else out.shape[2]
    y = torch.empty(B, T, Cp, device=x_nct.device) if out is None else out
    check(lib.tq_nct_to_btc(_p(x_nct.contiguous()), _p(scale), _p(None if cond_nct is None else cond_nct.contiguous()), _p(y), B, C0, C1,
                            T, Cp, _stream(x_nct.device)), "nct_to_btc")
    return y


def btc_to_nct(v_btc, C, c_off=0, a=None, s=None, skip_src=None, out=None):
    lib = _lib.load()
    B, T, Cp = v_btc.shape
    y = torch.empty(B, C, T, device=v_btc.device) if out is None else out
    check(lib.tq_btc_to_nct(_p(v_btc), _p(a), _p(s), _p(skip_src), _p(y), B, T, Cp, c_off, C, _stream(v_btc.device)), "btc_to_nct")
    return y


def _head_dim_route(lib, D, hd):
    return bool(lib.tq_attention_head_tile(D)) and (hd or D not in (32, 64, 128))


def attention(qkv, heads, return_lse=False, workspace=True, hd=False, out=None, lse=None):
    lib = _lib.load()
    B, T, C3 = qkv.shape
    D = C3 // (3 * heads)
    out = torch.empty(B, T, heads * D, device=qkv.device) if out is None else out
    if return_lse and lse is None:
        lse = torch.empty(B, heads, T, device=qkv.device)
    if _head_dim_route(lib, D, hd):
        ws = torch.empty(lib.tq_attention_hd_workspace_bytes(B, T, heads, D), dtype=torch.uint8, device=qkv.device) if workspace else None
        check(lib.tq_attention_fwd_hd(_p(qkv), _p(out), _p(lse), _p(ws), B, T, heads, D, _stream(qkv.device)), "attention (hd)")
        return (out, lse) if return_lse else out
    ws = torch.empty(lib.tq_attention_workspace_bytes(B, T, heads, D), dtype=torch.uint8, device=qkv.device) if workspace else None
    check(lib.tq_attention_fwd(_p(qkv), _p(out), _p(lse), _p(ws), B, T, heads, D, _stream(qkv.device)), "attention")
    return (out, lse) if return_lse else out


def attention_bwd(qkv, out, dout, lse, heads, workspace=True, hd=False, dqkv=None):
    lib = _lib.load()
    B, T, C3 = qkv.shape
    D = C3 // (3 * heads)
    dqkv = torch.empty_like(qkv) if dqkv is None else dqkv
    delta = torch.empty(B, heads, T, device=qkv.device)
    if _head_dim_route(lib, D, hd):
        check(lib.tq_attention_bwd_hd(_p(qkv), _p(out), _p(dout), _p(lse), _p(delta), _p(dqkv), None, B, T, heads, D,
                                      _stream(qkv.device)), "attention bwd (hd)")
        return dqkv
    ws = (torch.empty(2 * lib.tq_attention_workspace_bytes(B, T, heads, D), dtype=torch.uint8, device=qkv.device)
          if (workspace and D in (32, 64)) else None)
    check(lib.tq_attention_bwd_ws(_p(qkv), _p(out), _p(dout), _p(lse), _p(delta), _p(dqkv), _p(ws), B, T, heads, D,
                                  _stream(qkv.device)), "attention bwd")
    return dqkv


def linear(x, w, b=None):
    lib = _lib.load()
    B, E = x.shape
    N = w.shape[0]
    out = torch.empty(B, N, device=x.device)
    check(lib.tq_linear_fwd(_p(x), _p(w.contiguous()), _p(b), _p(out), B, E, N, _stream(x.device)), "linear")
    return out


from ._lib import TQ_BWD_ACCUM, TQ_BWD_DROPOUT, TQ_BWD_GN, TQ_BWD_SILU, TQ_BWD_STATS, TqConvBwdDesc


def conv1d_bwd_data(dy, weight, *, x0=None, x1=None, gscale=None, gshift=None, silu=False, stats=False, split=None,
                    accumulate_into=None, dropout_p=0.0, dropout_seed=0, dropout_site=0, wfmt=0, dy_amax=None, pad_cin=0):
    lib = _lib.load()
    B, T, C_dy = dy.shape
    C_out, w_ci, K = weight.shape
    assert C_dy == C_out or 0 < C_dy - C_out < 32
    C_in = pad_cin or w_ci
    C0 = C_in if split is None else split
    C1 = C_in - C0
    if accumulate_into is not None:
        g0, g1 = accumulate_into
    else:
        g0 = torch.empty(B, T, C0, device=dy.device)
        g1 = torch.empty(B, T, C1, device=dy.device) if C1 else None
    st = torch.empty(B, nslots(T), C_in, 2, device=dy.device) if stats else None
    d = TqConvBwdDesc()
    d.B, d.T, d.C_dy, d.C_dx0, d.C_dx1, d.ktaps = B, T, C_dy, C0, C1, K
    f = 0
    if gscale is not None:
        f |= TQ_BWD_GN
    if silu:
        f |= TQ_BWD_SILU
    if stats:
        f |= TQ_BWD_STATS
    if accumulate_into is not None:
        f |= TQ_BWD_ACCUM
    if dropout_p > 0:
        f |= TQ_BWD_DROPOUT
    d.flags = f
    d.dropout_site, d.dropout_p, d.dropout_seed = dropout_site, dropout_p, dropout_seed
    d.wfmt = wfmt
    if wfmt == _lib.TQ_WFMT_F16_MX6:
        if dy_amax is None:
            dy_amax = amax_bits(dy)
        d.dy_amax = dy_amax.data_ptr()
    wp = pack_conv_weight(weight, _lib.PACK_MODE_T[wfmt], geometry=(C_dy, C_in))
    check(lib.tq_conv1d_bwd_data(C.byref(d), _p(dy), _p(wp), _p(x0), _p(x1), _p(gscale), _p(gshift), _p(g0), _p(g1), _p(st),
                                 _stream(dy.device)), "conv1d_bwd_data")
    return g0, g1, st


def conv1d_bwd_weight(dy, x0, wshape, *, x1=None, gscale=None, gshift=None, silu=False, stride=1, upsample=False,
                      dropout_p=0.0, dropout_seed=0, dropout_site=0, colsum=None, out=None):
    lib = _lib.load()
    B, T_in, C0 = x0.shape
    C1 = 0 if x1 is None else x1.shape[2]
    C_out, C_in, K = wshape
    T_out = dy.shape[1]
    d = TqConvDesc()
    d.B, d.T_in, d.T_out, d.C_in0, d.C_in1, d.C_out = B, T_in, T_out, C0, C1, C_out
    d.ktaps, d.stride, d.pad, d.upsample = K, stride, K // 2, int(upsample)
    f = 0
    if gscale is not None:
        f |= TQ_CONV_GN
    if silu:
        f |= TQ_CONV_SILU
    if dropout_p > 0:
        f |= TQ_CONV_DROPOUT
    d.flags = f
    d.dropout_site, d.dropout_p, d.dropout_seed = dropout_site, dropout_p, dropout_seed
    ws = torch.empty(lib.tq_conv1d_bwd_weight_workspace(C.byref(d)), dtype=torch.uint8, device=dy.device)
    dw = torch.empty(C_out, C_in, K, device=dy.device) if out is None else out
    if colsum is not None:
        bc, c1 = colsum
        check(lib.tq_conv1d_bwd_weight_colsum(C.byref(d), _p(dy), _p(x0), _p(x1), _p(gscale), _p(gshift), _p(dw), _p(ws), ws.numel(),
                                              _p(bc), C_out if bc is not None else 0, _p(c1), None, _stream(dy.device)),
              "conv1d_bwd_weight_colsum")
        return dw
    check(lib.tq_conv1d_bwd_weight(C.byref(d), _p(dy), _p(x0), _p(x1), _p(gscale), _p(gshift), _p(dw), _p(ws), ws.numel(),
                                   _stream(dy.device)), "conv1d_bwd_weight")
    return dw


def gn_bwd_finalize(gstats, mean_rstd, gamma, T):
    lib = _lib.load()
    B, _, Cn, _ = gstats.shape
    dev = gamma.device
    a, b, c = (torch.empty(B, Cn, device=dev) for _ in range(3))
    dg, db = torch.zeros(Cn, device=dev), torch.zeros(Cn, device=dev)
    check(lib.tq_gn_bwd_finalize(_p(gstats), _p(mean_rstd), _p(gamma), B, Cn, T, _p(a), _p(b), _p(c), _p(dg), _p(db),
                                 _stream(dev)), "gn_bwd_finalize")
    return a, b, c, dg, db


def gn_bwd_apply(g, x, coefs, c_total, c_offset=0, r=None, accumulate_into=None):
    lib = _lib.load()
    B, T, Cs = g.shape
    dx = accumulate_into if accumulate_into is not None else torch.empty_like(g)
    check(lib.tq_gn_bwd_apply(_p(g), _p(x), _p(r), _p(coefs[0]), _p(coefs[1]), _p(coefs[2]), _p(dx), B, T, Cs, c_total, c_offset,
                              int(accumulate_into is not None), _stream(g.device)), "gn_bwd_apply")
    return dx


def colsum(dy, per_sample=True, total=True, bscale=None, amax=None, out=None):
    lib = _lib.load()
    B, T, Cn = dy.shape
    if out is not None:
        obc, oc, oc2 = out
        check(lib.tq_colsum(_p(dy), B, T, Cn, _p(obc), Cn, _p(oc), _p(oc2), _p(bscale), _p(amax), _stream(dy.device)), "colsum")
        return obc, oc, oc2
    obc = torch.zeros(B, Cn, device=dy.device) if per_sample else None
    oc = torch.zeros(Cn, device=dy.device) if total else None
    check(lib.tq_colsum(_p(dy), B, T, Cn, _p(obc), Cn, _p(oc), None, _p(bscale), _p(amax), _stream(dy.device)), "colsum")
    return obc, oc


def amax_bits(dy):
    lib = _lib.load()
    B, T, Cn = dy.shape
    out = torch.zeros(_lib.TQ_AMAX_WORDS, dtype=torch.int32, device=dy.device)
    check(lib.tq_colsum(_p(dy), B, T, Cn, None, 0, None, None, None, _p(out), _stream(dy.device)), "colsum (amax)")
    return out


def amax_value(block) -> float:
    return float(block.max().view(torch.float32).item()) if block.numel() > 1 else float(block.view(torch.float32).item())


def gn_bwd_apply_colsum(g, x, coefs, c_total, c_offset=0, r=None, accumulate_into=None, per_sample=True, total=True, amax=None, out=None):
    lib = _lib.load()
    B, T, Cs = g.shape
    if out is not None:
        dx, obc, oc, oc2 = out
        dx = dx if dx is not None else (accumulate_into if accumulate_into is not None else torch.empty_like(g))
        check(lib.tq_gn_bwd_apply_colsum(_p(g), _p(x), _p(r), _p(coefs[0]), _p(coefs[1]), _p(coefs[2]), _p(dx), B, T, Cs, c_total, c_offset,
                                         int(accumulate_into is not None), _p(obc), Cs, _p(oc), _p(oc2), _p(amax), _stream(g.device)),
              "gn_bwd_apply_colsum")
        return dx, obc, oc, oc2
    dx = accumulate_into if accumulate_into is not None else torch.empty_like(g)
    obc = torch.zeros(B, Cs, device=g.device) if per_sample else None
    oc = torch.zeros(Cs, device=g.device) if total else None
    check(lib.tq_gn_bwd_apply_colsum(_p(g), _p(x), _p(r), _p(coefs[0]), _p(coefs[1]), _p(coefs[2]), _p(dx), B, T, Cs, c_total, c_offset,
                                     int(accumulate_into is not None), _p(obc), Cs, _p(oc), None, _p(amax), _stream(g.device)),
          "gn_bwd_apply_colsum")
    return dx, obc, oc


def zero_stuff(dy, T_in):
    lib = _lib.load()
    B, T_out, Cn = dy.shape
    out = torch.empty(B, T_in, Cn, device=dy.device)
    check(lib.tq_zero_stuff(_p(dy), _p(out), B, T_out, T_in, Cn, _stream(dy.device)), "zero_stuff")
    return out


def pair_sum(d_up, accumulate_into=None):
    lib = _lib.load()
    B, T2, Cn = d_up.shape
    dx = accumulate_into if accumulate_into is not None else torch.empty(B, T2 // 2, Cn, device=d_up.device)
    check(lib.tq_pair_sum(_p(d_up), _p(dx), B, T2 // 2, Cn, int(accumulate_into is not None), _stream(d_up.device)), "pair_sum")
    return dx


def avg_pool2(x, stats=True, out=None):
    lib = _lib.load()
    B, T_in, Cn = x.shape
    if out is not None:
        y, st = out
    else:
        y = torch.empty(B, T_in // 2, Cn, device=x.device)
        st = torch.empty(B, nslots(T_in // 2), Cn, 2, device=x.device) if stats else None
    check(lib.tq_avg_pool2_fwd(_p(x), _p(y), _p(st), B, T_in, Cn, _stream(x.device)), "avg_pool2")
    return y, st


def nearest_up2(x, stats=True, out=None):
    lib = _lib.load()
    B, T_in, Cn = x.shape
    if out is not None:
        y, st = out
    else:
        y = torch.empty(B, 2 * T_in, Cn, device=x.device)
        st = torch.empty(B, nslots(2 * T_in), Cn, 2, device=x.device) if stats else None
    check(lib.tq_nearest_up2_fwd(_p(x), _p(y), _p(st), B, T_in, Cn, _stream(x.device)), "nearest_up2")
    return y, st


def avg_pool2_bwd(dy, T_in, accumulate_into=None):
    lib = _lib.load()
    B, T_out, Cn = dy.shape
    assert T_in // 2 == T_out
    dx = accumulate_into if accumulate_into is not None else torch.empty(B, T_in, Cn, device=dy.device)
    check(lib.tq_avg_pool2_bwd(_p(dy), _p(dx), B, T_in, Cn, int(accumulate_into is not None), _stream(dy.device)), "avg_pool2_bwd")
    return dx


def stem_conv_bwd_weight(dy, x_nct, wshape, in_scale=None, workspace=True):
    lib = _lib.load()
    B, Cin, T = x_nct.shape
    Cout, _, K = wshape
    dw = torch.zeros(Cout, Cin, K, device=dy.device)
    ws = torch.empty(lib.tq_stem_head_bwd_workspace(), dtype=torch.uint8, device=dy.device) if workspace else None
    check(lib.tq_stem_conv_bwd_weight_ws(_p(dy), _p(x_nct), _p(in_scale), _p(dw), B, Cin, T, Cout, K, _p(ws), 0 if ws is None else ws.numel(),
                                         _stream(dy.device)), "stem wgrad")
# ... 18 lines not shown
```

Before: 355.5.

## Fuse GroupNorm backward apply and column sums into skip-path 1x1 dgrad epilogue

Adds an APPLY epilogue to the MFMA conv kernel for the unchained k=1 skip-connection data gradient. The epilogue computes a*G + b*x + c and adds it to the accumulator, optionally accumulates into the existing gradient, and computes column sums and amax in the same pass. This removes the separate gn_bwd_apply kernels and the extra global round trips of the dx tensor in residual-block backward. The cost is more register pressure and atomic reductions in the epilogue of that conv.

```diff
diff --git a/include/tqdne_hip.h b/include/tqdne_hip.h
--- a/include/tqdne_hip.h
+++ b/include/tqdne_hip.h
@@ -80,6 +80,23 @@
     const uint32_t* dy_amax;
 } TqConvBwdDesc;
 
+typedef struct TqBwdApply {
+    const float* g0;
+    const float* g1;
+    const float* coef_a;
+    const float* coef_b;
+    const float* coef_c;
+    float* colsum_bc0;
+    float* colsum_bc1;
+    float* colsum_c0;
+    float* colsum_c1;
+    float* colsum_c2_0;
+    float* colsum_c2_1;
+    uint32_t* amax_out0;
+    uint32_t* amax_out1;
+    int32_t bc_stride0, bc_stride1;
+} TqBwdApply;
+
 int tq_abi_version(void);
 int tq_build_flags(void);
 
@@ -118,6 +135,9 @@
 int tq_conv1d_bwd_data(const TqConvBwdDesc* desc, const float* dy, const void* packed_w_t, const float* x0, const float* x1,
                        const float* gscale, const float* gshift, float* dx0, float* dx1, float* gstats_partial,
                        hipStream_t stream);
+
+int tq_conv1d_bwd_data_apply(const TqConvBwdDesc* desc, const TqBwdApply* apply, const float* dy, const void* packed_w_t,
+                             const float* s0, const float* s1, float* dx0, float* dx1, hipStream_t stream);
 
 size_t tq_conv1d_bwd_weight_workspace(const TqConvDesc* desc);
 int tq_conv1d_bwd_weight(const TqConvDesc* desc, const float* dy, const float* x0, const float* x1, const float* gscale,
diff --git a/tqdne_amd/_build.py b/tqdne_amd/_build.py
--- a/tqdne_amd/_build.py
+++ b/tqdne_amd/_build.py
@@ -9,7 +9,7 @@
 CSRC = os.path.join(HERE, "csrc")
 LIBDIR = os.path.join(HERE, "lib")
 LIBPATH = os.path.join(LIBDIR, "libtqdne_hip.so")
-SOURCES = ["conv1d_fwd_k5a.hip", "conv1d_fwd_k5b.hip", "conv1d_fwd_k13.hip", "conv1d_resample.hip", "conv1d_dgrad.hip", "conv1d_mfma.hip",
+SOURCES = ["conv1d_fwd_k5a.hip", "conv1d_fwd_k5b.hip", "conv1d_fwd_k13.hip", "conv1d_resample.hip", "conv1d_dgrad.hip", "conv1d_dgrad_apply.hip", "conv1d_mfma.hip",
            "conv1d_fwd_wide.hip", "conv1d_fwd_wide_k13.hip", "small_ops.hip", "attention.hip", "attention_hd.hip", "backward.hip", "ends_wide.hip", "boundary.hip",
            "resample_plain.hip", "classifier.hip"]
 ARCH = "gfx950"
diff --git a/tqdne_amd/_lib.py b/tqdne_amd/_lib.py
--- a/tqdne_amd/_lib.py
+++ b/tqdne_amd/_lib.py
@@ -115,6 +115,13 @@
         ("ktaps", C.c_int32), ("flags", C.c_int32), ("dropout_site", C.c_uint32), ("dropout_p", C.c_float),
         ("dropout_seed", C.c_uint64), ("wfmt", C.c_int32), ("reserved", C.c_int32), ("dy_amax", C.c_void_p),
     ]
+
+
+class TqBwdApply(C.Structure):
+    _fields_ = [("g0", C.c_void_p), ("g1", C.c_void_p), ("coef_a", C.c_void_p), ("coef_b", C.c_void_p), ("coef_c", C.c_void_p),
+                ("colsum_bc0", C.c_void_p), ("colsum_bc1", C.c_void_p), ("colsum_c0", C.c_void_p), ("colsum_c1", C.c_void_p),
+                ("colsum_c2_0", C.c_void_p), ("colsum_c2_1", C.c_void_p), ("amax_out0", C.c_void_p), ("amax_out1", C.c_void_p),
+                ("bc_stride0", C.c_int32), ("bc_stride1", C.c_int32)]
 
 
 _PROTOS = {
@@ -178,6 +185,7 @@
     "tq_grad_clip_coef": (I, [VP, I, C.c_double, C.c_double, VP, VP]),
     "tq_ema_swap": (I, [VP, I, VP]),
     "tq_conv1d_bwd_data": (I, [VP] * 11),
+    "tq_conv1d_bwd_data_apply": (I, [VP] * 9),
     "tq_conv1d_bwd_weight_workspace": (SZ, [VP]),
     "tq_conv1d_bwd_weight": (I, [VP] * 8 + [SZ, VP]),
     "tq_conv1d_bwd_weight_colsum": (I, [VP] * 8 + [SZ, VP, I, VP, VP, VP]),
diff --git a/tqdne_amd/csrc/backward.hip b/tqdne_amd/csrc/backward.hip
--- a/tqdne_amd/csrc/backward.hip
+++ b/tqdne_amd/csrc/backward.hip
@@ -676,8 +676,8 @@
         const float4 cc = *reinterpret_cast<const float4*>(cC + ko);
         const float4 gv = reinterpret_cast<const float4*>(g)[i];
         const float4 xv = reinterpret_cast<const float4*>(x)[i];
-        float4 o = make_float4(a.x * gv.x + bb.x * xv.x + cc.x, a.y * gv.y + bb.y * xv.y + cc.y,
-                               a.z * gv.z + bb.z * xv.z + cc.z, a.w * gv.w + bb.w * xv.w + cc.w);
+        float4 o = make_float4(gn_bwd_apply_term(a.x, gv.x, bb.x, xv.x, cc.x), gn_bwd_apply_term(a.y, gv.y, bb.y, xv.y, cc.y),
+                               gn_bwd_apply_term(a.z, gv.z, bb.z, xv.z, cc.z), gn_bwd_apply_term(a.w, gv.w, bb.w, xv.w, cc.w));
         if (r) { const float4 rv = reinterpret_cast<const float4*>(r)[i]; o.x += rv.x; o.y += rv.y; o.z += rv.z; o.w += rv.w; }
         if (accum) { const float4 ov = reinterpret_cast<const float4*>(dx)[i]; o.x += ov.x; o.y += ov.y; o.z += ov.z; o.w += ov.w; }
         reinterpret_cast<float4*>(dx)[i] = o;
@@ -782,8 +782,8 @@
         const float4 kc = *reinterpret_cast<const float4*>(cC + ko);
         const size_t base = ((size_t)b * T + (size_t)slot * rpw) * Cs + 4 * c4;
         auto one = [&](const float4& gv, const float4& xv, const float4& rv, const float4& ov) -> float4 __attribute__((always_inline)) {
-            float4 o = make_float4(ka.x * gv.x + kb.x * xv.x + kc.x, ka.y * gv.y + kb.y * xv.y + kc.y,
-                                   ka.z * gv.z + kb.z * xv.z + kc.z, ka.w * gv.w + kb.w * xv.w + kc.w);
+            float4 o = make_float4(gn_bwd_apply_term(ka.x, gv.x, kb.x, xv.x, kc.x), gn_bwd_apply_term(ka.y, gv.y, kb.y, xv.y, kc.y),
+                                   gn_bwd_apply_term(ka.z, gv.z, kb.z, xv.z, kc.z), gn_bwd_apply_term(ka.w, gv.w, kb.w, xv.w, kc.w));
             o.x += rv.x; o.y += rv.y; o.z += rv.z; o.w += rv.w;
             o.x += ov.x; o.y += ov.y; o.z += ov.z; o.w += ov.w;
             return o;
@@ -894,8 +894,8 @@
             const size_t o = base + (size_t)tl * Cs;
             const float4 gv = *reinterpret_cast<const float4*>(g + o), xv = *reinterpret_cast<const float4*>(x + o);
             const float4 rv = r ? *reinterpret_cast<const float4*>(r + o) : z4, ov = accum ? *reinterpret_cast<const float4*>(dx + o) : z4;
-            float4 o4 = make_float4(ka.x * gv.x + kb.x * xv.x + kc.x, ka.y * gv.y + kb.y * xv.y + kc.y,
-                                    ka.z * gv.z + kb.z * xv.z + kc.z, ka.w * gv.w + kb.w * xv.w + kc.w);
+            float4 o4 = make_float4(gn_bwd_apply_term(ka.x, gv.x, kb.x, xv.x, kc.x), gn_bwd_apply_term(ka.y, gv.y, kb.y, xv.y, kc.y),
+                                    gn_bwd_apply_term(ka.z, gv.z, kb.z, xv.z, kc.z), gn_bwd_apply_term(ka.w, gv.w, kb.w, xv.w, kc.w));
             o4.x += rv.x; o4.y += rv.y; o4.z += rv.z; o4.w += rv.w;
             o4.x += ov.x; o4.y += ov.y; o4.z += ov.z; o4.w += ov.w;
             *reinterpret_cast<float4*>(dx + o) = o4;
diff --git a/tqdne_amd/csrc/common.hpp b/tqdne_amd/csrc/common.hpp
--- a/tqdne_amd/csrc/common.hpp
+++ b/tqdne_amd/csrc/common.hpp
@@ -67,6 +67,13 @@
     return v;
 }
 
+__device__ __forceinline__ float gn_bwd_apply_term(float ka, float g, float kb, float x, float kc) {
+    return ka * g + kb * x + kc;
+}
+__device__ __forceinline__ float amax_nan_inf(float m, float v) {
+    return v != v ? __builtin_inff() : fmaxf(m, fabsf(v));
+}
+
 __device__ __forceinline__ uint32_t mix32(uint32_t x) {
     x ^= x >> 16; x *= 0x7FEB352Du;
     x ^= x >> 15; x *= 0x846CA68Bu;
diff --git a/tqdne_amd/csrc/conv1d_dgrad_apply.hip b/tqdne_amd/csrc/conv1d_dgrad_apply.hip
--- /dev/null
+++ b/tqdne_amd/csrc/conv1d_dgrad_apply.hip
@@ -0,0 +1,20 @@
+#include "conv1d_kernel.hpp"
+
+namespace tq {
+int conv_launch_dgrad_apply(const ConvArgs& a, hipStream_t s) {
+    if (a.t_tile) return TQ_ERR_SHAPE;
+    if (a.wfmt == TQ_WFMT_F16_MX6) {
+        if (a.C0 % 64 || a.C1) return TQ_ERR_SHAPE;
+        if (a.C_out % 256 == 0) return launch<1, 1, 0, 8, 1, 1, 0, false, 2, false, 8, 2, 1024, true>(a, s);
+        if (a.C_out % 128 == 0) return launch<1, 1, 0, 4, 1, 1, 0, false, 2, false, 8, 2, 1024, true>(a, s);
+        if (a.C_out % 64 == 0) return launch<1, 1, 0, 2, 2, 1, 0, false, 2, false, 4, 2, 1024, true>(a, s);
+        return TQ_ERR_SHAPE;
+    }
+    if (a.wfmt != TQ_WFMT_BF16X3) return TQ_ERR_ARG;
+    if (a.C_out % 256 == 0) return launch<1, 1, 0, 8, 1, 1, 0, false, 0, false, 8, 2, 1024, true>(a, s);
+    if (a.C_out % 128 == 0) return launch<1, 1, 0, 4, 1, 1, 0, false, 0, false, 8, 2, 1024, true>(a, s);
+    if (a.C_out % 64 == 0) return launch<1, 1, 0, 2, 2, 1, 0, false, 0, false, 8, 2, 1024, true>(a, s);
+    if (a.C_out % 32 == 0) return launch<1, 1, 0, 1, 2, 1, 0, false, 0, false, 8, 2, 1024, true>(a, s);
+    return TQ_ERR_SHAPE;
+}
+}
diff --git a/tqdne_amd/csrc/conv1d_kernel.hpp b/tqdne_amd/csrc/conv1d_kernel.hpp
--- a/tqdne_amd/csrc/conv1d_kernel.hpp
+++ b/tqdne_amd/csrc/conv1d_kernel.hpp
@@ -40,6 +40,8 @@
 #ifndef TQ_STAGE_PRE
 #define TQ_STAGE_PRE 5
 #endif
+
+template <int V> struct IntC { static constexpr int value = V; };
 
 template <int KT, int STRIDE, int UPS, int WM, int WN, int SCH = 0, int TBW = 8, int NCB = 2>
 struct Cfg {
@@ -68,8 +70,10 @@
     static constexpr int PAD = (STRIDE == 1) ? (KT / 2) : 1;
 };
 
-template <int KT, int STRIDE, int UPS, int WM, int WN, int EPI, int ACT, bool FUSE, int SCH, bool PW = false, int TBW = 8, int NCB = 2, int GTW = 1024>
+template <int KT, int STRIDE, int UPS, int WM, int WN, int EPI, int ACT, bool FUSE, int SCH, bool PW = false, int TBW = 8, int NCB = 2, int GTW = 1024,
+          bool APPLY = false>
 __global__ __launch_bounds__(64 * WM * WN, 2) void conv1d_mfma_kernel(const ConvArgs p) {
+    static_assert(!APPLY || (EPI == 1 && KT == 1 && ACT == 0 && !FUSE && !PW), "apply term: the un-chained k = 1 data gradient");
     static_assert(GTW == 1024 || (GTW == 2048 && SCH == 2 && ACT >= 1 && EPI == 0 && !PW && STRIDE == 1 && UPS == 0 && WN == 1 && NCB == 2 && (TBW == 8 || TBW == 2)),
                   "wide coefficient table: the fp16 + MX-fp6 forward tiles of 128 and 32 positions");
     static_assert(SCH == 0 || STRIDE == 1, "the fp16-range schemes serve stride-1 launches");
@@ -959,6 +963,124 @@
             }
         }
     }
+    } else if constexpr (APPLY) {
+        const int Ctot = p.C_out;
+        float* dst[2]; const float* sx[2]; const float* gx[2]; int cs[2], cc[2]; bool second[2];
+        f32x4 ka[2], kb[2], kc[2];
+        float s1[2][4], mx[2];
+#pragma unroll
+        for (int cbk = 0; cbk < 2; ++cbk) {
+            const int co = co_wave + cbk * 16 + 4 * (lane >> 4);
+            if (co < p.OC0) { dst[cbk] = p.y; sx[cbk] = p.fx0; gx[cbk] = p.ap_g0; cs[cbk] = p.OC0; cc[cbk] = co; second[cbk] = false; }
+            else            { dst[cbk] = p.y1; sx[cbk] = p.fx1; gx[cbk] = p.ap_g1; cs[cbk] = Ctot - p.OC0; cc[cbk] = co - p.OC0; second[cbk] = true; }
+            ka[cbk] = *reinterpret_cast<const f32x4*>(p.ap_a + (size_t)b * Ctot + co);
+            kb[cbk] = *reinterpret_cast<const f32x4*>(p.ap_b + (size_t)b * Ctot + co);
+            kc[cbk] = *reinterpret_cast<const f32x4*>(p.ap_c + (size_t)b * Ctot + co);
+            mx[cbk] = 0.f;
+#pragma unroll
+            for (int j = 0; j < 4; ++j) s1[cbk][j] = 0.f;
+        }
+        auto run = [&](auto first_c, auto count_c, auto prev_c) __attribute__((always_inline)) {
+            constexpr int TB0 = decltype(first_c)::value, NB = decltype(count_c)::value;
+            constexpr bool PREV = decltype(prev_c)::value != 0;
+            f32x4 gq[NB][2], sq[NB][2], oq[PREV ? NB : 1][2];
+#pragma unroll
+            for (int i = 0; i < NB; ++i) {
+                const int t = t0 + wn * C::WT + (TB0 + i) * 16 + (lane & 15);
+                const int tc = t < p.T_out ? t : p.T_out - 1;
+#pragma unroll
+                for (int cbk = 0; cbk < 2; ++cbk) {
+                    const size_t o = ((size_t)b * p.T_out + tc) * cs[cbk] + cc[cbk];
+                    gq[i][cbk] = *reinterpret_cast<const f32x4*>(gx[cbk] + o);
+                    sq[i][cbk] = *reinterpret_cast<const f32x4*>(sx[cbk] + o);
+                    if constexpr (PREV) oq[i][cbk] = *reinterpret_cast<const f32x4*>(dst[cbk] + o);
+                }
+            }
+#pragma unroll
+            for (int i = 0; i < NB; ++i) {
+                int t = t0 + wn * C::WT + (TB0 + i) * 16 + (lane & 15);
+                asm volatile("" : "+v"(t));
+                if (t < p.T_out) {
+#pragma unroll
+                    for (int cbk = 0; cbk < 2; ++cbk) {
+                        const size_t o = ((size_t)b * p.T_out + t) * cs[cbk] + cc[cbk];
+                        float v[4] = {acc[cbk][TB0 + i][0], acc[cbk][TB0 + i][1], acc[cbk][TB0 + i][2], acc[cbk][TB0 + i][3]};
+                        if constexpr (SCH == 2) { v[0] *= dy_unscale; v[1] *= dy_unscale; v[2] *= dy_unscale; v[3] *= dy_unscale; }
+                        if constexpr (PREV) {
+#pragma unroll
+                            for (int j = 0; j < 4; ++j) v[j] += oq[i][cbk][j];
+                        }
+#pragma unroll
+                        for (int j = 0; j < 4; ++j) {
+                            v[j] = gn_bwd_apply_term(ka[cbk][j], gq[i][cbk][j], kb[cbk][j], sq[i][cbk][j], kc[cbk][j]) + v[j];
+                            s1[cbk][j] += v[j];
+                            mx[cbk] = amax_nan_inf(mx[cbk], v[j]);
+                        }
+                        *reinterpret_cast<float4*>(dst[cbk] + o) = make_float4(v[0], v[1], v[2], v[3]);
+                    }
+                }
+            }
+        };
+        if (p.bflags & TQ_BWD_ACCUM) {
+            run(IntC<0>{}, IntC<TBW / 2>{}, IntC<1>{});
+            run(IntC<TBW / 2>{}, IntC<TBW - TBW / 2>{}, IntC<1>{});
+        } else {
+            run(IntC<0>{}, IntC<TBW>{}, IntC<0>{});
+        }
+        const bool want_sum = p.cs_c[0] || p.cs_c[1] || p.cs_bc[0] || p.cs_bc[1];
+        const bool want_max = p.cs_amax[0] || p.cs_amax[1];
+        if (want_sum || want_max) {
+            unsigned m0 = 0u, m1 = 0u;
+#pragma unroll
+            for (int cbk = 0; cbk < 2; ++cbk) {
+                const unsigned m = __float_as_uint(mx[cbk]);
+                if (second[cbk]) m1 = max(m1, m); else m0 = max(m0, m);
+#pragma unroll
+                for (int j = 0; j < 4; ++j) {
+#pragma unroll
+                    for (int o = 1; o < 16; o <<= 1) s1[cbk][j] += __shfl_xor(s1[cbk][j], o);
+                }
+            }
+#pragma unroll
+            for (int o = 32; o > 0; o >>= 1) {
+                m0 = max(m0, (unsigned)__shfl_xor((int)m0, o));
+                m1 = max(m1, (unsigned)__shfl_xor((int)m1, o));
+            }
+            __syncthreads();
+            float* red = reinterpret_cast<float*>(lds);
+            unsigned* wmax = reinterpret_cast<unsigned*>(red + WN * C::MT);
+            if ((lane & 15) == 0) {
+#pragma unroll
+                for (int cbk = 0; cbk < 2; ++cbk)
+#pragma unroll
+                    for (int j = 0; j < 4; ++j) red[wn * C::MT + wm * 32 + cbk * 16 + 4 * (lane >> 4) + j] = s1[cbk][j];
+            }
+            if (lane == 0) { wmax[2 * wave] = m0; wmax[2 * wave + 1] = m1; }
+            __syncthreads();
+            if (want_sum && tid < C::MT) {
+                float s = red[tid];
+#pragma unroll
+                for (int w = 1; w < WN; ++w) s += red[w * C::MT + tid];
+                const int co = ct * C::MT + tid;
+                const bool d1 = co >= p.OC0;
+                const int cl = d1 ? co - p.OC0 : co;
+                float* bc = d1 ? p.cs_bc[1] : p.cs_bc[0];
+                float* c1 = d1 ? p.cs_c[1] : p.cs_c[0];
+                float* c2 = d1 ? p.cs_c2[1] : p.cs_c2[0];
+                const int stride = d1 ? p.cs_stride[1] : p.cs_stride[0];
+                if (bc) atomicAdd(bc + (size_t)b * stride + cl, s);
+                if (c1) atomicAdd(c1 + cl, s);
+                if (c2) atomicAdd(c2 + cl, s);
+            }
+            if (want_max && tid == 0) {
+                unsigned a0 = 0u, a1 = 0u;
+#pragma unroll
+                for (int w = 0; w < WM * WN; ++w) { a0 = max(a0, wmax[2 * w]); a1 = max(a1, wmax[2 * w + 1]); }
+                const int way = (blockIdx.x % TQ_AMAX_WAYS) * TQ_AMAX_STRIDE;
+                if (p.cs_amax[0] && a0 != 0u) atomicMax(p.cs_amax[0] + way, a0);
+                if (p.cs_amax[1] && a1 != 0u) atomicMax(p.cs_amax[1] + way, a1);
+            }
+        }
     } else {
         const int slot = (t0 >> 7) + (TBW == 8 ? wn : 0);
         const int Ctot = p.C_out;
@@ -1099,11 +1221,12 @@
 };
 constexpr int TQ_LDS_WORKGROUP_MAX = 163840;
 
-template <int KT, int STRIDE, int UPS, int WM, int WN, int EPI, int ACT, bool FUSE, int SCH = 0, bool PW = false, int TBW = 8, int NCB = 2, int GTW = 1024>
+template <int KT, int STRIDE, int UPS, int WM, int WN, int EPI, int ACT, bool FUSE, int SCH = 0, bool PW = false, int TBW = 8, int NCB = 2, int GTW = 1024,
+          bool APPLY = false>
 int launch(const ConvArgs& a, hipStream_t stream) {
     using C = Cfg<KT, STRIDE, UPS, WM, WN, SCH, TBW, NCB>;
     using L = ConvLds<KT, STRIDE, UPS, WM, WN, EPI, ACT, SCH, PW, TBW, NCB, GTW>;
-    auto kern = conv1d_mfma_kernel<KT, STRIDE, UPS, WM, WN, EPI, ACT, FUSE, SCH, PW, TBW, NCB, GTW>;
+    auto kern = conv1d_mfma_kernel<KT, STRIDE, UPS, WM, WN, EPI, ACT, FUSE, SCH, PW, TBW, NCB, GTW, APPLY>;
     constexpr int GTAB_MAX = L::GTAB_MAX;
     constexpr int LDS_BYTES = L::BYTES;
     static_assert(LDS_BYTES <= TQ_LDS_WORKGROUP_MAX, "tile + coefficient table exceed the LDS a workgroup may declare");
diff --git a/tqdne_amd/csrc/conv1d_mfma.hip b/tqdne_amd/csrc/conv1d_mfma.hip
--- a/tqdne_amd/csrc/conv1d_mfma.hip
+++ b/tqdne_amd/csrc/conv1d_mfma.hip
@@ -132,9 +132,8 @@
     }
 }
 
-extern "C" int tq_conv1d_bwd_data(const TqConvBwdDesc* d, const float* dy, const void* wpk_t, const float* x0,
-                                  const float* x1, const float* gscale, const float* gshift, float* dx0, float* dx1,
-                                  float* gstats, hipStream_t stream) {
+static int bwd_data_args(const TqConvBwdDesc* d, const float* dy, const void* wpk_t, const float* x0, const float* x1,
+                         const float* gscale, const float* gshift, float* dx0, float* dx1, float* gstats, ConvArgs& a) {
     if (!d || !dy || !wpk_t || !dx0) return TQ_ERR_ARG;
     if (d->C_dy <= 0 || d->C_dy % 32 || d->C_dx0 <= 0 || d->C_dx0 % 32 || d->C_dx1 < 0 || d->C_dx1 % 32) return TQ_ERR_SHAPE;
     if (d->C_dx1 > 0 && !dx1) return TQ_ERR_ARG;
@@ -143,7 +142,6 @@
     if ((d->flags & TQ_BWD_GN) && (!gscale || !gshift)) return TQ_ERR_ARG;
     if ((d->flags & TQ_BWD_STATS) && !gstats) return TQ_ERR_ARG;
     if (d->B <= 0 || d->T <= 0 || (d->ktaps != 1 && d->ktaps != 3 && d->ktaps != 5)) return TQ_ERR_SHAPE;
-    ConvArgs a;
     a.x0 = dy; a.x1 = nullptr; a.gscale = nullptr; a.gshift = nullptr;
     a.wpk = reinterpret_cast<const uint4*>(wpk_t);
     a.bias = nullptr; a.emb = nullptr; a.res = nullptr; a.y = dx0; a.stats = gstats;
@@ -175,7 +173,38 @@
     a.kv = nullptr; a.kvH = a.kvD = a.kvTp = 0; a.kvscale = 1.f; a.kv_vf16 = 0;
     a.range_flag = nullptr;
     a.cf_st0 = a.cf_st1 = a.cf_gamma = a.cf_beta = nullptr; a.cf_mean_rstd = nullptr; a.cf_ns0 = a.cf_ns1 = 0;
-    return conv_launch_dgrad(a, d->ktaps, stream);
+    return 0;
+}
+
+extern "C" int tq_conv1d_bwd_data(const TqConvBwdDesc* d, const float* dy, const void* wpk_t, const float* x0,
+                                  const float* x1, const float* gscale, const float* gshift, float* dx0, float* dx1,
+                                  float* gstats, hipStream_t stream) {
+    ConvArgs a;
+    const int rc = bwd_data_args(d, dy, wpk_t, x0, x1, gscale, gshift, dx0, dx1, gstats, a);
+    return rc ? rc : conv_launch_dgrad(a, d->ktaps, stream);
+}
+
+extern "C" int tq_conv1d_bwd_data_apply(const TqConvBwdDesc* d, const TqBwdApply* ap, const float* dy, const void* wpk_t,
+                                        const float* s0, const float* s1, float* dx0, float* dx1, hipStream_t stream) {
+    if (!d || !ap || !s0 || !ap->g0 || !ap->coef_a || !ap->coef_b || !ap->coef_c) return TQ_ERR_ARG;
+    if (d->flags & ~TQ_BWD_ACCUM) return TQ_ERR_ARG;
+    if (d->ktaps != 1) return TQ_ERR_SHAPE;
+    if (d->C_dx1 > 0 && (!s1 || !ap->g1)) return TQ_ERR_ARG;
+    if ((ap->colsum_c2_0 && !ap->colsum_c0) || (ap->colsum_c2_1 && !ap->colsum_c1)) return TQ_ERR_ARG;
+    ConvArgs a;
+    const int rc = bwd_data_args(d, dy, wpk_t, nullptr, nullptr, nullptr, nullptr, dx0, dx1, nullptr, a);
+    if (rc) return rc;
+    const bool two = d->C_dx1 > 0;
+    a.fx0 = s0; a.fx1 = two ? s1 : nullptr;
+    a.ap_g0 = ap->g0; a.ap_g1 = two ? ap->g1 : nullptr;
+    a.ap_a = ap->coef_a; a.ap_b = ap->coef_b; a.ap_c = ap->coef_c;
+    a.cs_bc[0] = ap->colsum_bc0; a.cs_stride[0] = ap->bc_stride0; a.cs_c[0] = ap->colsum_c0; a.cs_c2[0] = ap->colsum_c2_0;
+    a.cs_amax[0] = ap->amax_out0;
+    if (two) {
+        a.cs_bc[1] = ap->colsum_bc1; a.cs_stride[1] = ap->bc_stride1; a.cs_c[1] = ap->colsum_c1; a.cs_c2[1] = ap->colsum_c2_1;
+        a.cs_amax[1] = ap->amax_out1;
+    }
+    return conv_launch_dgrad_apply(a, stream);
 }
 
 namespace {
diff --git a/tqdne_amd/csrc/conv_args.hpp b/tqdne_amd/csrc/conv_args.hpp
--- a/tqdne_amd/csrc/conv_args.hpp
+++ b/tqdne_amd/csrc/conv_args.hpp
@@ -46,6 +46,16 @@
     const float* cf_gamma;
     const float* cf_beta;
     float* cf_mean_rstd;
+    const float* ap_g0 = nullptr;
+    const float* ap_g1 = nullptr;
+    const float* ap_a = nullptr;
+    const float* ap_b = nullptr;
+    const float* ap_c = nullptr;
+    float* cs_bc[2] = {nullptr, nullptr};
+    float* cs_c[2] = {nullptr, nullptr};
+    float* cs_c2[2] = {nullptr, nullptr};
+    uint32_t* cs_amax[2] = {nullptr, nullptr};
+    int cs_stride[2] = {0, 0};
 };
 
 
@@ -71,6 +81,7 @@
 int conv_launch_qkv(const ConvArgs& a, hipStream_t stream);
 int conv_launch_resample(const ConvArgs& a, int ktaps, int stride, hipStream_t stream);
 int conv_launch_dgrad(const ConvArgs& a, int ktaps, hipStream_t stream);
+int conv_launch_dgrad_apply(const ConvArgs& a, hipStream_t stream);
 constexpr int CONV_GTAB_NARROW = 1024, CONV_GTAB_WIDE = 2048;
 inline bool conv_wide_table(const ConvArgs& a) { return a.C0 + a.C1 > CONV_GTAB_NARROW || (a.flags & TQ_CONV_WIDE_TABLE); }
 int conv_launch_fwd_wide(const ConvArgs& a, int ktaps, int act, bool fuse, hipStream_t stream);
diff --git a/tqdne_amd/engine_bwd.py b/tqdne_amd/engine_bwd.py
--- a/tqdne_amd/engine_bwd.py
+++ b/tqdne_amd/engine_bwd.py
@@ -9,7 +9,7 @@
 
 from . import _lib
 from ._lib import (PACK_MODE_T, TQ_AMAX_WORDS, TQ_BWD_ACCUM, TQ_BWD_DROPOUT, TQ_BWD_GN, TQ_BWD_SILU, TQ_BWD_STATS, TQ_WFMT_BF16X3, TQ_WFMT_F16_MX6, STAT_SLOT,
-                   TqConvBwdDesc, TqConvDesc, _p, check)
+                   TqBwdApply, TqConvBwdDesc, TqConvDesc, _p, check)
 
 
 TAIL_WORDS = 2
@@ -236,12 +236,49 @@
             op[0] = lib.tq_gn_bwd_apply_colsum
             op[1] = op[1] + [bc, stride, _p(self.g(c1)) if c1 is not None else None, _p(self.g(c2)) if c2 is not None else None, amax]
             op[2] = "gn_bwd_apply+colsum:" + name
+        elif wr is not None and wr[0][0] is lib.tq_conv1d_bwd_data_apply:
+            op, ap, i = wr
+            if c2 is not None and c1 is None:
+                raise RuntimeError(name + ": a second column-sum destination without a first")
+            for field, v in (("colsum_bc%d", bc), ("bc_stride%d", stride), ("colsum_c%d", _p(self.g(c1)) if c1 is not None else None),
+                             ("colsum_c2_%d", _p(self.g(c2)) if c2 is not None else None), ("amax_out%d", amax)):
+                setattr(ap, field % i, v)
+            op[2] += "+colsum:" + name
         else:
             self.ops.append([lib.tq_colsum, [_p(dy), self.B, T_dy, C_dy, bc, stride,
                                              _p(self.g(c1)) if c1 is not None else None, _p(self.g(c2)) if c2 is not None else None, None, amax],
                              "colsum:" + name])
 
     def _dgrad(self, rec, dy, T, dsts, accumulate, chain=True, stats=True, amax_of=None):
+        lib, site = self.lib, rec.site
+        d = self._dgrad_desc(rec, dy, T, dsts, amax_of)
+        f = TQ_BWD_ACCUM if accumulate else 0
+        gst = None
+        s0 = rec.srcs[0]
+        s1 = rec.srcs[1] if len(rec.srcs) > 1 else None
+        if chain:
+            if rec.gn is not None:
+                f |= TQ_BWD_GN
+                if stats:
+                    f |= TQ_BWD_STATS
+                    gst = self._empty(self.B, _nslots(T), site.C_in, 2)
+            if rec.silu:
+                f |= TQ_BWD_SILU
+            if rec.dropout:
+                self.bwd_dropout_descs.append(d)
+        d.flags = f
+        d.dropout_site = rec.desc.dropout_site
+        self.op_flops[len(self.ops)] = 2 * site.C_in * site.C_out * site.K * (rec.desc.T_out if rec.stride == 2 else T) * self.B
+        self.ops.append([lib.tq_conv1d_bwd_data, [C.byref(d), _p(dy), _p(site.packed_t), _p(s0.buf) if chain else None,
+                                                  _p(s1.buf) if (chain and s1) else None,
+                                                  _p(rec.gn[0]) if (chain and rec.gn) else None,
+                                                  _p(rec.gn[1]) if (chain and rec.gn) else None, _p(dsts[0]),
+                                                  _p(dsts[1]) if len(dsts) > 1 else None, _p(gst)], "dgrad:" + site.name])
+        for t_ in dsts:
+            self._wrote(t_)
+        return gst
+
+    def _dgrad_desc(self, rec, dy, T, dsts, amax_of=None):
         lib, site = self.lib, rec.site
         amax = self.amax_ptr((amax_of if amax_of is not None else dy).data_ptr(), create=False)
         cin_ok = site.C_in % 128 == 0 or (site.C_in % 64 == 0 and DGRAD_MX6_C64)
@@ -268,32 +305,27 @@
         d.C_dx1 = dsts[1].shape[2] if len(dsts) > 1 else 0
         assert d.C_dx0 + d.C_dx1 == site.C_in
         d.ktaps = site.K
-        f = TQ_BWD_ACCUM if accumulate else 0
-        gst = None
-        s0 = rec.srcs[0]
-        s1 = rec.srcs[1] if len(rec.srcs) > 1 else None
-        if chain:
-            if rec.gn is not None:
-                f |= TQ_BWD_GN
-                if stats:
-                    f |= TQ_BWD_STATS
-                    gst = self._empty(self.B, _nslots(T), site.C_in, 2)
-            if rec.silu:
-                f |= TQ_BWD_SILU
-            if rec.dropout:
-                self.bwd_dropout_descs.append(d)
-        d.flags = f
+        self._keep.append(d)
+        return d
+
+    def _dgrad_apply(self, rec, dy, T, srcs, G, coef, accumulate):
+        lib, site = self.lib, rec.site
+        dsts = [self.grad(s) for s in srcs]
+        d = self._dgrad_desc(rec, dy, T, dsts)
+        assert d.ktaps == 1 and not (rec.gn or rec.silu or rec.dropout), site.name
+        d.flags = TQ_BWD_ACCUM if accumulate else 0
         d.dropout_site = rec.desc.dropout_site
-        self._keep.append(d)
-        self.op_flops[len(self.ops)] = 2 * site.C_in * site.C_out * site.K * (rec.desc.T_out if rec.stride == 2 else T) * self.B
-        self.ops.append([lib.tq_conv1d_bwd_data, [C.byref(d), _p(dy), _p(site.packed_t), _p(s0.buf) if chain else None,
-                                                  _p(s1.buf) if (chain and s1) else None,
-                                                  _p(rec.gn[0]) if (chain and rec.gn) else None,
-                                                  _p(rec.gn[1]) if (chain and rec.gn) else None, _p(dsts[0]),
-                                                  _p(dsts[1]) if len(dsts) > 1 else None, _p(gst)], "dgrad:" + site.name])
-        for t_ in dsts:
-            self._wrote(t_)
-        return gst
+        ap = TqBwdApply()
+        ap.g0, ap.g1 = _p(G[0]), (_p(G[1]) if len(G) > 1 else None)
+        ap.coef_a, ap.coef_b, ap.coef_c = _p(coef[0]), _p(coef[1]), _p(coef[2])
+        self._keep.append(ap)
+        self.op_flops[len(self.ops)] = 2 * site.C_in * site.C_out * T * self.B
+        self.ops.append([lib.tq_conv1d_bwd_data_apply, [C.byref(d), C.byref(ap), _p(dy), _p(site.packed_t), _p(srcs[0].buf),
+                                                        _p(srcs[1].buf) if len(srcs) > 1 else None, _p(dsts[0]),
+                                                        _p(dsts[1]) if len(dsts) > 1 else None], "dgrad:" + site.name + "+gn_bwd_apply"])
+        for i, (t_, s) in enumerate(zip(dsts, srcs)):
+            self._grad_writer[t_.data_ptr()] = (self.ops[-1], ap, i)
+            s.gw = True
 
     def _gn_bwd(self, gst, gn, norm, T, Ctot):
         ca, cb, cc = self._empty(self.B, Ctot), self._empty(self.B, Ctot), self._empty(self.B, Ctot)
@@ -408,13 +440,7 @@
             self._wgrad(rec_sk, dout, bias_colsum=False)
             acc = srcs[0].gw
             assert all(s.gw == acc for s in srcs)
-            self._dgrad(rec_sk, dout, T, [self.grad(s) for s in srcs], accumulate=acc, chain=False)
-            for s in srcs:
-                s.gw = True
-            coff = 0
-            for Gs, s in zip(G1, srcs):
-                self._gn_apply(Gs, s, coef1, Ctot, coff)
-                coff += s.C
+            self._dgrad_apply(rec_sk, dout, T, srcs, G1, coef1, accumulate=acc)
 
     def _bwd_attn(self, t):
         self._recompute(t)
diff --git a/tqdne_amd/ops.py b/tqdne_amd/ops.py
--- a/tqdne_amd/ops.py
+++ b/tqdne_amd/ops.py
@@ -239,6 +239,36 @@
     return g0, g1, st
 
 
+def conv1d_bwd_data_apply(dy, weight, srcs, G, coefs, *, accumulate_into=None, wfmt=0, dy_amax=None, sums=None):
+    lib = _lib.load()
+    B, T, C_dy = dy.shape
+    C_out, C_in, K = weight.shape
+    assert K == 1 and C_dy == C_out and len(srcs) == len(G) in (1, 2) and sum(s.shape[2] for s in srcs) == C_in
+    dx = list(accumulate_into) if accumulate_into is not None else [torch.empty_like(s) for s in srcs]
+    d = _lib.TqConvBwdDesc()
+    d.B, d.T, d.C_dy, d.C_dx0, d.C_dx1, d.ktaps = B, T, C_dy, srcs[0].shape[2], srcs[1].shape[2] if len(srcs) > 1 else 0, 1
+    d.flags = _lib.TQ_BWD_ACCUM if accumulate_into is not None else 0
+    d.wfmt = wfmt
+    if wfmt == _lib.TQ_WFMT_F16_MX6:
+        if dy_amax is None:
+            dy_amax = amax_bits(dy)
+        d.dy_amax = dy_amax.data_ptr()
+    ap = _lib.TqBwdApply()
+    ap.g0, ap.g1 = _p(G[0]), _p(G[1]) if len(G) > 1 else None
+    ap.coef_a, ap.coef_b, ap.coef_c = _p(coefs[0]), _p(coefs[1]), _p(coefs[2])
+    for i, s in enumerate(sums or ()):
+        if s:
+            setattr(ap, "colsum_bc%d" % i, _p(s.get("bc")))
+            setattr(ap, "bc_stride%d" % i, srcs[i].shape[2] if s.get("bc") is not None else 0)
+            setattr(ap, "colsum_c%d" % i, _p(s.get("c")))
+            setattr(ap, "colsum_c2_%d" % i, _p(s.get("c2")))
+            setattr(ap, "amax_out%d" % i, _p(s.get("amax")))
+    wp = pack_conv_weight(weight, _lib.PACK_MODE_T[wfmt])
+    check(lib.tq_conv1d_bwd_data_apply(C.byref(d), C.byref(ap), _p(dy), _p(wp), _p(srcs[0]), _p(srcs[1]) if len(srcs) > 1 else None,
+                                       _p(dx[0]), _p(dx[1]) if len(dx) > 1 else None, _stream(dy.device)), "conv1d_bwd_data_apply")
+    return dx
+
+
 def conv1d_bwd_weight(dy, x0, wshape, *, x1=None, gscale=None, gshift=None, silu=False, stride=1, upsample=False,
                       dropout_p=0.0, dropout_seed=0, dropout_site=0, colsum=None, out=None):
     lib = _lib.load()
```

Result: no change. 356.1 (median of 6 runs) (+0.2%).
